# ZJU-FAST-Lab/Fast-Racing

Hardware: AMD Instinct MI355X
Metric: constraint-samples/s (higher is better)
Workload: dtype f64; 1 GPU; headline: 32 candidate trajs/GPU x 64 pieces x 16 quadrature intervals (34816 constraint samples/step/GPU), 16-gate Zhangjiajie-like corridor, K_i=8; state=iterate after 60 L-BFGS iterations from the reference initial guess, parallelism=candidates sharded 32/GPU, no data-path collective, front_end=one process, one device

## Files before the change

### fast-racing_amd/__init__.py

```python
from __future__ import annotations

import ctypes as C
import os

import numpy as np

from . import scenario

HERE = os.path.dirname(os.path.abspath(__file__))
LIB_PATH = os.path.join(HERE, "libfrx.so")

_dp = np.ctypeslib.ndpointer(dtype=np.float64, flags="C_CONTIGUOUS")
_ip = np.ctypeslib.ndpointer(dtype=np.int32, flags="C_CONTIGUOUS")


class FrxConfig(C.Structure):
    _fields_ = [
        ("rho", C.c_double), ("total_t", C.c_double), ("grid_res", C.c_double),
        ("qd_intervals", C.c_int), ("c2_diffeo", C.c_int),
        ("horiz_half_len", C.c_double), ("vert_half_len", C.c_double), ("safe_margin", C.c_double),
        ("vel_max", C.c_double), ("thr_acc_min", C.c_double), ("thr_acc_max", C.c_double),
        ("body_rate_max", C.c_double), ("grav_acc", C.c_double),
        ("penalty_pvtb", C.c_double * 4),
    ]

    @classmethod
    def from_params(cls, params: dict, **override):
        p = dict(params); p.update(override)
        c = cls()
        for name, _ in cls._fields_:
            if name == "penalty_pvtb":
                c.penalty_pvtb = (C.c_double * 4)(*p["penalty_pvtb"])
            else:
                setattr(c, name, p[name])
        return c


class LbfgsParams(C.Structure):
    _fields_ = [
        ("mem_size", C.c_int), ("g_epsilon", C.c_double), ("past", C.c_int), ("delta", C.c_double),
        ("max_iterations", C.c_int), ("max_linesearch", C.c_int), ("min_step", C.c_double), ("max_step", C.c_double),
        ("f_dec_coeff", C.c_double), ("s_curv_coeff", C.c_double), ("xtol", C.c_double),
    ]


BATCH_EVAL_FN = C.CFUNCTYPE(None, C.c_void_p, C.c_int, C.POINTER(C.c_int), C.POINTER(C.c_double), C.POINTER(C.c_double),
                            C.POINTER(C.c_double))

ABI_SYMBOLS = [
    "frx_version", "frx_last_error", "frx_device_count", "frx_lbfgs_default_params", "frx_lbfgs_gcopter_params",
    "frx_problem_create", "frx_problem_destroy", "frx_problem_set_solver", "frx_problem_set_lbfgs_mode", "frx_problem_totals", "frx_problem_layout", "frx_initial_guess",
    "frx_objective_eval", "frx_objective_eval_device", "frx_penalty_eval", "frx_penalty_eval_device", "frx_forward",
    "frx_optimize", "frx_optimize_stats", "frx_lbfgs_minimize_batch",
    "frx_problem_create_from_h", "frx_enumerate_vertices", "frx_traj_to_msg", "frx_msg_sample", "frx_line_segment_dilate", "frx_corridor_generate", "frx_traj_max_rates", "frx_objective_eval_async", "frx_wait",
    "frx_problem_set_resident", "frx_optimize_path", "frx_penalty_problem_create", "frx_eval_status",
    "frx_dilate_batch", "frx_multi_create", "frx_multi_destroy", "frx_multi_info", "frx_multi_layout", "frx_multi_initial_guess", "frx_multi_optimize", "frx_multi_last_exchange",
    "frx_map_mark_cloud", "frx_map_is_blocked", "frx_grid_search", "frx_jps_plan", "frx_route_plan",
    "frx_trajectory_check", "frx_trajectory_check_device", "frx_trajectory_sample", "frx_trajectory_sample_device",
    "frx_trajectory_extrema", "frx_trajectory_extrema_device",
    "frx_gate_from_corners", "frx_trajectory_gates", "frx_trajectory_gates_device", "frx_gate_flags",
    "frx_trajectory_clearance", "frx_trajectory_clearance_workspace", "frx_trajectory_clearance_device",
    "frx_corridor_generate_batch", "frx_corridor_generate_batch_device",
    "frx_enumerate_vertices_batch", "frx_enumerate_vertices_batch_device", "frx_corridor_slots_to_tasks_device",
]
DEBUG_SYMBOLS = [
    "frx_debug_trace", "frx_resident_profile", "frx_debug_direction_log", "frx_debug_direction_log_read", "frx_debug_set_resident_retry",
    "frx_debug_resident_counts", "frx_debug_resident_clusters", "frx_debug_resident_predictions", "frx_eval_stage_times", "frx_profile_phases", "frx_dv_selftest", "frx_jps_tables", "frx_debug_host_cpu_share", "frx_debug_taken_over", "frx_debug_compact_from_history",
    "frx_debug_set_eval_fused", "frx_debug_eval_fused", "frx_debug_eval_geometry", "frx_debug_set_eval_solo", "frx_debug_eval_solo", "frx_debug_penalty_kernel", "frx_debug_mailbox_numa", "frx_eval_launch_time", "frx_debug_profile_eval_cluster", "frx_debug_profile_eval_tail", "frx_debug_set_takeover_at", "frx_debug_shader_clock",
    "frx_debug_set_clear_chunk", "frx_debug_map_blocked_device", "frx_debug_dv_layout", "frx_debug_dv_round", "frx_debug_fold_rows",
]

CHECK_FIELDS = ("corridor", "speed", "thrust_min", "thrust_max", "body_rate", "acc", "worst_t", "worst_k")
CHECK_MAX_INTERVALS = 16384
CHECK_FLAG_CORRIDOR, CHECK_FLAG_SPEED, CHECK_FLAG_THRUST_MIN, CHECK_FLAG_THRUST_MAX, CHECK_FLAG_BODY_RATE, CHECK_FLAG_NONFINITE = 1, 2, 4, 8, 16, 32
EXTREMA_FIELDS = ("speed", "acc", "thrust_min", "thrust_max", "body_rate", "t_speed", "t_acc", "t_thrust_min", "t_thrust_max", "t_body_rate")
GATE_FIELDS = ("n_cross", "n_pass", "margin", "time", "piece", "u", "v", "reach_u", "reach_v", "normal_speed")
GATE_FLAG_MISSED, GATE_FLAG_REPEAT, GATE_FLAG_ORDER, GATE_FLAG_NONFINITE = 1, 2, 4, 8
CLEAR_FIELDS = ("ell", "dist", "worst_t", "worst_i")
CLEAR_MAX_POINTS = 1 << 24
CLEAR_FLAG_COLLISION, CLEAR_FLAG_NONFINITE = 1, 2
CLEAR_TILE, CLEAR_PASS = 64, 1024
SAMPLE_FIELDS = 20
SAMPLE_VIEWS = dict(pos=slice(0, 3), vel=slice(3, 6), acc=slice(6, 9), jerk=slice(9, 12), thrust=12, quat=slice(13, 17), omega=slice(17, 20))

_lib = None


def lib():
    global _lib
    if _lib is None:
        if not os.path.exists(LIB_PATH):
            raise RuntimeError(f"{LIB_PATH} is missing: build it first (python -c 'import __graft_entry__ as g; g.build()'). "
                               "There is no fallback implementation.")
        L = C.CDLL(LIB_PATH)
        L.frx_version.restype = C.c_int
        L.frx_last_error.restype = C.c_char_p
        L.frx_device_count.restype = C.c_int
        L.frx_lbfgs_default_params.argtypes = [C.POINTER(LbfgsParams)]
        L.frx_lbfgs_gcopter_params.argtypes = [C.POINTER(LbfgsParams), C.c_double]
        L.frx_problem_create.argtypes = [C.POINTER(FrxConfig), C.c_int, C.c_int, _ip, _dp, _dp, _ip, _dp, _ip, _dp, C.POINTER(C.c_void_p)]
        L.frx_problem_create_from_h.argtypes = [C.POINTER(FrxConfig), C.c_int, C.c_int, _ip, _dp, _dp, _ip, _dp, C.POINTER(C.c_void_p)]
        L.frx_enumerate_vertices.argtypes = [C.c_int, _dp, C.c_void_p, C.c_int, C.POINTER(C.c_int)]
        _up = np.ctypeslib.ndpointer(dtype=np.uint32, flags='C_CONTIGUOUS')
        L.frx_traj_to_msg.argtypes = [C.c_int, _dp, _dp, _dp, _dp, _dp, _dp, _up]
        L.frx_msg_sample.argtypes = [C.c_int, _dp, _dp, _dp, _dp, _up, C.c_double, _dp, _dp, _dp, _dp]
        L.frx_dv_selftest.argtypes = [C.c_int, C.c_int, C.c_int, C.c_int, C.c_int, C.c_void_p, C.c_uint, C.POINTER(C.c_double), C.POINTER(C.c_double)]
        L.frx_debug_dv_layout.argtypes = [C.c_int, C.c_void_p, C.c_int, C.c_void_p]
        L.frx_debug_dv_round.argtypes = [C.c_int, C.c_int, C.c_int, C.c_void_p, C.c_int] + [C.c_void_p] * 17
        L.frx_line_segment_dilate.argtypes = [_dp, _dp, _dp, C.c_int, C.c_void_p, C.c_double, C.c_int, C.POINTER(C.c_int), C.c_void_p, C.c_void_p, C.c_void_p]
        L.frx_corridor_generate.argtypes = [C.c_int, _dp, C.c_int, C.c_void_p, _dp, C.c_double, C.c_double, BLOCKED_FN, C.c_void_p, C.c_int, C.c_int,
                                            C.POINTER(C.c_int), _ip, _dp]
        L.frx_traj_max_rates.argtypes = [C.c_int, _dp, _dp, _dp, _dp]
        L.frx_objective_eval_async.argtypes = [C.c_void_p, _dp, _dp, _dp]
        L.frx_wait.argtypes = [C.c_void_p]
        L.frx_problem_set_resident.argtypes = [C.c_void_p, C.c_int]
        L.frx_optimize_path.argtypes = [C.c_void_p, C.POINTER(C.c_int), C.POINTER(C.c_uint)]
        L.frx_debug_trace.argtypes = [C.c_void_p, C.c_void_p, C.c_int]
        L.frx_resident_profile.argtypes = [C.c_void_p, C.c_void_p, C.c_int]
        L.frx_debug_direction_log.argtypes = [C.c_void_p, C.c_int, C.c_int]
        L.frx_debug_direction_log_read.argtypes = [C.c_void_p, C.c_int, C.c_void_p, C.c_int, C.POINTER(C.c_int), C.POINTER(C.c_int)]
        L.frx_debug_set_resident_retry.argtypes = [C.c_void_p, C.c_int]
        L.frx_debug_resident_counts.argtypes = [C.c_void_p, C.POINTER(C.c_int), C.POINTER(C.c_int)]
        L.frx_debug_resident_predictions.argtypes = [C.c_void_p, C.c_void_p]
        L.frx_debug_resident_clusters.argtypes = [C.c_void_p, C.POINTER(C.c_int)]
        L.frx_dilate_batch.argtypes = [C.c_int, C.c_int, _dp, _dp, _dp, C.c_int, C.c_void_p, C.c_double, C.c_int, _ip, _dp, _dp, _dp]
        L.frx_eval_stage_times.argtypes = [C.c_void_p, _dp, C.c_int, _dp]
        L.frx_eval_launch_time.argtypes = [C.c_void_p, _dp, C.c_int, _dp]
        L.frx_debug_set_eval_fused.argtypes = [C.c_void_p, C.c_int]
        L.frx_debug_eval_fused.argtypes = [C.c_void_p]
        L.frx_debug_eval_geometry.argtypes = [C.c_void_p]
        L.frx_debug_set_eval_solo.argtypes = [C.c_void_p, C.c_int]
        L.frx_debug_eval_solo.argtypes = [C.c_void_p]
        L.frx_debug_penalty_kernel.argtypes = [C.c_void_p]
        L.frx_debug_mailbox_numa.argtypes = [C.c_void_p, C.c_void_p]
        L.frx_debug_profile_eval_cluster.argtypes = [C.c_void_p, _dp, C.c_void_p]
        L.frx_debug_profile_eval_tail.argtypes = [C.c_void_p, _dp, C.c_void_p]
        L.frx_multi_create.argtypes = [C.POINTER(FrxConfig), C.c_int, C.c_void_p, C.c_int, _ip, _dp, _dp, _ip, _dp, _ip, _dp, C.POINTER(C.c_void_p)]
        L.frx_multi_destroy.argtypes = [C.c_void_p]
        L.frx_multi_info.argtypes = [C.c_void_p, C.POINTER(C.c_int), C.POINTER(C.c_int), C.c_void_p, C.c_void_p]
        L.frx_multi_layout.argtypes = [C.c_void_p, _ip, _ip]
        L.frx_multi_initial_guess.argtypes = [C.c_void_p, _dp]
        L.frx_multi_optimize.argtypes = [C.c_void_p, C.POINTER(LbfgsParams), _dp, _dp, _dp, _dp, _dp, _ip, _ip, _ip, C.POINTER(C.c_int), C.POINTER(C.c_double),
                                         _dp, _dp, C.POINTER(C.c_int)]
        L.frx_multi_last_exchange.argtypes = [C.c_void_p]
        L.frx_problem_destroy.argtypes = [C.c_void_p]
        L.frx_problem_set_solver.argtypes = [C.c_void_p, C.c_int]
        L.frx_problem_set_lbfgs_mode.argtypes = [C.c_void_p, C.c_int]
        L.frx_profile_phases.argtypes = [C.c_void_p, _dp, np.ctypeslib.ndpointer(dtype=np.int64, flags='C_CONTIGUOUS')]
        L.frx_problem_totals.argtypes = [C.c_void_p, _ip]
        L.frx_problem_layout.argtypes = [C.c_void_p, _ip, _ip, _ip, _ip]
        L.frx_initial_guess.argtypes = [C.c_void_p, _dp]
        L.frx_objective_eval.argtypes = [C.c_void_p, _dp, _dp, _dp]
        L.frx_objective_eval_device.argtypes = [C.c_void_p, C.c_void_p, C.c_void_p, C.c_void_p, C.c_void_p]
        L.frx_penalty_eval.argtypes = [C.c_void_p, _dp, _dp, _dp, _dp, _dp]
        L.frx_penalty_eval_device.argtypes = [C.c_void_p, C.c_void_p, C.c_void_p, C.c_void_p, C.c_void_p]
        L.frx_forward.argtypes = [C.c_void_p, _dp, _dp, _dp]
        L.frx_trajectory_check.argtypes = [C.c_void_p, C.c_void_p, C.c_void_p, C.c_int, C.c_void_p, C.c_void_p, C.c_void_p]
        L.frx_trajectory_check_device.argtypes = [C.c_void_p, C.c_void_p, C.c_void_p, C.c_int, C.c_void_p, C.c_void_p]
        L.frx_trajectory_extrema.argtypes = [C.c_void_p, C.c_void_p, C.c_void_p, C.c_void_p, C.c_void_p, C.c_void_p]
        L.frx_trajectory_extrema_device.argtypes = [C.c_void_p, C.c_void_p, C.c_void_p, C.c_void_p, C.c_void_p]
        L.frx_gate_from_corners.argtypes = [C.c_int, C.c_void_p, C.c_void_p, C.c_void_p]
        L.frx_trajectory_gates.argtypes = [C.c_void_p] * 7
        L.frx_trajectory_gates_device.argtypes = [C.c_void_p, C.c_void_p, C.c_void_p, C.c_int, C.c_void_p, C.c_void_p, C.c_void_p, C.c_void_p]
        L.frx_gate_flags.argtypes = [C.c_int, C.c_void_p, C.c_void_p, C.c_void_p]
        L.frx_trajectory_sample.argtypes = [C.c_void_p, C.c_void_p, C.c_void_p, C.c_int, C.c_double, C.c_double, C.c_void_p, C.c_void_p]
        L.frx_trajectory_sample_device.argtypes = [C.c_void_p, C.c_void_p, C.c_void_p, C.c_int, C.c_double, C.c_double, C.c_void_p, C.c_void_p, C.c_void_p]
        L.frx_trajectory_clearance.argtypes = [C.c_void_p, C.c_void_p, C.c_void_p, C.c_int, C.c_int, C.c_void_p, C.c_void_p, C.c_void_p, C.c_void_p]
        L.frx_trajectory_clearance_workspace.argtypes = [C.c_void_p, C.c_int, C.c_int, C.POINTER(C.c_size_t)]
        L.frx_trajectory_clearance_device.argtypes = [C.c_void_p, C.c_void_p, C.c_void_p, C.c_int, C.c_int, C.c_void_p, C.c_void_p, C.c_void_p, C.c_void_p]
        L.frx_debug_set_clear_chunk.argtypes = [C.c_void_p, C.c_int]
        L.frx_debug_fold_rows.argtypes = [C.c_int, C.c_int] + [C.c_void_p] * 6
        L.frx_corridor_generate_batch.argtypes = [C.c_int, C.c_int, C.c_void_p, C.c_void_p, C.c_int, C.c_void_p, C.c_void_p, C.c_double, C.c_double, C.c_void_p, C.c_int, C.c_int,
                                                  C.c_void_p, C.c_void_p, C.c_int, C.c_void_p, C.c_void_p, C.c_void_p]
        L.frx_corridor_generate_batch_device.argtypes = [C.c_int, C.c_void_p, C.c_void_p, C.c_int, C.c_void_p, C.c_void_p, C.c_double, C.c_double, C.c_void_p, C.c_int, C.c_int,
                                                         C.c_void_p, C.c_void_p, C.c_void_p, C.c_void_p, C.c_void_p]
        L.frx_enumerate_vertices_batch.argtypes = [C.c_int, C.c_int, C.c_void_p, C.c_void_p, C.c_void_p, C.c_int, C.c_void_p, C.c_void_p, C.c_int, C.c_void_p, C.c_void_p]
        L.frx_enumerate_vertices_batch_device.argtypes = [C.c_int, C.c_void_p, C.c_void_p, C.c_int, C.c_void_p, C.c_void_p, C.c_void_p, C.c_void_p]
        L.frx_corridor_slots_to_tasks_device.argtypes = [C.c_int, C.c_int, C.c_int, C.c_void_p, C.c_void_p, C.c_void_p, C.c_void_p]
        L.frx_debug_map_blocked_device.argtypes = [C.c_int, C.c_void_p, C.c_int, C.c_void_p, C.c_void_p, C.c_void_p]
        L.frx_optimize.argtypes = [C.c_void_p, C.POINTER(LbfgsParams), _dp, _dp, _dp, _dp, _dp, _ip, _ip, _ip]
        L.frx_optimize_stats.argtypes = [C.c_void_p, _dp]
        L.frx_lbfgs_minimize_batch.argtypes = [C.c_int, _ip, _dp, _dp, _ip, _ip, _ip, C.POINTER(LbfgsParams), BATCH_EVAL_FN,
                                               C.c_void_p, C.c_int]
        _vp = C.c_void_p
        L.frx_map_mark_cloud.argtypes = [C.c_double * 3, C.c_int * 3, C.c_double, C.c_int, _vp, _vp]
        L.frx_map_is_blocked.argtypes = [_vp, _vp, _vp]
        L.frx_grid_search.argtypes = [_vp, _vp, _vp, _vp, C.c_double, C.c_int, C.c_int, C.c_int, _vp, _vp, _vp, _vp]
        L.frx_jps_tables.argtypes = [_vp] * 6
        L.frx_jps_plan.argtypes = [_vp, _vp, _vp, C.c_double, C.c_int, C.c_int, _vp, _vp, _vp, _vp, _vp, _vp, _vp, _vp]
        L.frx_route_plan.argtypes = [_vp, _vp, _vp, C.c_int, _vp, C.c_double, C.c_int, C.c_int, C.c_int, _vp, _vp, _vp, _vp]
        for name in ABI_SYMBOLS + DEBUG_SYMBOLS:
            fn = getattr(L, name)
            if name not in ("frx_version", "frx_last_error", "frx_device_count", "frx_lbfgs_default_params",
                            "frx_lbfgs_gcopter_params", "frx_problem_destroy"):
                fn.restype = C.c_int
        _lib = L
    return _lib


class FrxError(RuntimeError):
    code = 0


def _check(rc: int):
    if rc != 0:
        e = FrxError(f"frx error {rc}: {lib().frx_last_error().decode()}")
        e.code = rc
        raise e


def shader_clock(device: int = 0, ms: float = 2.0):
    a, b, c = C.c_double(), C.c_double(), C.c_double()
    _check(lib().frx_debug_shader_clock(device, C.c_double(ms), C.byref(a), C.byref(b), C.byref(c)))
    return a.value, b.value, c.value


def gcopter_lbfgs_params(rel_cost_tol: float, max_iterations: int = 0) -> LbfgsParams:
    p = LbfgsParams()
    lib().frx_lbfgs_gcopter_params(C.byref(p), rel_cost_tol)
    p.max_iterations = max_iterations
    return p


def pack_batch(cands):
    coarse_n = np.array([c.coarse_n for c in cands], dtype=np.int32)
    ini = np.concatenate([c.ini_state.T.reshape(-1) for c in cands]).astype(np.float64)
    fin = np.concatenate([c.fin_state.T.reshape(-1) for c in cands]).astype(np.float64)
    h_off = [0]; v_off = [0]; h_rec = []; v_rec = []
    for c in cands:
        for h in c.h_polys:
            h_off.append(h_off[-1] + h.shape[1]); h_rec.append(h.T.reshape(-1))
        for v in c.v_polys:
            v_off.append(v_off[-1] + v.shape[1]); v_rec.append(v.T.reshape(-1))
    v_all = np.concatenate(v_rec).astype(np.float64) if v_rec else np.zeros(0)
    return (coarse_n, ini, fin, np.array(h_off, dtype=np.int32), np.concatenate(h_rec).astype(np.float64),
            np.array(v_off, dtype=np.int32), v_all)


def enumerate_vertices(hpoly: np.ndarray) -> np.ndarray:
    rec = np.ascontiguousarray(hpoly.T.reshape(-1), dtype=np.float64)
    nv = C.c_int()
    _check(lib().frx_enumerate_vertices(hpoly.shape[1], rec, None, 0, C.byref(nv)))
    out = np.zeros(3 * nv.value)
    _check(lib().frx_enumerate_vertices(hpoly.shape[1], rec, out.ctypes.data, nv.value, C.byref(nv)))
    return out.reshape(-1, 3).T.copy()


BLOCKED_FN = C.CFUNCTYPE(C.c_int, C.POINTER(C.c_double), C.POINTER(C.c_double), C.c_void_p)


def line_segment_dilate(p1, p2, bbox, obs, offset: float = 0.0):
    p1 = np.ascontiguousarray(p1, dtype=np.float64); p2 = np.ascontiguousarray(p2, dtype=np.float64); bbox = np.ascontiguousarray(bbox, dtype=np.float64)
    obs = np.ascontiguousarray(obs, dtype=np.float64).reshape(-1, 3)
    n = C.c_int()
    op = obs.ctypes.data if len(obs) else None
    _check(lib().frx_line_segment_dilate(p1, p2, bbox, len(obs), op, offset, 0, C.byref(n), None, None, None))
    rec = np.zeros(6 * n.value); Cm = np.zeros(9); d = np.zeros(3)
    _check(lib().frx_line_segment_dilate(p1, p2, bbox, len(obs), op, offset, n.value, C.byref(n), rec.ctypes.data, Cm.ctypes.data, d.ctypes.data))
    return rec.reshape(-1, 6).T.copy(), Cm.reshape(3, 3), d


def dilate_batch(p1, p2, bbox, obs, offset: float = 0.0, cap_planes: int = 96, device: int = 0):
    p1 = np.ascontiguousarray(p1, dtype=np.float64).reshape(-1, 3); p2 = np.ascontiguousarray(p2, dtype=np.float64).reshape(-1, 3)
    obs = np.ascontiguousarray(obs, dtype=np.float64).reshape(-1, 3)
    S = len(p1)
    npl = np.zeros(S, np.int32); rec = np.zeros(S * cap_planes * 6); Cm = np.zeros(S * 9); d = np.zeros(S * 3)
    _check(lib().frx_dilate_batch(device, S, p1.reshape(-1), p2.reshape(-1), np.ascontiguousarray(bbox, dtype=np.float64), len(obs),
                                  obs.ctypes.data if len(obs) else None, offset, cap_planes, npl, rec, Cm, d))
    rec = rec.reshape(S, cap_planes, 6)
    return [(rec[s, :npl[s]].T.copy(), Cm[9 * s:9 * s + 9].reshape(3, 3).copy(), d[3 * s:3 * s + 3].copy()) for s in range(S)]


def corridor_generate(path, obs, bbox, map_height: float, max_seg: float = 4.0, blocked=None, cap_polys: int = 4096, cap_planes: int = 1 << 18):
    path = np.ascontiguousarray(path, dtype=np.float64).reshape(-1, 3); obs = np.ascontiguousarray(obs, dtype=np.float64).reshape(-1, 3)
    user = None
    if isinstance(blocked, VoxelMap):
        cb = C.cast(lib().frx_map_is_blocked, BLOCKED_FN); user = C.cast(C.pointer(blocked._s), C.c_void_p)
    else:
        cb = BLOCKED_FN(lambda a, b, u: int(bool(blocked(np.array(a[:3]), np.array(b[:3]))))) if blocked else C.cast(None, BLOCKED_FN)
    n = C.c_int(); h_off = np.zeros(cap_polys + 1, dtype=np.int32); h_rec = np.zeros(6 * cap_planes)
    _check(lib().frx_corridor_generate(len(path), path.reshape(-1), len(obs), obs.ctypes.data if len(obs) else None, np.ascontiguousarray(bbox, dtype=np.float64),
                                       map_height, max_seg, cb, user, cap_polys, cap_planes, C.byref(n), h_off, h_rec))
    return [h_rec[6 * h_off[k]:6 * h_off[k + 1]].reshape(-1, 6).T.copy() for k in range(n.value)]
# ... 385 lines not shown

    def initial_guess(self):
        x = np.zeros(self.NX)
        _check(lib().frx_initial_guess(self.h, x))
        return x

    def objective(self, x):
        f = np.zeros(self.B); g = np.zeros(self.NX)
        _check(lib().frx_objective_eval(self.h, np.ascontiguousarray(x, dtype=np.float64), f, g))
        return f, g

    def objective_device(self, x_ptr: int, f_ptr: int, g_ptr: int, stream: int = 0):
        _check(lib().frx_objective_eval_device(self.h, x_ptr, f_ptr, g_ptr, stream))

    def penalty(self, T, Cf):
        cost = np.zeros(self.B); gdT = np.zeros(self.P); gdC = np.zeros(self.P * 18)
        _check(lib().frx_penalty_eval(self.h, np.ascontiguousarray(T, dtype=np.float64),
                                      np.ascontiguousarray(Cf, dtype=np.float64).reshape(-1), cost, gdT, gdC))
        return cost, gdT, gdC.reshape(-1, 3)

    def penalty_device(self, T_ptr: int, C_ptr: int, out_ptr: int, stream: int = 0):
        _check(lib().frx_penalty_eval_device(self.h, T_ptr, C_ptr, out_ptr, stream))

    def _traj_TC(self, who, T, Cf):
        T = np.ascontiguousarray(T, dtype=np.float64).reshape(-1); Cf = np.ascontiguousarray(Cf, dtype=np.float64).reshape(-1)
        if T.size != self.P or Cf.size != 18 * self.P:
            raise ValueError(f"{who}: expected {self.P} durations and {18 * self.P} coefficients, got {T.size} and {Cf.size}")
        return T, Cf

    def _traj_folded(self, fields, cand_key, entry, *args):
        piece = np.zeros((self.P, len(fields))); cand = np.zeros((self.B, len(fields))); flags = np.zeros(self.B, np.uint32)
        _check(entry(self.h, *args, piece.ctypes.data, cand.ctypes.data, flags.ctypes.data))
        out = {"piece": piece, cand_key: cand, "flags": flags}
        out.update({name: cand[:, i] for i, name in enumerate(fields)})
        return out

    def trajectory_check(self, T, Cf, intervals: int = 256):
        T, Cf = self._traj_TC("trajectory_check", T, Cf)
        return self._traj_folded(CHECK_FIELDS, "candidate", lib().frx_trajectory_check, T.ctypes.data, Cf.ctypes.data, int(intervals))

    def trajectory_check_device(self, T_ptr: int, C_ptr: int, out_ptr: int, intervals: int = 256, stream: int = 0):
        _check(lib().frx_trajectory_check_device(self.h, T_ptr, C_ptr, int(intervals), out_ptr, stream))

    def trajectory_extrema(self, T, Cf):
        T, Cf = self._traj_TC("trajectory_extrema", T, Cf)
        return self._traj_folded(EXTREMA_FIELDS, "cand", lib().frx_trajectory_extrema, T.ctypes.data, Cf.ctypes.data)

    def trajectory_extrema_device(self, T_ptr: int, C_ptr: int, out_ptr: int, stream: int = 0):
        _check(lib().frx_trajectory_extrema_device(self.h, T_ptr, C_ptr, out_ptr, stream))

    def trajectory_gates(self, T, Cf, gates, gate_off):
        T, Cf = self._traj_TC("trajectory_gates", T, Cf)
        gate_off = np.ascontiguousarray(gate_off, dtype=np.int32).reshape(-1)
        gates = np.ascontiguousarray(gates, dtype=np.float64)
        if gate_off.size != self.B + 1:
            raise ValueError(f"trajectory_gates: gate_off must hold {self.B + 1} offsets, got {gate_off.size}")
        if gates.ndim != 2 or gates.shape[1] != 9 or gates.shape[0] != int(gate_off[-1]):
            raise ValueError(f"trajectory_gates: gates must have shape ({int(gate_off[-1])}, 9), got {gates.shape}")
        rows = np.zeros((gates.shape[0], len(GATE_FIELDS))); flags = np.zeros(self.B, np.uint32)
        _check(lib().frx_trajectory_gates(self.h, T.ctypes.data, Cf.ctypes.data, gate_off.ctypes.data, gates.ctypes.data, rows.ctypes.data, flags.ctypes.data))
        out = {"gate": rows, "flags": flags}
        out.update({name: rows[:, i] for i, name in enumerate(GATE_FIELDS)})
        return out

    def trajectory_gates_device(self, T_ptr: int, C_ptr: int, n_gates: int, gate_off_ptr: int, gates_ptr: int, out_ptr: int, stream: int = 0):
        _check(lib().frx_trajectory_gates_device(self.h, T_ptr, C_ptr, int(n_gates), gate_off_ptr, gates_ptr, out_ptr, stream))

    def trajectory_sample(self, T, Cf, n_samples: int, dt: float = 0.0, t0: float = 0.0, times=None):
        T, Cf = self._traj_TC("trajectory_sample", T, Cf)
        S = int(n_samples)
        tp = None
        if times is not None:
            times = np.ascontiguousarray(times, dtype=np.float64)
            if times.shape != (self.B, S):
                raise ValueError(f"trajectory_sample: times must have shape ({self.B}, {S}), got {times.shape}")
            tp = times.ctypes.data
        rows = np.empty((self.B, max(S, 0), SAMPLE_FIELDS))
        _check(lib().frx_trajectory_sample(self.h, T.ctypes.data, Cf.ctypes.data, S, float(t0), float(dt), tp, rows.ctypes.data))
        out = dict(rows=rows)
        out.update({name: rows[..., sl] for name, sl in SAMPLE_VIEWS.items()})
        return out

    def trajectory_sample_device(self, T_ptr: int, C_ptr: int, out_ptr: int, n_samples: int, dt: float = 0.0, t0: float = 0.0, times_ptr: int = 0,
                                 stream: int = 0):
        _check(lib().frx_trajectory_sample_device(self.h, T_ptr, C_ptr, int(n_samples), float(t0), float(dt), times_ptr or None, out_ptr, stream))

    def trajectory_clearance(self, T, Cf, obs, intervals: int = 256):
        T, Cf = self._traj_TC("trajectory_clearance", T, Cf)
        obs = np.ascontiguousarray(obs, dtype=np.float64)
        if obs.ndim != 2 or obs.shape[1] != 3:
            raise ValueError(f"trajectory_clearance: obs must have shape (n_obs, 3), got {obs.shape}")
        return self._traj_folded(CLEAR_FIELDS, "cand", lib().frx_trajectory_clearance, T.ctypes.data, Cf.ctypes.data, int(intervals), obs.shape[0], obs.ctypes.data)

    def trajectory_clearance_workspace(self, n_obs: int, intervals: int = 256) -> int:
        n = C.c_size_t(0)
        _check(lib().frx_trajectory_clearance_workspace(self.h, int(intervals), int(n_obs), C.byref(n)))
        return int(n.value)

    def trajectory_clearance_device(self, T_ptr: int, C_ptr: int, obs_ptr: int, n_obs: int, work_ptr: int, out_ptr: int, intervals: int = 256, stream: int = 0):
        _check(lib().frx_trajectory_clearance_device(self.h, T_ptr, C_ptr, int(intervals), int(n_obs), obs_ptr, work_ptr or None, out_ptr, stream))

    def set_clear_chunk(self, points: int):
        _check(lib().frx_debug_set_clear_chunk(self.h, int(points)))

    def forward(self, x):
        T = np.zeros(self.P); Cf = np.zeros(self.P * 18)
        _check(lib().frx_forward(self.h, np.ascontiguousarray(x, dtype=np.float64), T, Cf))
        return T, Cf.reshape(-1, 3)

    def optimize(self, rel_cost_tol: float, x0=None, max_iterations: int = 0):
        x = self.initial_guess() if x0 is None else np.ascontiguousarray(x0, dtype=np.float64).copy()
        pm = gcopter_lbfgs_params(rel_cost_tol, max_iterations)
        Cf = np.zeros(self.P * 18); T = np.zeros(self.P)
        jc = np.zeros(self.B); obj = np.zeros(self.B)
        st = np.zeros(self.B, np.int32); it = np.zeros(self.B, np.int32); ev = np.zeros(self.B, np.int32)
        _check(lib().frx_optimize(self.h, C.byref(pm), x, Cf, T, jc, obj, st, it, ev))
        stats = np.zeros(4)
        _check(lib().frx_optimize_stats(self.h, stats))
        resident, dev_status = self.optimize_path()
        return dict(x=x, C=Cf.reshape(-1, 3), T=T, jerk_cost=jc, objective=obj, status=st, iters=it, evals=ev,
                    ms_total=stats[0], ms_device=stats[1], ms_host=stats[2], rounds=int(stats[3]), resident=resident, device_status=dev_status,
                    resident_failed=self.resident_counts()[0], resident_retried=self.resident_counts()[1], predictions=self.resident_predictions(),
                    clusters=self.resident_clusters() if resident else 0, taken_over=self.taken_over())

    def stage_times(self, x, reps: int = 100):
        out = np.zeros(3)
        _check(lib().frx_eval_stage_times(self.h, np.ascontiguousarray(x, dtype=np.float64), reps, out))
        return {"forward": float(out[0]), "penalty": float(out[1]), "adjoint": float(out[2])}

    def eval_launch_time(self, x, reps: int = 100) -> float:
        out = np.zeros(1)
        _check(lib().frx_eval_launch_time(self.h, np.ascontiguousarray(x, dtype=np.float64), reps, out))
        return float(out[0])

    def profile_eval_cluster(self, x):
        out = np.zeros(64, np.int64)
        _check(lib().frx_debug_profile_eval_cluster(self.h, np.ascontiguousarray(x, dtype=np.float64), out.ctypes.data))
        return out

    def profile_eval_tail(self, x):
        out = np.zeros(80, np.int64)
        _check(lib().frx_debug_profile_eval_tail(self.h, np.ascontiguousarray(x, dtype=np.float64), out.ctypes.data))
        return out

    def set_eval_fused(self, on: bool):
        _check(lib().frx_debug_set_eval_fused(self.h, int(on)))

    def eval_fused(self) -> int:
        return int(lib().frx_debug_eval_fused(self.h))

    def eval_geometry(self) -> int:
        return int(lib().frx_debug_eval_geometry(self.h))

    def set_eval_solo(self, mode: int):
        _check(lib().frx_debug_set_eval_solo(self.h, int(mode)))

    def solo_applies(self) -> bool:
        was = int(lib().frx_debug_set_eval_solo(self.h, 2))
        if was != 0: return False
        ok = self.eval_solo() >= 1
        _check(lib().frx_debug_set_eval_solo(self.h, 1))
        return ok

    def eval_solo(self) -> int:
        return int(lib().frx_debug_eval_solo(self.h))

    def mailbox_numa(self):
        out = np.zeros(4, np.int32)
        _check(lib().frx_debug_mailbox_numa(self.h, out.ctypes.data))
        return {"cmd_node": int(out[0]), "res_node": int(out[1]), "device_node": int(out[2]), "caller_cpu": int(out[3])}

    def penalty_kernel(self) -> str:
        return {0: "frx::k_penalty", 1: "frx::k_penalty_lat", 2: "frx::k_penalty_lat2"}.get(int(lib().frx_debug_penalty_kernel(self.h)), "?")

    def algorithmic_bytes(self) -> int:
        return 312 * self.P + 48 * self.sum_K

    def samples(self) -> int:
        return self.P * (self.kappa + 1)


class PenaltyProblem(Problem):

    def __init__(self, params: dict, piece_n, piece_poly, h_polys, device: int = 0, **override):
        self.cfg = FrxConfig.from_params(params, **override)
        self.kappa = int(self.cfg.qd_intervals)
        piece_n = np.ascontiguousarray(piece_n, dtype=np.int32); piece_poly = np.ascontiguousarray(piece_poly, dtype=np.int32)
        h_off = np.zeros(len(h_polys) + 1, dtype=np.int32)
        for i, hp in enumerate(h_polys):
            h_off[i + 1] = h_off[i] + hp.shape[1]
        h_rec = np.ascontiguousarray(np.concatenate([hp.T.reshape(-1) for hp in h_polys]), dtype=np.float64)
        h = C.c_void_p()
        _check(lib().frx_penalty_problem_create(C.byref(self.cfg), device, len(piece_n), C.c_void_p(piece_n.ctypes.data), C.c_void_p(piece_poly.ctypes.data),
                                                C.c_void_p(h_off.ctypes.data), C.c_void_p(h_rec.ctypes.data), C.byref(h)))
        self.h = h
        t = np.zeros(6, dtype=np.int32)
        _check(lib().frx_problem_totals(self.h, t))
        self.B, self.P, self.Pc, self.NX, self.Kmax, self.sum_K = (int(v) for v in t)
        self.piece_off = np.zeros(self.B + 1, np.int32); self.coarse_off = np.zeros(self.B + 1, np.int32)
        self.x_off = np.zeros(self.B + 1, np.int32); self.dim_t = np.zeros(self.B, np.int32)
        _check(lib().frx_problem_layout(self.h, self.piece_off, self.coarse_off, self.x_off, self.dim_t))
```

### fast-racing_amd/csrc/frx_api.cpp

```cpp
#include <hip/hip_runtime_api.h>

#include <algorithm>
#include <atomic>
#include <cctype>
#include <cfloat>
#include <chrono>
#include <cmath>
#include <cstdint>
#include <cstdio>
#include <cstdlib>
#include <cstring>
#include <functional>
#include <map>
#include <memory>
#include <mutex>
#include <string>
#include <thread>

#include <pthread.h>
#include <sched.h>
#include <unistd.h>
#include <sys/syscall.h>
#include <vector>

#include "../../include/frx.h"
#include "../../include/frx_debug.h"
#include "frx_device.hpp"
#include "frx_launch_forms.hpp"
#include "frx_internal.hpp"
#include "frx_lbfgs.hpp"
#include "frx_host_pool.hpp"
#include "frx_host_setup.hpp"
#include "frx_compact.hpp"
#include "frx_traj_fold.hpp"
#include "frx_gate_host.hpp"

namespace {

thread_local std::string g_err = "";
int fail(int code, const std::string &msg) { g_err = msg; return code; }

#define HIP_TRY(expr)                                                                                   \
    do {                                                                                                \
        hipError_t e_ = (expr);                                                                         \
        if (e_ != hipSuccess)                                                                           \
            return fail(FRX_ERR_HIP, std::string(#expr) + ": " + hipGetErrorString(e_));                \
    } while (0)

struct HipEventPair {
    hipEvent_t e0 = nullptr, e1 = nullptr;
    hipError_t create() { hipError_t e = hipEventCreate(&e0); return e != hipSuccess ? e : hipEventCreate(&e1); }
    ~HipEventPair() { if (e0) (void)hipEventDestroy(e0); if (e1) (void)hipEventDestroy(e1); }
};

using clk = std::chrono::steady_clock;
inline double ms_since(clk::time_point t0) { return std::chrono::duration<double, std::milli>(clk::now() - t0).count(); }

template <class T> struct DevBuf {
    T *p = nullptr;
    size_t n = 0;
    ~DevBuf() { if (p) (void)hipFree(p); }
    void release() { if (p) (void)hipFree(p); p = nullptr; n = 0; }
    hipError_t alloc(size_t count) {
        release();
        const hipError_t e = hipMalloc((void **)&p, std::max<size_t>(count, 1) * sizeof(T));
        if (e == hipSuccess) n = count; else p = nullptr;
        return e;
    }
    hipError_t upload(const std::vector<T> &h) {
        hipError_t e = alloc(h.size());
        if (e != hipSuccess || h.empty()) return e;
        return hipMemcpy(p, h.data(), h.size() * sizeof(T), hipMemcpyHostToDevice);
    }
};
template <class T> struct PinBuf {
    T *p = nullptr;
    size_t n = 0;
    ~PinBuf() { if (p) (void)hipHostFree(p); }
    void release() { if (p) (void)hipHostFree(p); p = nullptr; n = 0; }
    hipError_t alloc(size_t count) {
        release();
        hipError_t e = hipHostMalloc((void **)&p, std::max<size_t>(count, 1) * sizeof(T), hipHostMallocMapped | hipHostMallocCoherent);
        if (e == hipSuccess) { n = count; std::memset(p, 0, std::max<size_t>(count, 1) * sizeof(T)); } else p = nullptr;
        return e;
    }
};

}

namespace frx {
int set_error(int code, const std::string &msg) { return fail(code, msg); }

static std::atomic<int> g_extra_plans{0};
void concurrent_plans_hint(int delta) { g_extra_plans.fetch_add(delta, std::memory_order_relaxed); }
double host_cpu_budget() {
    double cpus = (double)std::max(1u, std::thread::hardware_concurrency());
    cpu_set_t allowed;
    CPU_ZERO(&allowed);
    if (sched_getaffinity(0, sizeof(allowed), &allowed) == 0 && CPU_COUNT(&allowed) > 0) cpus = std::min(cpus, (double)CPU_COUNT(&allowed));
    auto read2 = [](const char *path, double &a, double &b) -> int {
        FILE *f = std::fopen(path, "r");
        if (!f) return 0;
        char t0[64] = {0}, t1[64] = {0};
        const int n = std::fscanf(f, "%63s %63s", t0, t1);
        std::fclose(f);
        if (n >= 1 && std::strcmp(t0, "max") == 0) return -1;
        if (n >= 1) a = std::atof(t0);
        if (n >= 2) b = std::atof(t1);
        return n;
    };
    double q = 0.0, per = 0.0;
    const int n2 = read2("/sys/fs/cgroup/cpu.max", q, per);
    if (n2 == 2 && q > 0.0 && per > 0.0) cpus = std::min(cpus, q / per);
    else if (n2 == 0) {
        double q1 = 0.0, p1 = 0.0, dummy = 0.0;
        if (read2("/sys/fs/cgroup/cpu/cpu.cfs_quota_us", q1, dummy) >= 1 && read2("/sys/fs/cgroup/cpu/cpu.cfs_period_us", p1, dummy) >= 1 && q1 > 0.0 && p1 > 0.0)
            cpus = std::min(cpus, q1 / p1);
    }
    if (const char *e = std::getenv("FRX_HOST_CPUS")) { const double v = std::atof(e); if (v > 0.0) cpus = v; }
    return std::max(1.0, cpus);
}
int host_cpu_share();
int mailbox_threads(int S) { return std::max(1, std::min(std::max(1, std::min(4, S / 16)), host_cpu_share() - 1)); }
static int share_of(int extra_plans) {
    int ranks = 1;
    if (const char *e = std::getenv("FRX_LOCAL_RANKS")) ranks = std::max(1, std::atoi(e));
    else if (const char *e2 = std::getenv("LOCAL_WORLD_SIZE")) {
        ranks = std::max(1, std::atoi(e2));
        cpu_set_t allowed;
        CPU_ZERO(&allowed);
        const long online = sysconf(_SC_NPROCESSORS_ONLN);
        if (ranks > 1 && sched_getaffinity(0, sizeof(allowed), &allowed) == 0 && online > 0 && (long)CPU_COUNT(&allowed) * ranks <= online) ranks = 1;
    }
    const int plans = ranks * (1 + std::max(0, extra_plans));
    return std::max(1, (int)(host_cpu_budget() / plans));
}
int host_cpu_share() { return share_of(g_extra_plans.load(std::memory_order_relaxed)); }
int mailbox_threads_for(int S, int extra_plans) { return std::max(1, std::min(std::max(1, std::min(4, S / 16)), share_of(extra_plans) - 1)); }
int host_cpu_share_for(int extra_plans) { return share_of(extra_plans); }
}

static bool device_numa_cpus(int device, cpu_set_t *out);
static bool device_numa_cpus_uncached(int device, cpu_set_t *out);
static bool device_numa_cpus(int device, cpu_set_t *out) {
    struct Entry { bool ok; cpu_set_t set; };
    static std::mutex lock;
    static std::map<int, Entry> cache;
    std::lock_guard<std::mutex> g(lock);
    auto it = cache.find(device);
    if (it == cache.end()) { Entry e; e.ok = device_numa_cpus_uncached(device, &e.set); it = cache.emplace(device, e).first; }
    if (it->second.ok) *out = it->second.set;
    return it->second.ok;
}
static bool device_numa_cpus_uncached(int device, cpu_set_t *out) {
    char bdf[64] = {0};
    if (hipDeviceGetPCIBusId(bdf, sizeof(bdf), device) != hipSuccess) return false;
    for (char *c = bdf; *c; c++) *c = (char)std::tolower(*c);
    int node = -1;
    { const std::string p = std::string("/sys/bus/pci/devices/") + bdf + "/numa_node"; if (FILE *f = std::fopen(p.c_str(), "r")) { if (std::fscanf(f, "%d", &node) != 1) node = -1; std::fclose(f); } }
    if (node < 0) return false;
    std::string list;
    { const std::string p = "/sys/devices/system/node/node" + std::to_string(node) + "/cpulist"; if (FILE *f = std::fopen(p.c_str(), "r")) { char buf[4096] = {0}; if (std::fgets(buf, sizeof(buf), f)) list = buf; std::fclose(f); } }
    if (list.empty()) return false;
    cpu_set_t allowed, want;
    CPU_ZERO(&allowed); CPU_ZERO(&want);
    if (sched_getaffinity(0, sizeof(allowed), &allowed) != 0) return false;
    for (size_t i = 0; i < list.size();) {
        if (!std::isdigit((unsigned char)list[i])) { i++; continue; }
        size_t j = i; int a = 0; while (j < list.size() && std::isdigit((unsigned char)list[j])) a = 10 * a + (list[j++] - '0');
        int b = a;
        if (j < list.size() && list[j] == '-') { j++; b = 0; while (j < list.size() && std::isdigit((unsigned char)list[j])) b = 10 * b + (list[j++] - '0'); }
        for (int c = a; c <= b && c < CPU_SETSIZE; c++) if (CPU_ISSET(c, &allowed)) CPU_SET(c, &want);
        i = j;
    }
    if (CPU_COUNT(&want) < 2) return false;
    *out = want;
    return true;
}

struct NumaScope {
    cpu_set_t saved; bool active = false;
    explicit NumaScope(int device) {
        const char *e = std::getenv("FRX_NUMA"), *ea = std::getenv("FRX_NUMA_ALLOC");
        cpu_set_t want;
        if ((e && e[0] == '0') || (ea && ea[0] == '0') || !device_numa_cpus(device, &want)) return;
        if (pthread_getaffinity_np(pthread_self(), sizeof(saved), &saved) != 0) return;
        active = pthread_setaffinity_np(pthread_self(), sizeof(want), &want) == 0;
    }
    ~NumaScope() { if (active) (void)pthread_setaffinity_np(pthread_self(), sizeof(saved), &saved); }
};

constexpr int FRX_STAMP_SLOTS = 80;

struct frx_problem {
    frx_config cfg;
    int device = 0, B = 0, P = 0, Pc = 0, NX = 0, Kmax = 0, maxN = 0, maxCN = 0, sumKfine = 0;
    bool softT = true;
    std::vector<frx::HostCand> cand;
    std::vector<int> poff, coff, xoff, boff, dimT;
    frx::DevProblem dp;
    hipStream_t stream = nullptr;
    DevBuf<int> d_cvoff, d_poff, d_coff, d_xoff, d_boff, d_piece_hbeg, d_piece_K, d_piece_coarse, d_piece_iv, d_coarse_iv, d_coarse_fbeg, d_wp_vbeg,
        d_wp_nv, d_wp_xbeg;
    DevBuf<double> d_head, d_tail, d_hblk, d_vrec;
    DevBuf<double> d_x, d_f, d_g, d_T, d_C, d_band, d_out20;
    DevBuf<long long> d_stamps;
    DevBuf<double> d_pcrw;
    DevBuf<double> d_wq;
    PinBuf<double> h_x, h_f, h_g, h_T, h_C, h_out20;
    DevBuf<double> d_check;
    DevBuf<double> d_extrema;
    DevBuf<double> d_sample;
    DevBuf<double> d_gates;
    DevBuf<double> d_clear;
    int clear_chunk = 0;
    DevBuf<double> d_xp, d_gp, d_dir, d_S, d_Y, d_ys, d_gt;
    PinBuf<frx::DvCommand> h_cmd;
    PinBuf<frx::DvResult> h_res;
    int dv_mem = 0; size_t dv_hs = 0;
    double *pending_f = nullptr, *pending_g = nullptr;
    frx::TapLaunch tap;
    DevBuf<unsigned> d_arrive; PinBuf<unsigned> h_flag; DevBuf<int> d_flags, d_pflags;
    DevBuf<double> d_pubsyg, d_part, d_upub, d_dpub, d_rdbg, d_out20ll;
    int dirlog_cap = 0, dirlog_cands = 0, dirlog_nxp = 0;
    std::vector<double> dirlog;
    DevBuf<unsigned long long> d_rprof;
    std::vector<unsigned long long> rprof;
    DevBuf<unsigned> d_rwords;
    DevBuf<unsigned char> d_rargs;
    PinBuf<unsigned long long> h_rcmd, h_rres;
    int rk_B = 0, rk_S = 0, rk_G = 0, rk_NXP = 0;
    DevBuf<int> d_rs_int; DevBuf<double> d_rs_f, d_rs_rinv, d_rs_yy, d_rs_vd;
    int taken_over = 0;
    long takeover_at = 0;
    int resident_clusters = 0;
    int resident_mode = 1;
    int resident_retry = 0;
    int resident_retried = 0;
    unsigned long long spec_counts[4] = {0, 0, 0, 0};
    int resident_failed = 0;
    int resident_used = 0;
    unsigned resident_status = 0;
    std::vector<double> trace;
    DevBuf<unsigned long long> d_ev_ll; unsigned *d_ev_words = nullptr;
    int eval_fused = 0, eval_fused_G = 0, eval_fused_stamps = 0;
    unsigned long long eval_fused_ticks = 25000000ull;
    std::vector<unsigned char> ev_args, ev_args_st;
    DevBuf<unsigned char> d_ev_args, d_ev_args_st;
    PinBuf<unsigned> h_ev_status;
    unsigned eval_fused_code = 0;
    int eval_solo = 0, eval_solo_min_B = 0, eval_solo_max_B = 0;
    frx::LaunchGeom geo;
    bool banded_ok = true;
    bool penalty_only = false;
    int lbfgs_mode = 0;
    double stats[4] = {0, 0, 0, 0};
};

namespace {

int launch_eval(frx_problem *p, const double *x_dev, double *f_dev, double *g_dev, void *st, bool backward) {
    if (p->eval_fused && p->h_ev_status.p && *(volatile unsigned *)p->h_ev_status.p != 0u) { p->eval_fused_code = *(volatile unsigned *)p->h_ev_status.p; p->eval_fused = 0; }
    switch (frx::eval_route(backward, p->tap.d != nullptr, p->dp.cand_active != nullptr, p->dp.stamps != nullptr, p->eval_fused != 0, p->eval_fused_stamps != 0, p->eval_solo, p->B,
                            p->eval_solo_min_B, p->eval_solo_max_B, p->geo.lds_solo != 0, p->geo.solver == frx::SOLVER_KNOT_PCR)) {
    case frx::EVAL_CLUSTER: {
        const bool stamped = p->dp.stamps != nullptr;
        if (stamped && !p->d_ev_args_st.p) return (int)hipErrorInvalidValue;
        return frx::launch_eval_cluster(p->geo, p->B, stamped ? p->ev_args_st.data() : p->ev_args.data(), stamped ? p->d_ev_args_st.p : p->d_ev_args.p, x_dev, f_dev, g_dev, p->eval_fused_ticks, st, p->h_ev_status.p);
    }
    case frx::EVAL_SOLO: return frx::launch_eval_solo(p->dp, p->geo, x_dev, p->d_T.p, p->d_C.p, p->d_out20.p, f_dev, g_dev, st, p->tap);
    case frx::EVAL_STAGES: break;
    }
    int e = frx::launch_forward(p->dp, p->geo, x_dev, p->d_T.p, p->d_C.p, backward ? p->d_band.p : (double *)nullptr, st);
    if (e || !backward) return e;
    if ((e = frx::launch_penalty(p->dp, p->geo, p->d_T.p, p->d_C.p, p->d_out20.p, st))) return e;
    return frx::launch_backward(p->dp, p->geo, x_dev, p->d_T.p, p->d_C.p, p->d_band.p, p->d_out20.p, f_dev, g_dev, st, p->tap);
}

int eval_cluster_status(frx_problem *p, const double *f) {
    if (!p->eval_fused_G || !p->d_ev_words) return FRX_OK;
    const unsigned seen = p->h_ev_status.p ? *(volatile unsigned *)p->h_ev_status.p : 0u;
    if (!p->eval_fused && !p->eval_fused_code && !seen) return FRX_OK;
    bool any_nan = f == nullptr || seen != 0u || p->eval_fused_code != 0u;
    for (int b = 0; f && b < p->B; b++) any_nan = any_nan || f[b] != f[b];
    if (!any_nan) return FRX_OK;
    unsigned st = 0;
    unsigned *w = p->d_ev_words + (size_t)64 * p->B;
    HIP_TRY(hipMemcpy(&st, w, sizeof(unsigned), hipMemcpyDeviceToHost));
    if (st == 0 && seen == 0u && p->eval_fused_code == 0u) return FRX_OK;
    if (st == 0) st = seen ? seen : p->eval_fused_code;
    HIP_TRY(hipMemset(w, 0, sizeof(unsigned)));
    if (p->h_ev_status.p) *(volatile unsigned *)p->h_ev_status.p = 0u;
    p->eval_fused = 0; p->eval_fused_code = 0;
    return fail(FRX_ERR_TIMEOUT, "one-launch evaluation: a wait between the workgroups of a cluster expired (code " + std::to_string(st) + "); this handle continues with one launch per stage");
}

}

extern "C" {

int frx_version(void) { return FRX_VERSION; }
const char *frx_last_error(void) { return g_err.c_str(); }
int frx_device_count(void) {
    int n = 0;
    if (hipGetDeviceCount(&n) != hipSuccess) return 0;
    return n;
}
void frx_lbfgs_default_params(frx_lbfgs_params *p) { if (p) frx::lbfgs_defaults(*p); }
void frx_lbfgs_gcopter_params(frx_lbfgs_params *p, double rel_cost_tol) {
    if (!p) return;
    frx::lbfgs_defaults(*p);
    p->mem_size = 128; p->past = 3; p->g_epsilon = 1.0e-16; p->min_step = 1.0e-32; p->delta = rel_cost_tol;
}

int frx_problem_create(const frx_config *cfg, int device, int B, const int *coarse_n, const double *ini_state,
                       const double *fin_state, const int *h_off, const double *h_rec, const int *v_off, const double *v_rec,
                       frx_problem **out) {
    if (!cfg || !coarse_n || !ini_state || !fin_state || !h_off || !h_rec || !v_off || !v_rec || !out || B <= 0)
        return fail(FRX_ERR_INVALID_ARG, "frx_problem_create: null argument or B <= 0");
    if (cfg->qd_intervals < 1) return fail(FRX_ERR_INVALID_ARG, "qd_intervals must be >= 1");
    *out = nullptr;
    int ndev = 0;
    if (hipGetDeviceCount(&ndev) != hipSuccess || ndev <= 0)
        return fail(FRX_ERR_NO_DEVICE, "no HIP device available (this library has no CPU fallback)");
    if (device < 0 || device >= ndev) return fail(FRX_ERR_INVALID_ARG, "device ordinal out of range");
    if (hipSetDevice(device) != hipSuccess) return fail(FRX_ERR_NO_DEVICE, "hipSetDevice failed");

    const auto t_create0 = clk::now();
    frx_problem *p = new (std::nothrow) frx_problem();
    if (!p) return fail(FRX_ERR_ALLOC, "out of host memory");
    p->cfg = *cfg;
    p->device = device;
    p->B = B;
    p->softT = cfg->rho > 0;
    p->cand.resize(B);
    p->poff.assign(B + 1, 0); p->coff.assign(B + 1, 0); p->xoff.assign(B + 1, 0); p->boff.assign(B + 1, 0);
    p->dimT.assign(B, 0);

    std::vector<int> piece_hbeg, piece_K, piece_coarse, piece_iv, coarse_iv, coarse_fbeg, wp_vbeg, wp_nv, wp_xbeg, cvoff(B + 1, 0);
    std::vector<double> hrec, horg, vrec, head(ini_state, ini_state + 9 * (size_t)B), tail(fin_state, fin_state + 9 * (size_t)B);
    int hpoly = 0, vpoly = 0;
    for (int b = 0; b < B; b++) {
        frx::HostCand &hc = p->cand[b];
        const int cN = coarse_n[b];
        if (cN < 1) { delete p; return fail(FRX_ERR_INVALID_ARG, "coarse_n[b] < 1"); }
        if (frx::host_cand_init(hc, *cfg, p->softT, cN, ini_state + 9 * (size_t)b, fin_state + 9 * (size_t)b, v_off + vpoly, v_rec) != FRX_OK) {
            delete p; return fail(FRX_ERR_EMPTY_POLYTOPE, "a corridor polytope has no vertices");
        }
        cvoff[b] = (int)(vrec.size() / 3);
        const int gp0 = p->poff[b], gc0 = p->coff[b];
        int offset = 0;
        int xcur = p->xoff[b] + hc.dimT;
        for (int i = 0; i < cN; i++) {
            const int hb = h_off[hpoly + i], K = h_off[hpoly + i + 1] - hb;
            if (K < 1) { delete p; return fail(FRX_ERR_INVALID_ARG, "an H-polytope has no half-spaces"); }
            const int hbeg_dev = (int)(hrec.size() / 4);
            const double *org = h_rec + 6 * (size_t)hb + 3;
            horg.push_back(org[0]); horg.push_back(org[1]); horg.push_back(org[2]);
            for (int k = 0; k < K; k++) {
                const double *rec = h_rec + 6 * (size_t)(hb + k);
                const double nn = std::sqrt(rec[0] * rec[0] + rec[1] * rec[1] + rec[2] * rec[2]);
                const double n0 = rec[0] / nn, n1 = rec[1] / nn, n2 = rec[2] / nn;
                hrec.push_back(n0); hrec.push_back(n1); hrec.push_back(n2);
                hrec.push_back(n0 * (rec[3] - org[0]) + n1 * (rec[4] - org[1]) + n2 * (rec[5] - org[2]) - cfg->safe_margin);
            }
            p->Kmax = std::max(p->Kmax, K);
            coarse_iv.push_back(hc.intervals[i]);
            coarse_fbeg.push_back(gp0 + offset);
            for (int j = 0; j < hc.intervals[i]; j++) {
                int vm = -1;
                if (j < hc.intervals[i] - 1) vm = 2 * i;
                else if (i < cN - 1) vm = 2 * i + 1;
                if (vm >= 0) {
                    const int nv = (int)(hc.cfgVs[vm].size() / 3);
                    wp_vbeg.push_back((int)(vrec.size() / 3)); wp_nv.push_back(nv); wp_xbeg.push_back(xcur);
                    vrec.insert(vrec.end(), hc.cfgVs[vm].begin(), hc.cfgVs[vm].end());
                    xcur += nv - 1;
                }
                piece_hbeg.push_back(hbeg_dev); piece_K.push_back(K); piece_coarse.push_back(gc0 + i); piece_iv.push_back(hc.intervals[i]);
                p->sumKfine += K;
                offset++;
            }
        }
        hpoly += cN;
        vpoly += 2 * cN - 1;
        p->dimT[b] = hc.dimT;
        p->poff[b + 1] = gp0 + hc.fineN;
        p->coff[b + 1] = gc0 + cN;
        p->xoff[b + 1] = p->xoff[b] + hc.dimT + hc.dimP;
        p->boff[b + 1] = p->boff[b] + 6 * hc.fineN * FRX_BAND_W;
        p->maxN = std::max(p->maxN, hc.fineN);
        p->maxCN = std::max(p->maxCN, cN);
    }
    cvoff[B] = (int)(vrec.size() / 3);
    p->P = p->poff[B]; p->Pc = p->coff[B]; p->NX = p->xoff[B];
    int maxXb = 1, maxVb = 3;
    for (int b = 0; b < B; b++) {
        maxXb = std::max(maxXb, p->xoff[b + 1] - p->xoff[b]);
        maxVb = std::max(maxVb, 3 * (cvoff[b + 1] - cvoff[b]));
    }

    const int spp = cfg->qd_intervals + 1;
    frx::LaunchGeom &ge = p->geo;
    ge.maxN = p->maxN; ge.maxCN = p->maxCN; ge.Kmax = p->Kmax;
    ge.lpp = std::min(spp, 64);
    ge.ppw = 64 / ge.lpp;
    {
        int best_w = 1; double best_u = 0.0;
        for (int w = 1; w <= 4; w++) {
            const double u = (double)((64 * w) / ge.lpp * ge.lpp) / (64.0 * w);
            if (u > best_u + 1e-9) { best_u = u; best_w = w; }
        }
        int simds = 1024;
        { hipDeviceProp_t prop; if (hipGetDeviceProperties(&prop, device) == hipSuccess) simds = 4 * prop.multiProcessorCount; }
        if ((p->P + ge.ppw - 1) / ge.ppw <= simds) best_w = 1;
        if (const char *pw = std::getenv("FRX_PENALTY_WAVES")) { const int w = std::atoi(pw); if (w >= 1 && w <= 4) best_w = w; }
        while (best_w > 1 && frx::pen_wg_bytes((64 * best_w) / ge.lpp, p->Kmax, best_w, 21) > (size_t)160 * 1024) best_w--;
        ge.pen_w = best_w; ge.ppg = (64 * best_w) / ge.lpp;
    }
    ge.lds_fwd = sizeof(double) * ((size_t)6 * p->maxN * (FRX_BAND_W + 3) + p->maxN + p->maxCN);
    ge.lds_bwd = sizeof(double) * ((size_t)6 * p->maxN * (FRX_BAND_W + 6) + 2 * (size_t)p->maxN + p->maxCN);
    ge.lds_pen = frx::pen_wg_bytes(ge.ppg, p->Kmax, ge.pen_w, 21);
    ge.lds_pen2 = (ge.pen_w == 4 && spp <= 64) ? frx::pen_wg_bytes(ge.ppg, p->Kmax, ge.pen_w, 11) : 0;
    ge.solver = frx::SOLVER_KNOT_PCR;
    ge.knot_threads = 64 * ((p->maxN + 63) / 64);
    {
        const size_t nt = ge.knot_threads;
        ge.maxXb = maxXb; ge.maxVb = maxVb;
        ge.pcr_steps = 0;
        for (int s = 1; s < p->maxN - 1; s <<= 1) ge.pcr_steps++;
        ge.lds_kfwd = sizeof(double) * (36 * nt + 9 * (nt + 1) + nt + p->maxCN + maxXb + maxVb + (size_t)(ge.pcr_steps * 8 + 5) * nt);
        ge.pcr_steps = 0;
        for (int s = 1; s < p->maxN - 1; s <<= 1) ge.pcr_steps++;
        ge.lds_kbwd = sizeof(double) * (36 * nt + 9 * (nt + 1) + 2 * nt + p->maxCN + 2 * 4 + 2 + 2 * maxXb + maxVb + (size_t)(ge.pcr_steps * 8 + 5) * nt);
    }
    {
        int cus = 256;
        { hipDeviceProp_t prop; if (hipGetDeviceProperties(&prop, device) == hipSuccess) cus = prop.multiProcessorCount; }
        const char *ef = std::getenv("FRX_EVAL_FUSED");
        const int G = frx::eval_cluster_geometry(ge);
        int ranks = 1;
        if (const char *e = std::getenv("FRX_LOCAL_RANKS")) ranks = std::max(1, std::atoi(e));
        else if (const char *e2 = std::getenv("LOCAL_WORLD_SIZE")) ranks = std::max(1, std::atoi(e2));
        const bool shared_device = ranks > ndev && !(ef && ef[0] == '1');
        if (!G || (long long)B * G > cus || (ef && ef[0] == '0') || shared_device) { ge.ev_G = 0; ge.lds_ev = 0; }
        p->eval_fused_G = ge.ev_G; p->eval_fused = ge.ev_G ? 1 : 0;
        frx::eval_solo_geometry(ge, spp);
        p->eval_solo = ge.lds_solo ? 1 : 0; p->eval_solo_min_B = 384; p->eval_solo_max_B = 512;
        if (const char *es = std::getenv("FRX_EVAL_SOLO")) { if (es[0] == '0') p->eval_solo = 0; else if (es[0] == '1' && ge.lds_solo) p->eval_solo = 2; }
        if (const char *mb = std::getenv("FRX_EVAL_SOLO_MIN_B")) { const int v = std::atoi(mb); if (v > 0) p->eval_solo_min_B = v; }
        if (const char *mb = std::getenv("FRX_EVAL_SOLO_MAX_B")) { const int v = std::atoi(mb); if (v > 0) p->eval_solo_max_B = v; }
        if (const char *tm = std::getenv("FRX_EVAL_TIMEOUT_MS")) { const double v = std::atof(tm); if (v > 0.0) p->eval_fused_ticks = (unsigned long long)(v * 1e5); }
    }
    const size_t lds_cap = 160 * 1024;
    if (ge.knot_threads > 256 || ge.lds_kbwd > lds_cap) {
        delete p;
        return fail(FRX_ERR_CAPACITY, "a candidate's knot system does not fit one workgroup: " + std::to_string(ge.lds_kbwd / 1024) + " KB of LDS needed, 160 KB available (" +
                                          std::to_string(ge.knot_threads) + " knot threads, limit 256; about 128 pieces per candidate fit; the reference caps at 100, cuda_computer.cuh:24)");
    }
    p->banded_ok = !(ge.lds_bwd > lds_cap || ge.lds_fwd > lds_cap);
    if (!p->banded_ok) { ge.lds_fwd = ge.lds_bwd = 1024; }
    if (ge.lds_pen > lds_cap) {
        delete p;
        return fail(FRX_ERR_CAPACITY, "piece count / half-space count too large for the LDS-resident kernels (160 KiB per CU)");
    }

#define CR(expr)                                                                                        \
    do {                                                                                                \
        hipError_t e_ = (expr);                                                                         \
        if (e_ != hipSuccess) {                                                                         \
            std::string m_ = std::string(#expr) + ": " + hipGetErrorString(e_);                        \
            if (p->stream) (void)hipStreamDestroy(p->stream);                                           \
            delete p;                                                                                   \
            return fail(e_ == hipErrorOutOfMemory ? FRX_ERR_ALLOC : FRX_ERR_HIP, m_);                   \
        }                                                                                               \
    } while (0)
    const double ms_host_build = ms_since(t_create0);
    CR(hipStreamCreateWithFlags(&p->stream, hipStreamNonBlocking));
    CR((hipError_t)frx::launch_set_limits(p->geo));
    CR((hipError_t)frx::eval_solo_raise_limit(p->geo));
    if (p->geo.lds_solo && frx::eval_solo_blocks_per_cu(p->geo) < 1) { p->geo.lds_solo = 0; p->eval_solo = 0; }
    if (p->geo.ev_G && frx::eval_cluster_blocks_per_cu(p->geo.lds_ev) < 1) { p->geo.ev_G = 0; p->geo.lds_ev = 0; p->eval_fused_G = 0; p->eval_fused = 0; }
    CR(p->d_cvoff.upload(cvoff)); CR(p->d_poff.upload(p->poff)); CR(p->d_coff.upload(p->coff)); CR(p->d_xoff.upload(p->xoff)); CR(p->d_boff.upload(p->boff));
    CR(p->d_piece_hbeg.upload(piece_hbeg)); CR(p->d_piece_K.upload(piece_K)); CR(p->d_piece_coarse.upload(piece_coarse)); CR(p->d_piece_iv.upload(piece_iv));
    CR(p->d_coarse_iv.upload(coarse_iv)); CR(p->d_coarse_fbeg.upload(coarse_fbeg));
    CR(p->d_wp_vbeg.upload(wp_vbeg)); CR(p->d_wp_nv.upload(wp_nv)); CR(p->d_wp_xbeg.upload(wp_xbeg));
    CR(p->d_head.upload(head)); CR(p->d_tail.upload(tail)); {
        const int hs = (p->Kmax + 1) * 4;
        std::vector<double> hblk((size_t)p->P * hs, 0.0);
        for (int gp = 0; gp < p->P; gp++) {
            double *blk = &hblk[(size_t)gp * hs];
            const int gc = piece_coarse[gp], K = piece_K[gp];
            blk[0] = horg[3 * (size_t)gc]; blk[1] = horg[3 * (size_t)gc + 1]; blk[2] = horg[3 * (size_t)gc + 2]; blk[3] = (double)K;
            std::memcpy(blk + 4, &hrec[4 * (size_t)piece_hbeg[gp]], sizeof(double) * 4 * K);
        }
        CR(p->d_hblk.upload(hblk));
    } CR(p->d_vrec.upload(vrec));
    CR(p->d_x.alloc(p->NX)); CR(p->d_f.alloc(B)); CR(p->d_g.alloc(p->NX));
    CR(p->d_T.alloc(p->P)); CR(p->d_C.alloc((size_t)p->P * 18)); CR(p->d_band.alloc(p->boff[B])); CR(p->d_out20.alloc((size_t)p->P * 20));
    CR(p->d_pcrw.alloc((size_t)(p->geo.pcr_steps * 8 + 4) * p->P)); p->geo.pcrw = p->d_pcrw.p;
    CR(p->d_wq.alloc((size_t)4 * p->P)); CR(hipMemset(p->d_wq.p, 0, sizeof(double) * 4 * p->P));
    if (p->eval_fused_G) {
        const size_t n_ll = (size_t)40 * p->P, n_w64 = ((size_t)64 * B + 2) / 2;
        CR(p->d_ev_ll.alloc(n_ll + n_w64)); CR(hipMemset(p->d_ev_ll.p, 0, sizeof(unsigned long long) * (n_ll + n_w64)));
        p->d_ev_words = (unsigned *)(p->d_ev_ll.p + n_ll);
        { NumaScope numa_alloc(device); CR(p->h_ev_status.alloc(16)); }
        p->ev_args.assign(frx::eval_cluster_args_bytes(), 0); CR(p->d_ev_args.alloc(p->ev_args.size()));
    }
    {
        NumaScope numa_alloc(device);
        CR(p->h_x.alloc(p->NX)); CR(p->h_f.alloc(B)); CR(p->h_g.alloc(p->NX));
        CR(p->h_T.alloc(p->P)); CR(p->h_C.alloc((size_t)p->P * 18)); CR(p->h_out20.alloc((size_t)p->P * 20));
    }
#undef CR

    frx::DevProblem &d = p->dp;
    d.B = B; d.P = p->P; d.kappa = cfg->qd_intervals; d.inv_kappa = 1.0 / cfg->qd_intervals; d.soft = p->softT ? 1 : 0; d.c2 = cfg->c2_diffeo ? 1 : 0;
    d.rho = p->softT ? cfg->rho : 0.0;
    d.sumT = p->softT ? 1.0 : cfg->total_t;
    d.pc.ell[0] = cfg->horiz_half_len; d.pc.ell[1] = cfg->horiz_half_len; d.pc.ell[2] = cfg->vert_half_len;
    d.pc.safeMargin = cfg->safe_margin;
    d.pc.vMaxSqr = cfg->vel_max * cfg->vel_max;
    d.pc.thrMinSqr = cfg->thr_acc_min * cfg->thr_acc_min;
    d.pc.thrMaxSqr = cfg->thr_acc_max * cfg->thr_acc_max;
    d.pc.bdrMaxSqr = cfg->body_rate_max * cfg->body_rate_max;
    d.pc.gAcc = cfg->grav_acc;
    for (int q = 0; q < 4; q++) d.pc.chi[q] = cfg->penalty_pvtb[q];
    d.cvoff = p->d_cvoff.p; d.poff = p->d_poff.p; d.coff = p->d_coff.p; d.xoff = p->d_xoff.p; d.boff = p->d_boff.p;
    d.headPVA = p->d_head.p; d.tailPVA = p->d_tail.p;
    d.piece_hbeg = p->d_piece_hbeg.p; d.piece_K = p->d_piece_K.p; d.piece_coarse = p->d_piece_coarse.p; d.piece_iv = p->d_piece_iv.p;
    d.coarse_iv = p->d_coarse_iv.p; d.coarse_fbeg = p->d_coarse_fbeg.p;
    d.wp_vbeg = p->d_wp_vbeg.p; d.wp_nv = p->d_wp_nv.p; d.wp_xbeg = p->d_wp_xbeg.p;
    d.hblk = p->d_hblk.p; d.vrec = p->d_vrec.p; d.wq_glob = p->d_wq.p; d.stamps = nullptr; d.cand_active = nullptr; d.piece_active = nullptr;
    if (p->eval_fused_G) {
        frx::eval_cluster_args(p->dp, p->geo, p->d_T.p, p->d_C.p, p->d_ev_ll.p, p->d_ev_words, p->ev_args.data());
        const hipError_t e_ = hipMemcpy(p->d_ev_args.p, p->ev_args.data(), p->ev_args.size(), hipMemcpyHostToDevice);
        if (e_ != hipSuccess) { const std::string m_ = std::string("upload of the evaluation arguments: ") + hipGetErrorString(e_); (void)hipStreamDestroy(p->stream); delete p; return fail(FRX_ERR_HIP, m_); }
    }
    if (std::getenv("FRX_SETUP_TIMING")) fprintf(stderr, "[frx setup] frx_problem_create: B = %d, host descriptors %.3f ms, device allocations + uploads %.3f ms\n", B, ms_host_build, ms_since(t_create0) - ms_host_build);
    *out = p;
    return FRX_OK;
}

void frx_problem_destroy(frx_problem *p) {
    if (!p) return;
    (void)hipSetDevice(p->device);
    if (p->stream) { (void)hipStreamSynchronize(p->stream); (void)hipStreamDestroy(p->stream); }
    delete p;
}

int frx_penalty_problem_create(const frx_config *cfg, int device, int B, const int *piece_n, const int *piece_poly, const int *h_off, const double *h_rec,
                               frx_problem **out) {
    if (!cfg || !piece_n || !piece_poly || !h_off || !h_rec || !out || B <= 0) return fail(FRX_ERR_INVALID_ARG, "frx_penalty_problem_create: null argument or B <= 0");
    *out = nullptr;
    size_t P = 0;
    for (int b = 0; b < B; b++) { if (piece_n[b] < 1) return fail(FRX_ERR_INVALID_ARG, "piece_n[b] < 1"); P += (size_t)piece_n[b]; }
    std::vector<int> hoff2(P + 1, 0), voff(1, 0);
    std::vector<double> hrec2, vrec, states((size_t)9 * B, 0.0);
    for (size_t gp = 0; gp < P; gp++) {
        const int m = piece_poly[gp];
        if (m < 0) return fail(FRX_ERR_INVALID_ARG, "piece_poly: negative polytope index");
        const int hb = h_off[m], K = h_off[m + 1] - hb;
        if (K < 1) return fail(FRX_ERR_INVALID_ARG, "an H-polytope has no half-spaces");
        hrec2.insert(hrec2.end(), h_rec + 6 * (size_t)hb, h_rec + 6 * (size_t)(hb + K));
        hoff2[gp + 1] = hoff2[gp] + K;
    }
    for (int b = 0; b < B; b++)
        for (int q = 0; q < 2 * piece_n[b] - 1; q++) {
            const double v2[6] = {0.0, 0.0, 0.0, 1.0, 0.0, 0.0};
            vrec.insert(vrec.end(), v2, v2 + 6);
            voff.push_back(voff.back() + 2);
        }
    frx_config c2 = *cfg;
    c2.grid_res = INFINITY;
    if (!(c2.rho > 0.0)) { c2.rho = 1.0; }
    frx_problem *p = nullptr;
    const int rc = frx_problem_create(&c2, device, B, piece_n, states.data(), states.data(), hoff2.data(), hrec2.data(), voff.data(), vrec.data(), &p);
    if (rc != FRX_OK) return rc;
    p->penalty_only = true;
    *out = p;
    return FRX_OK;
}

int frx_problem_set_lbfgs_mode(frx_problem *p, int mode) {
    if (!p) return fail(FRX_ERR_INVALID_ARG, "null argument");
    if (mode != FRX_LBFGS_DEVICE_VECTORS && mode != FRX_LBFGS_HOST_VECTORS) return fail(FRX_ERR_INVALID_ARG, "unknown L-BFGS mode");
    p->lbfgs_mode = mode;
    return FRX_OK;
}

int frx_problem_set_solver(frx_problem *p, int solver) {
    if (!p) return fail(FRX_ERR_INVALID_ARG, "null argument");
    if (solver != FRX_SOLVER_KNOT_PCR && solver != FRX_SOLVER_BANDED_LU) return fail(FRX_ERR_INVALID_ARG, "unknown solver id");
    if (solver == FRX_SOLVER_BANDED_LU && !p->banded_ok)
        return fail(FRX_ERR_CAPACITY, "banded-LU kernels need the 6N x 13 band in LDS: too many pieces");
    p->geo.solver = solver;
    return FRX_OK;
}

int frx_profile_phases(frx_problem *p, const double *x, long long *out32) {
    if (!p || !x || !out32) return fail(FRX_ERR_INVALID_ARG, "null argument");
    HIP_TRY(hipSetDevice(p->device));
    if (!p->d_stamps.p) HIP_TRY(p->d_stamps.alloc(FRX_STAMP_SLOTS));
    HIP_TRY(hipMemset(p->d_stamps.p, 0, 64 * sizeof(long long)));
    std::vector<double> f(p->B), g(p->NX);
    int rc = frx_objective_eval(p, x, f.data(), g.data());
    if (rc != FRX_OK) return rc;
    p->dp.stamps = p->d_stamps.p;
    rc = frx_objective_eval(p, x, f.data(), g.data());
    p->dp.stamps = nullptr;
    if (rc != FRX_OK) return rc;
    HIP_TRY(hipMemcpy(out32, p->d_stamps.p, 32 * sizeof(long long), hipMemcpyDeviceToHost));
    return FRX_OK;
}

static int profile_eval_cluster(frx_problem *p, const double *x, long long *out, int first, int n) {
    if (!p || !x || !out) return fail(FRX_ERR_INVALID_ARG, "null argument");
    if (!p->eval_fused) return fail(FRX_ERR_INVALID_ARG, "the one-launch evaluation does not apply to this handle");
    HIP_TRY(hipSetDevice(p->device));
    if (!p->d_stamps.p) HIP_TRY(p->d_stamps.alloc(FRX_STAMP_SLOTS));
    HIP_TRY(hipMemset(p->d_stamps.p, 0, FRX_STAMP_SLOTS * sizeof(long long)));
    std::vector<double> f(p->B), g(p->NX);
    int rc = frx_objective_eval(p, x, f.data(), g.data());
    if (rc != FRX_OK) return rc;
    p->dp.stamps = p->d_stamps.p; p->eval_fused_stamps = 1;
    {
        p->ev_args_st.assign(frx::eval_cluster_args_bytes(), 0);
        frx::eval_cluster_args(p->dp, p->geo, p->d_T.p, p->d_C.p, p->d_ev_ll.p, p->d_ev_words, p->ev_args_st.data());
        hipError_t e_ = p->d_ev_args_st.p ? hipSuccess : p->d_ev_args_st.alloc(p->ev_args_st.size());
        if (e_ == hipSuccess) e_ = hipMemcpy(p->d_ev_args_st.p, p->ev_args_st.data(), p->ev_args_st.size(), hipMemcpyHostToDevice);
        if (e_ != hipSuccess) { p->dp.stamps = nullptr; p->eval_fused_stamps = 0; return fail(FRX_ERR_HIP, hipGetErrorString(e_)); }
    }
    rc = frx_objective_eval(p, x, f.data(), g.data());
    p->dp.stamps = nullptr; p->eval_fused_stamps = 0;
    if (rc != FRX_OK) return rc;
    HIP_TRY(hipMemcpy(out, p->d_stamps.p + first, n * sizeof(long long), hipMemcpyDeviceToHost));
    return FRX_OK;
}
int frx_debug_profile_eval_cluster(frx_problem *p, const double *x, long long *out64) { return profile_eval_cluster(p, x, out64, 0, 64); }
int frx_debug_profile_eval_tail(frx_problem *p, const double *x, long long *out80) { return profile_eval_cluster(p, x, out80, 0, FRX_STAMP_SLOTS); }

int frx_dv_selftest(int device, int n, int B, int m, int iters, const int *geom4, unsigned seed, double *max_rel_err, double *avg_us) {
    if (n < 1 || B < 1 || m < 1 || m > 512 || iters < 1 || !max_rel_err || !avg_us) return fail(FRX_ERR_INVALID_ARG, "bad selftest argument");
    HIP_TRY(hipSetDevice(device));
    int E = 0, W = 0, PF = 0, BLK = 4;
    frx::dv_geometry(n, &E, &W, &PF);
    if (geom4) { E = geom4[0]; W = geom4[1]; PF = geom4[2]; BLK = geom4[3]; }
    if (E == 0 || n > 64 * W * E) return fail(FRX_ERR_CAPACITY, "vector too long for k_lbfgs_pre");
    const char *tight_env = std::getenv("FRX_DV_TIGHT");
    const size_t HS = frx::dv_row_stride(n, E, W, !(tight_env && tight_env[0] == '0')), NX = (size_t)n * B;
    DevBuf<double> dx, dg, dxp, dgp, dd, dS, dY, dys, dgt; DevBuf<int> dxoff;
    PinBuf<frx::DvCommand> cmd; PinBuf<frx::DvResult> res;
    hipError_t e;
    if ((e = dx.alloc(NX)) || (e = dg.alloc(NX)) || (e = dxp.alloc(NX)) || (e = dgp.alloc(NX)) || (e = dd.alloc(NX)) || (e = dS.alloc(m * B * HS)) ||
        (e = dY.alloc(m * B * HS)) || (e = dys.alloc((size_t)B * m)) || (e = dgt.alloc((size_t)B * m * 4)) || (e = dxoff.alloc(B + 1)) || (e = cmd.alloc(B)) || (e = res.alloc(B)))
        return fail(FRX_ERR_ALLOC, hipGetErrorString(e));
    HIP_TRY(hipMemset(dS.p, 0, sizeof(double) * m * B * HS)); HIP_TRY(hipMemset(dY.p, 0, sizeof(double) * m * B * HS));
    HIP_TRY(hipMemset(dys.p, 0, sizeof(double) * B * m)); HIP_TRY(hipMemset(dgt.p, 0, sizeof(double) * B * m * 4));
    std::vector<int> xoff(B + 1);
    for (int b = 0; b <= B; b++) xoff[b] = b * n;
    HIP_TRY(hipMemcpy(dxoff.p, xoff.data(), sizeof(int) * (B + 1), hipMemcpyHostToDevice));
    frx::DvLaunch dv;
    dv.xoff = dxoff.p; dv.x = dx.p; dv.g = dg.p; dv.xp = dxp.p; dv.gp = dgp.p; dv.d = dd.p; dv.S = dS.p; dv.Y = dY.p; dv.ys = dys.p; dv.gt = dgt.p;
    dv.ld = NX; dv.hs = HS; dv.m = m; dv.B = B; dv.E = E; dv.W = W; dv.PF = PF; dv.BLK = BLK;
    unsigned long long st = 0x9E3779B97F4A7C15ull * (seed + 1);
    auto rnd = [&]() { st += 0x9E3779B97F4A7C15ull; unsigned long long z = st; z = (z ^ (z >> 30)) * 0xBF58476D1CE4E5B9ull; z = (z ^ (z >> 27)) * 0x94D049BB133111EBull; z ^= z >> 31; return (double)(z >> 11) * (1.0 / 9007199254740992.0) - 0.5; };
    std::vector<double> x(NX), g(NX), xp(NX), gp(NX), dref(n), ddev(NX);
    std::vector<std::vector<double>> S(B * (size_t)m, std::vector<double>(n)), Y(B * (size_t)m, std::vector<double>(n));
    std::vector<double> ysv((size_t)B * m), alpha(m);
    for (size_t i = 0; i < NX; i++) { x[i] = rnd(); g[i] = rnd(); }
    HIP_TRY(hipMemcpy(dx.p, x.data(), sizeof(double) * NX, hipMemcpyHostToDevice)); HIP_TRY(hipMemcpy(dg.p, g.data(), sizeof(double) * NX, hipMemcpyHostToDevice));
    for (int b = 0; b < B; b++) { cmd.p[b].flags = frx::DV_INIT; cmd.p[b].slot = cmd.p[b].bound = cmd.p[b].newest = 0; cmd.p[b].step = 0.0; }
    if (frx::launch_lbfgs_pre(dv, cmd.p, res.p, nullptr)) return fail(FRX_ERR_HIP, "k_lbfgs_pre launch (geometry not instantiated?)");
    HIP_TRY(hipDeviceSynchronize());
    xp = x; gp = g;
    HipEventPair evp; HIP_TRY(evp.create());
    const hipEvent_t e0 = evp.e0, e1 = evp.e1;
    double worst = 0.0, us_sum = 0.0; int us_n = 0, end = 0;
    for (int k = 1; k <= iters; k++) {
        for (size_t i = 0; i < NX; i++) { const double sx = 0.1 * rnd(); x[i] = xp[i] + sx; g[i] = gp[i] + 3.0 * sx + 0.05 * rnd(); }
        HIP_TRY(hipMemcpy(dx.p, x.data(), sizeof(double) * NX, hipMemcpyHostToDevice)); HIP_TRY(hipMemcpy(dg.p, g.data(), sizeof(double) * NX, hipMemcpyHostToDevice));
        const int bound = m <= k ? m : k;
        for (int b = 0; b < B; b++) { cmd.p[b].flags = frx::DV_ADVANCE; cmd.p[b].slot = end; cmd.p[b].bound = bound; cmd.p[b].newest = end; cmd.p[b].step = 0.0; }
        HIP_TRY(hipEventRecord(e0, nullptr));
        if (frx::launch_lbfgs_pre(dv, cmd.p, res.p, nullptr)) return fail(FRX_ERR_HIP, "k_lbfgs_pre launch");
        HIP_TRY(hipEventRecord(e1, nullptr));
        HIP_TRY(hipDeviceSynchronize());
        float ms = 0.f; HIP_TRY(hipEventElapsedTime(&ms, e0, e1));
        if (k > iters - 32) { us_sum += 1e3 * ms; us_n++; }
        HIP_TRY(hipMemcpy(ddev.data(), dd.p, sizeof(double) * NX, hipMemcpyDeviceToHost));
        for (int b = 0; b < B; b++) {
            double *sx = S[(size_t)b * m + end].data(), *yx = Y[(size_t)b * m + end].data();
            double ys = 0.0, yy = 0.0;
            for (int i = 0; i < n; i++) { sx[i] = x[b * (size_t)n + i] - xp[b * (size_t)n + i]; yx[i] = g[b * (size_t)n + i] - gp[b * (size_t)n + i]; ys += yx[i] * sx[i]; yy += yx[i] * yx[i]; }
            ysv[(size_t)b * m + end] = ys;
            for (int i = 0; i < n; i++) dref[i] = -g[b * (size_t)n + i];
            int j = (end + 1) % m;
            for (int i = 0; i < bound; i++) {
                j = (j + m - 1) % m;
                const double *sj = S[(size_t)b * m + j].data(), *yj = Y[(size_t)b * m + j].data();
                double a = 0.0; for (int q = 0; q < n; q++) a += sj[q] * dref[q];
                a /= ysv[(size_t)b * m + j]; alpha[j] = a;
                for (int q = 0; q < n; q++) dref[q] -= a * yj[q];
            }
            for (int q = 0; q < n; q++) dref[q] *= ys / yy;
            for (int i = 0; i < bound; i++) {
                const double *sj = S[(size_t)b * m + j].data(), *yj = Y[(size_t)b * m + j].data();
                double be = 0.0; for (int q = 0; q < n; q++) be += yj[q] * dref[q];
                be /= ysv[(size_t)b * m + j];
                for (int q = 0; q < n; q++) dref[q] += (alpha[j] - be) * sj[q];
                j = (j + 1) % m;
            }
            double num = 0.0, den = 0.0, dgr = 0.0;
            for (int q = 0; q < n; q++) { num = std::max(num, std::fabs(dref[q] - ddev[b * (size_t)n + q])); den = std::max(den, std::fabs(dref[q])); dgr += dref[q] * g[b * (size_t)n + q]; }
            worst = std::max(worst, num / den);
            worst = std::max(worst, std::fabs(res.p[b].dginit - dgr) / std::max(std::fabs(dgr), 1e-300));
        }
        xp = x; gp = g; end = (end + 1) % m;
    }
    *max_rel_err = worst; *avg_us = us_n ? us_sum / us_n : 0.0;
    return FRX_OK;
}

int frx_debug_dv_layout(int n_max, const int *geom4, int tight, int *out5) {
    if (n_max < 1 || !out5) return fail(FRX_ERR_INVALID_ARG, "bad layout argument");
    int E = 0, W = 0, PF = 0, BLK = 4;
    frx::dv_geometry(n_max, &E, &W, &PF);
    if (geom4) { E = geom4[0]; W = geom4[1]; PF = geom4[2]; BLK = geom4[3]; }
    if (E < 2 || E > 8 || (E & 1) || W < 1 || W > 8 || PF < 1 || PF > 16 || BLK < 1 || BLK > 4 || n_max > 64 * W * E)
        return fail(FRX_ERR_CAPACITY, "vector too long for k_lbfgs_pre (or no such geometry)");
    out5[0] = E; out5[1] = W; out5[2] = PF; out5[3] = BLK; out5[4] = (int)frx::dv_row_stride(n_max, E, W, tight != 0);
    return FRX_OK;
}

int frx_debug_dv_round(int device, int B, int m, const int *geom4, int hs, const long long *lens7, const int *xoff, double *x, double *g, double *xp, double *gp,
                       double *d, double *S, double *Y, double *ys, double *gt, const void *cmd, void *res, const int *poff, int *dflags, int *pflags,
                       const double *f) {
    if (B < 1 || m < 1 || m > 512 || !geom4 || !lens7 || !xoff || !x || !g || !xp || !gp || !d || !S || !Y || !ys || !gt || !cmd || !res)
        return fail(FRX_ERR_INVALID_ARG, "bad dv round argument");
    const int E = geom4[0], W = geom4[1], PF = geom4[2], BLK = geom4[3];
    if (E < 2 || E > 8 || (E & 1) || W < 1 || W > 8 || PF < 1 || PF > 16 || BLK < 1 || BLK > 4) return fail(FRX_ERR_INVALID_ARG, "no such k_lbfgs_pre geometry");
    const long long n_vec = lens7[0], n_hist = lens7[1], n_ys = lens7[2], n_gt = lens7[3], n_df = lens7[4], n_pf = lens7[5], n_res = lens7[6];
    int n_max = 0;
    if (xoff[0] < 0) return fail(FRX_ERR_INVALID_ARG, "xoff[0] < 0");
    for (int b = 0; b < B; b++) {
        if (xoff[b + 1] <= xoff[b]) return fail(FRX_ERR_INVALID_ARG, "every candidate needs at least one variable");
        n_max = std::max(n_max, xoff[b + 1] - xoff[b]);
    }
    if (n_max > 64 * W * E) return fail(FRX_ERR_CAPACITY, "vector too long for the geometry");
    if ((size_t)hs != frx::dv_row_stride(n_max, E, W, true) && hs != 64 * W * E) return fail(FRX_ERR_INVALID_ARG, "hs is neither the tight nor the full row of this batch");
    if (xoff[B] > n_vec || (long long)B * m * hs > n_hist || (long long)B * m > n_ys || (long long)B * m * 4 > n_gt || n_res < B)
        return fail(FRX_ERR_INVALID_ARG, "an array is shorter than the batch needs");
    const frx::DvCommand *hc = (const frx::DvCommand *)cmd;
    for (int b = 0; b < B; b++)
        if ((hc[b].flags & frx::DV_ADVANCE) && (hc[b].slot < 0 || hc[b].slot >= m || hc[b].bound < 1 || hc[b].bound > m))
            return fail(FRX_ERR_INVALID_ARG, "ADVANCE command with slot or bound outside the history");
    if (dflags && n_df < B) return fail(FRX_ERR_INVALID_ARG, "dflags shorter than the batch");
    if ((pflags != nullptr) != (poff != nullptr)) return fail(FRX_ERR_INVALID_ARG, "pflags and poff come together");
    if (pflags) {
        if (poff[0] < 0 || poff[B] > n_pf) return fail(FRX_ERR_INVALID_ARG, "pflags shorter than poff asks for");
        for (int b = 0; b < B; b++) if (poff[b + 1] < poff[b]) return fail(FRX_ERR_INVALID_ARG, "poff not ascending");
    }
    HIP_TRY(hipSetDevice(device));
    DevBuf<double> dx, dg, dxp, dgp, dd, dS, dY, dys, dgt, df; DevBuf<int> dxoff, dpoff, ddf, dpf;
    PinBuf<frx::DvCommand> pc; PinBuf<frx::DvResult> pr;
    hipError_t e;
    if ((e = dx.alloc(n_vec)) || (e = dg.alloc(n_vec)) || (e = dxp.alloc(n_vec)) || (e = dgp.alloc(n_vec)) || (e = dd.alloc(n_vec)) || (e = dS.alloc(n_hist)) ||
        (e = dY.alloc(n_hist)) || (e = dys.alloc(n_ys)) || (e = dgt.alloc(n_gt)) || (e = dxoff.alloc(B + 1)) || (e = pc.alloc(B)) || (e = pr.alloc(n_res)) ||
        (dflags && (e = ddf.alloc(n_df))) || (pflags && ((e = dpf.alloc(n_pf)) || (e = dpoff.alloc(B + 1)))) || (f && (e = df.alloc(B))))
        return fail(FRX_ERR_ALLOC, hipGetErrorString(e));
    auto up = [](auto &buf, const void *h, long long count) { return count > 0 ? hipMemcpy(buf.p, h, sizeof(*buf.p) * count, hipMemcpyHostToDevice) : hipSuccess; };
    auto down = [](void *h, auto &buf, long long count) { return count > 0 ? hipMemcpy(h, buf.p, sizeof(*buf.p) * count, hipMemcpyDeviceToHost) : hipSuccess; };
    HIP_TRY(up(dx, x, n_vec)); HIP_TRY(up(dg, g, n_vec)); HIP_TRY(up(dxp, xp, n_vec)); HIP_TRY(up(dgp, gp, n_vec)); HIP_TRY(up(dd, d, n_vec));
    HIP_TRY(up(dS, S, n_hist)); HIP_TRY(up(dY, Y, n_hist)); HIP_TRY(up(dys, ys, n_ys)); HIP_TRY(up(dgt, gt, n_gt)); HIP_TRY(up(dxoff, xoff, B + 1));
    if (dflags) HIP_TRY(up(ddf, dflags, n_df));
    if (pflags) { HIP_TRY(up(dpf, pflags, n_pf)); HIP_TRY(up(dpoff, poff, B + 1)); }
    if (f) HIP_TRY(up(df, f, B));
    std::memcpy(pc.p, cmd, sizeof(frx::DvCommand) * B); std::memcpy(pr.p, res, sizeof(frx::DvResult) * n_res);
    frx::DvLaunch dv;
    dv.xoff = dxoff.p; dv.x = dx.p; dv.g = dg.p; dv.xp = dxp.p; dv.gp = dgp.p; dv.d = dd.p; dv.S = dS.p; dv.Y = dY.p; dv.ys = dys.p; dv.gt = dgt.p;
    dv.dflags = dflags ? ddf.p : nullptr; dv.pflags = pflags ? dpf.p : nullptr; dv.poff = pflags ? dpoff.p : nullptr;
    dv.ld = (size_t)n_vec; dv.hs = (size_t)hs; dv.m = m; dv.B = B; dv.E = E; dv.W = W; dv.PF = PF; dv.BLK = BLK;
    if (frx::launch_lbfgs_pre(dv, pc.p, pr.p, nullptr)) return fail(FRX_ERR_HIP, "k_lbfgs_pre launch (geometry not instantiated?)");
    if (f && frx::launch_lbfgs_post(dv, df.p, pc.p, pr.p, nullptr)) return fail(FRX_ERR_HIP, "k_lbfgs_post launch");
    HIP_TRY(hipDeviceSynchronize());
    HIP_TRY(down(x, dx, n_vec)); HIP_TRY(down(g, dg, n_vec)); HIP_TRY(down(xp, dxp, n_vec)); HIP_TRY(down(gp, dgp, n_vec)); HIP_TRY(down(d, dd, n_vec));
    HIP_TRY(down(S, dS, n_hist)); HIP_TRY(down(Y, dY, n_hist)); HIP_TRY(down(ys, dys, n_ys)); HIP_TRY(down(gt, dgt, n_gt));
    if (dflags) HIP_TRY(down(dflags, ddf, n_df));
    if (pflags) HIP_TRY(down(pflags, dpf, n_pf));
    std::memcpy(res, pr.p, sizeof(frx::DvResult) * n_res);
    return FRX_OK;
}

int frx_eval_stage_times(frx_problem *p, const double *x, int reps, double *out3_us) {
    if (!p || !x || !out3_us || reps < 1) return fail(FRX_ERR_INVALID_ARG, "null argument or reps < 1");
    HIP_TRY(hipSetDevice(p->device));
    std::vector<double> f(p->B), g(p->NX);
    int rc;
    {
        struct Stage { frx_problem *q; int was, was_solo; ~Stage() { q->eval_fused = was; q->eval_solo = was_solo; } } stage{p, p->eval_fused, p->eval_solo};
        p->eval_fused = 0; p->eval_solo = 0;
        rc = frx_objective_eval(p, x, f.data(), g.data());
    }
    if (rc != FRX_OK) return rc;
    HipEventPair evp; HIP_TRY(evp.create());
    const hipEvent_t e0 = evp.e0, e1 = evp.e1;
    auto time_it = [&](int which, double &us) -> int {
        for (int w = 0; w < 3; w++) {
            hipError_t e = hipSuccess;
            if (which == 0) e = (hipError_t)frx::launch_forward(p->dp, p->geo, p->d_x.p, p->d_T.p, p->d_C.p, p->d_band.p, p->stream);
            if (which == 1) e = (hipError_t)frx::launch_penalty(p->dp, p->geo, p->d_T.p, p->d_C.p, p->d_out20.p, p->stream);
            if (which == 2) e = (hipError_t)frx::launch_backward(p->dp, p->geo, p->d_x.p, p->d_T.p, p->d_C.p, p->d_band.p, p->d_out20.p, p->d_f.p, p->d_g.p, p->stream);
            if (e != hipSuccess) return fail(FRX_ERR_HIP, hipGetErrorString(e));
        }
        if (hipEventRecord(e0, p->stream) != hipSuccess) return fail(FRX_ERR_HIP, "hipEventRecord");
        for (int r = 0; r < reps; r++) {
            if (which == 0) (void)frx::launch_forward(p->dp, p->geo, p->d_x.p, p->d_T.p, p->d_C.p, p->d_band.p, p->stream);
            if (which == 1) (void)frx::launch_penalty(p->dp, p->geo, p->d_T.p, p->d_C.p, p->d_out20.p, p->stream);
            if (which == 2) (void)frx::launch_backward(p->dp, p->geo, p->d_x.p, p->d_T.p, p->d_C.p, p->d_band.p, p->d_out20.p, p->d_f.p, p->d_g.p, p->stream);
        }
        if (hipEventRecord(e1, p->stream) != hipSuccess || hipEventSynchronize(e1) != hipSuccess) return fail(FRX_ERR_HIP, "hipEventSynchronize");
        float ms = 0.f;
        if (hipEventElapsedTime(&ms, e0, e1) != hipSuccess) return fail(FRX_ERR_HIP, "hipEventElapsedTime");
        us = 1e3 * ms / reps;
        return FRX_OK;
    };
    for (int k = 0; k < 3; k++) if ((rc = time_it(k, out3_us[k])) != FRX_OK) break;
    return rc;
}

int frx_debug_set_eval_fused(frx_problem *p, int enable) {
    if (!p) return fail(FRX_ERR_INVALID_ARG, "null argument");
    if (enable && p->eval_fused_G && (p->eval_fused_code || (p->h_ev_status.p && *(volatile unsigned *)p->h_ev_status.p))) (void)eval_cluster_status(p, nullptr);
    p->eval_fused = (enable && p->eval_fused_G) ? 1 : 0;
    p->eval_fused_ticks = enable == 2 ? 1ull : 25000000ull;
    return FRX_OK;
}
int frx_debug_eval_fused(const frx_problem *p) { return (p && p->eval_fused) ? p->eval_fused_G : 0; }
int frx_debug_eval_geometry(const frx_problem *p) { return (p && p->eval_fused) ? frx::eval_cluster_class(p->geo) : 0; }
int frx_debug_set_eval_solo(frx_problem *p, int mode) {
    if (!p || mode < 0 || mode > 2) return fail(FRX_ERR_INVALID_ARG, "null argument or unknown mode");
    if (mode == 2 && !p->geo.lds_solo) return fail(FRX_ERR_INVALID_ARG, "the solo form does not apply to this handle (more than 64 pieces or samples per piece, or the banded solver)");
    p->eval_solo = mode;
    return FRX_OK;
}
int frx_debug_penalty_kernel(const frx_problem *p) {
    if (!p) return -1;
    const char *f = std::getenv("FRX_PENALTY_FORM"), *tp = std::getenv("FRX_PENALTY_TWOPHASE");
    return frx::penalty_form_code(frx::penalty_form(p->geo.lds_pen2 != 0, p->geo.lpp, !f ? 0 : f[0] == 'l' ? 1 : 2, tp ? tp[0] : 0));
}
int frx_debug_eval_solo(const frx_problem *p) {
    if (!p) return 0;
    const frx::EvalRoute plain = frx::eval_route(true, false, false, false, p->eval_fused != 0, p->eval_fused_stamps != 0, p->eval_solo, p->B, p->eval_solo_min_B,
                                                 p->eval_solo_max_B, p->geo.lds_solo != 0, p->geo.solver == frx::SOLVER_KNOT_PCR);
    return plain == frx::EVAL_SOLO ? frx::eval_solo_blocks_per_cu(p->geo) : 0;
}
int frx_eval_launch_time(frx_problem *p, const double *x, int reps, double *out_us) {
    if (!p || !x || !out_us || reps < 1) return fail(FRX_ERR_INVALID_ARG, "null argument or reps < 1");
    HIP_TRY(hipSetDevice(p->device));
    std::vector<double> f(p->B), g(p->NX);
    int rc = frx_objective_eval(p, x, f.data(), g.data());
    if (rc != FRX_OK) return rc;
    HipEventPair evp; HIP_TRY(evp.create());
    for (int w = 0; w < 3; w++) HIP_TRY((hipError_t)launch_eval(p, p->d_x.p, p->d_f.p, p->d_g.p, p->stream, true));
    HIP_TRY(hipEventRecord(evp.e0, p->stream));
    for (int r = 0; r < reps; r++) (void)launch_eval(p, p->d_x.p, p->d_f.p, p->d_g.p, p->stream, true);
    HIP_TRY(hipEventRecord(evp.e1, p->stream));
    HIP_TRY(hipEventSynchronize(evp.e1));
    float ms = 0.f;
    HIP_TRY(hipEventElapsedTime(&ms, evp.e0, evp.e1));
    *out_us = 1e3 * ms / reps;
    HIP_TRY(hipMemcpy(f.data(), p->d_f.p, sizeof(double) * p->B, hipMemcpyDeviceToHost));
    return eval_cluster_status(p, f.data());
}

int frx_problem_totals(const frx_problem *p, int *out6) {
    if (!p || !out6) return fail(FRX_ERR_INVALID_ARG, "null argument");
    out6[0] = p->B; out6[1] = p->P; out6[2] = p->Pc; out6[3] = p->NX; out6[4] = p->Kmax; out6[5] = p->sumKfine;
    return FRX_OK;
}
int frx_problem_layout(const frx_problem *p, int *piece_off, int *coarse_off, int *x_off, int *dim_t) {
    if (!p) return fail(FRX_ERR_INVALID_ARG, "null argument");
    if (piece_off) std::copy(p->poff.begin(), p->poff.end(), piece_off);
    if (coarse_off) std::copy(p->coff.begin(), p->coff.end(), coarse_off);
    if (x_off) std::copy(p->xoff.begin(), p->xoff.end(), x_off);
    if (dim_t) std::copy(p->dimT.begin(), p->dimT.end(), dim_t);
    return FRX_OK;
}

int frx_initial_guess(frx_problem *p, double *x0) {
    if (!p || !x0) return fail(FRX_ERR_INVALID_ARG, "null argument");
    if (p->penalty_only) return fail(FRX_ERR_INVALID_ARG, "this handle serves frx_penalty_eval[_device] only (frx_penalty_problem_create)");
    frx::initial_guess_batch(p->cfg, p->softT, p->cand, p->xoff.data(), x0);
    return FRX_OK;
}

int frx_objective_eval_device(frx_problem *p, const double *x_dev, double *f_dev, double *g_dev, void *hip_stream) {
    if (!p || !x_dev || !f_dev || !g_dev) return fail(FRX_ERR_INVALID_ARG, "null argument");
    if (p->penalty_only) return fail(FRX_ERR_INVALID_ARG, "this handle serves frx_penalty_eval[_device] only (frx_penalty_problem_create)");
    HIP_TRY((hipError_t)launch_eval(p, x_dev, f_dev, g_dev, hip_stream, true));
    return FRX_OK;
}

int frx_eval_status(frx_problem *p) {
    if (!p) return fail(FRX_ERR_INVALID_ARG, "null argument");
    HIP_TRY(hipSetDevice(p->device));
    return eval_cluster_status(p, nullptr);
}

int frx_objective_eval(frx_problem *p, const double *x, double *f, double *g) {
    if (!p || !x || !f || !g) return fail(FRX_ERR_INVALID_ARG, "null argument");
    if (p->penalty_only) return fail(FRX_ERR_INVALID_ARG, "this handle serves frx_penalty_eval[_device] only (frx_penalty_problem_create)");
    HIP_TRY(hipSetDevice(p->device));
    std::memcpy(p->h_x.p, x, sizeof(double) * p->NX);
    HIP_TRY(hipMemcpyAsync(p->d_x.p, p->h_x.p, sizeof(double) * p->NX, hipMemcpyHostToDevice, p->stream));
    HIP_TRY((hipError_t)launch_eval(p, p->d_x.p, p->d_f.p, p->d_g.p, p->stream, true));
    HIP_TRY(hipMemcpyAsync(p->h_f.p, p->d_f.p, sizeof(double) * p->B, hipMemcpyDeviceToHost, p->stream));
    HIP_TRY(hipMemcpyAsync(p->h_g.p, p->d_g.p, sizeof(double) * p->NX, hipMemcpyDeviceToHost, p->stream));
    HIP_TRY(hipStreamSynchronize(p->stream));
    std::memcpy(f, p->h_f.p, sizeof(double) * p->B);
    std::memcpy(g, p->h_g.p, sizeof(double) * p->NX);
    return eval_cluster_status(p, f);
}

int frx_objective_eval_async(frx_problem *p, const double *x, double *f, double *g) {
    if (!p || !x || !f || !g) return fail(FRX_ERR_INVALID_ARG, "null argument");
    if (p->penalty_only) return fail(FRX_ERR_INVALID_ARG, "this handle serves frx_penalty_eval[_device] only (frx_penalty_problem_create)");
    if (p->pending_f) return fail(FRX_ERR_INVALID_ARG, "an asynchronous evaluation is already in flight on this handle (call frx_wait)");
    HIP_TRY(hipSetDevice(p->device));
    std::memcpy(p->h_x.p, x, sizeof(double) * p->NX);
    HIP_TRY(hipMemcpyAsync(p->d_x.p, p->h_x.p, sizeof(double) * p->NX, hipMemcpyHostToDevice, p->stream));
    HIP_TRY((hipError_t)launch_eval(p, p->d_x.p, p->d_f.p, p->d_g.p, p->stream, true));
    HIP_TRY(hipMemcpyAsync(p->h_f.p, p->d_f.p, sizeof(double) * p->B, hipMemcpyDeviceToHost, p->stream));
    HIP_TRY(hipMemcpyAsync(p->h_g.p, p->d_g.p, sizeof(double) * p->NX, hipMemcpyDeviceToHost, p->stream));
    p->pending_f = f; p->pending_g = g;
    return FRX_OK;
}
int frx_wait(frx_problem *p) {
    if (!p) return fail(FRX_ERR_INVALID_ARG, "null argument");
    HIP_TRY(hipSetDevice(p->device));
    HIP_TRY(hipStreamSynchronize(p->stream));
    if (p->pending_f) {
        std::memcpy(p->pending_f, p->h_f.p, sizeof(double) * p->B);
        std::memcpy(p->pending_g, p->h_g.p, sizeof(double) * p->NX);
        const double *fdone = p->pending_f;
        p->pending_f = nullptr; p->pending_g = nullptr;
        return eval_cluster_status(p, fdone);
    }
    return FRX_OK;
}

int frx_penalty_eval_device(frx_problem *p, const double *T_dev, const double *C_dev, double *out_dev, void *hip_stream) {
    if (!p || !T_dev || !C_dev || !out_dev) return fail(FRX_ERR_INVALID_ARG, "null argument");
    HIP_TRY((hipError_t)frx::launch_penalty(p->dp, p->geo, T_dev, C_dev, out_dev, hip_stream));
    return FRX_OK;
}

static int stage_TC(frx_problem *p, const double *T, const double *C) {
    std::memcpy(p->h_T.p, T, sizeof(double) * p->P);
    std::memcpy(p->h_C.p, C, sizeof(double) * 18 * (size_t)p->P);
    HIP_TRY(hipMemcpyAsync(p->d_T.p, p->h_T.p, sizeof(double) * p->P, hipMemcpyHostToDevice, p->stream));
    HIP_TRY(hipMemcpyAsync(p->d_C.p, p->h_C.p, sizeof(double) * 18 * (size_t)p->P, hipMemcpyHostToDevice, p->stream));
    return FRX_OK;
}
static int fetch_rows(frx_problem *p, const double *d_rows, size_t n, double *piece_out) {
    HIP_TRY(hipMemcpyAsync(p->h_out20.p, d_rows, sizeof(double) * n, hipMemcpyDeviceToHost, p->stream));
    HIP_TRY(hipStreamSynchronize(p->stream));
    if (piece_out) std::memcpy(piece_out, p->h_out20.p, sizeof(double) * n);
    return FRX_OK;
}
static int grow(DevBuf<double> &buf, size_t need, const char *entry) {
    if (buf.n < need && buf.alloc(need) != hipSuccess) {
        (void)hipGetLastError();
        return fail(FRX_ERR_ALLOC, std::string(entry) + ": cannot allocate " + std::to_string(need * sizeof(double)) + " bytes on the device");
    }
    return FRX_OK;
}
#define FRX_TRY(expr) do { const int rc_ = (expr); if (rc_ != FRX_OK) return rc_; } while (0)

int frx_penalty_eval(frx_problem *p, const double *T, const double *C, double *cost, double *gdT, double *gdC) {
    if (!p || !T || !C || !cost || !gdT || !gdC) return fail(FRX_ERR_INVALID_ARG, "null argument");
    HIP_TRY(hipSetDevice(p->device));
    FRX_TRY(stage_TC(p, T, C));
    FRX_TRY(frx_penalty_eval_device(p, p->d_T.p, p->d_C.p, p->d_out20.p, p->stream));
    FRX_TRY(fetch_rows(p, p->d_out20.p, 20 * (size_t)p->P, nullptr));
    for (int b = 0; b < p->B; b++) {
        double s = 0.0;
        for (int gp = p->poff[b]; gp < p->poff[b + 1]; gp++) {
            const double *o = p->h_out20.p + 20 * (size_t)gp;
            s += o[0];
            gdT[gp] += o[1];
            for (int v = 0; v < 18; v++) gdC[18 * (size_t)gp + v] += o[2 + v];
// ... 1082 lines not shown
```

### fast-racing_amd/csrc/frx_device.hpp

```cpp
#pragma once
#include <cstddef>
#include <cstdlib>

#include "frx_math.hpp"

#define FRX_BAND_W 13

namespace frx {

struct DevProblem {
    int B, P, kappa, soft, c2;
    double rho, sumT;
    double inv_kappa;
    PenaltyConst pc;
    const int *poff, *coff, *xoff, *boff;
    const int *cvoff;
    const double *headPVA, *tailPVA;
    const int *piece_hbeg, *piece_K;
    const int *piece_coarse, *piece_iv;
    const int *coarse_iv, *coarse_fbeg;
    const int *wp_vbeg, *wp_nv, *wp_xbeg;
    const double *hblk;
    const double *vrec;
    const int *cand_active, *piece_active;
    double *wq_glob;
    long long *stamps;
};

enum { SOLVER_KNOT_PCR = 0, SOLVER_BANDED_LU = 1 };

struct LaunchGeom {
    int maxN, maxCN, Kmax, lpp, ppw;
    int pen_w, ppg;
    size_t lds_fwd, lds_bwd, lds_pen;
    size_t lds_pen2;
    int solver;
    int knot_threads;
    size_t lds_kfwd, lds_kbwd;
    int maxXb, maxVb;
    int pcr_steps;
    double *pcrw;
    int ev_G = 0;
    size_t lds_ev = 0;
    size_t lds_solo = 0;
};

inline bool env_is(const char *name, char ch) { const char *e = std::getenv(name); return e && e[0] == ch; }
inline bool env_off(const char *name) { return env_is(name, '0'); }

struct TapLaunch {
    const double *d = nullptr; const int *flags = nullptr; void *res = nullptr;
    unsigned *arrive = nullptr; volatile unsigned *flag = nullptr; unsigned round = 0;
};

int raise_lds_limit(const void *fn, size_t bytes);
int launch_set_limits(const LaunchGeom &g);
int launch_forward(const DevProblem &dp, const LaunchGeom &g, const double *x, double *T, double *C, double *band, void *stream);
int launch_penalty(const DevProblem &dp, const LaunchGeom &g, const double *T, const double *C, double *out20, void *stream);
int launch_backward(const DevProblem &dp, const LaunchGeom &g, const double *x, const double *T, const double *C,
                    const double *band, const double *out20, double *f, double *grad, void *stream, const TapLaunch &tap = TapLaunch());


int eval_cluster_class(const LaunchGeom &g);
int eval_cluster_geometry(LaunchGeom &g);
size_t eval_cluster_args_bytes();
void eval_cluster_args(const DevProblem &dp, const LaunchGeom &g, double *T, double *C, unsigned long long *ll, unsigned *words, void *out);
int launch_eval_cluster(const LaunchGeom &g, int B, const void *args_host, const void *args_dev, const double *x, double *f, double *grad,
                        unsigned long long timeout_ticks, void *stream, unsigned *status_host = nullptr);
int eval_cluster_blocks_per_cu(size_t lds_bytes);
int eval_cluster_raise_limit(size_t lds_bytes);

int eval_solo_geometry(LaunchGeom &g, int samples_per_piece);
int eval_solo_raise_limit(const LaunchGeom &g);
int eval_solo_blocks_per_cu(const LaunchGeom &g);
int launch_eval_solo(const DevProblem &dp, const LaunchGeom &g, const double *x, double *T, double *C, double *out20, double *f, double *grad, void *stream,
                     const TapLaunch &tap = TapLaunch());

int check_geometry(int intervals, int Kmax, int *lpp, int *ppw);
int launch_check(const DevProblem &dp, int Kmax, const double *T, const double *C, int intervals, double *out, void *stream);

enum { EXTREMA_FIELDS = 10 };
int launch_extrema(int P, double g_acc, const double *T, const double *C, double *out, void *stream);

enum { GATE_FIELDS = 10 };
int launch_gates(int B, const int *poff, double g_acc, const double *ell, const double *T, const double *C, int n_gates, const int *gate_off,
                 const double *gates, double *out, void *stream);

int sample_fits(int maxN);
int launch_sample(const DevProblem &dp, int maxN, const double *T, const double *C, int S, double t0, double dt, const double *times, double *out,
                  void *stream);

enum { CLEAR_TILE = 64,
       CLEAR_PASS = 1024,
       CLEAR_TARGET_WGS = 2048 };
inline int clear_geometry(int P, int n_obs, int force, int *chunk, int *nchunks) {
    long long c = force;
    if (force <= 0) {
        const long long want = P < CLEAR_TARGET_WGS ? CLEAR_TARGET_WGS / P : 1;
        c = ((long long)n_obs + want - 1) / want;
        c = (c + CLEAR_PASS - 1) / CLEAR_PASS * CLEAR_PASS;
    }
    const long long nc = ((long long)n_obs + c - 1) / c;
    if ((long long)P * nc > 0x7fffffffLL) return 0;
    *chunk = (int)(c < n_obs ? c : n_obs); *nchunks = (int)nc;
    return 1;
}
int launch_clear(const DevProblem &dp, const double *T, const double *C, int intervals, int n_obs, const double *obs, int chunk, int nchunks,
                 double *work, double *rows, void *stream);

struct DvBuffers;
struct DvLaunch {
    const int *xoff; double *x, *g, *xp, *gp, *d, *S, *Y, *ys, *gt; int *dflags = nullptr, *pflags = nullptr; const int *poff = nullptr; size_t ld; size_t hs = 0; int m, B, E, W, PF, BLK;
};
inline void dv_geometry(int n, int *E, int *W, int *PF) {
    size_t best = ~(size_t)0;
    *E = *W = *PF = 0;
    for (int e : {8, 6, 4, 2})
        for (int w = 1; w <= 8; w++) {
            const size_t hs = (size_t)64 * w * e;
            if ((size_t)n <= hs && hs < best) { best = hs; *E = e; *W = w; *PF = e == 2 ? 16 : e == 8 ? 4 : 8; }
        }
}
inline size_t dv_row_stride(int n, int E, int W, bool tight = true) {
    const size_t HS = (size_t)64 * W * E, hs = ((size_t)n + 2 + 15) & ~(size_t)15;
    if (!tight || hs >= HS) return HS;
    if (HS < 512) return HS;
    if (hs / 2 <= (size_t)64 * W * (E / 2 - 1)) return HS;
    return hs;
}
int launch_lbfgs_pre(const DvLaunch &dv, const void *cmd, void *res, void *stream);

struct RoundLaunch {
    double *x, *g, *xp, *gp, *d, *f, *T, *C, *out20;
    unsigned long long *out20ll = nullptr;
    double *pubsyg, *part, *upub, *dpub, *dbg;
    unsigned *words;
    void *h_cmd, *h_res;
    unsigned long long timeout_ticks;
    unsigned long long *prof = nullptr;
    unsigned long long *trace = nullptr; int trace_cap = 0; unsigned trace_lo = 0, trace_hi = 0;
    int B, S, G, m, E, NXP;
    int dbg_cap = 0, dbg_cands = 0;
    double ls_ftol = 1e-4, ls_gtol = 0.9, ls_min_step = 1e-20, ls_max_step = 1e20, ls_xtol = 1e-16;
    int ls_max_linesearch = 40, speculate = 1;
    int cmd_stride = 4;
    int fast_control = 1;
    int stamp_round = 0;
    const int *rs_cand = nullptr, *rs_newest = nullptr, *rs_bound = nullptr;
    const double *rs_f = nullptr, *rs_S = nullptr, *rs_Y = nullptr, *rs_rinv = nullptr, *rs_yy = nullptr, *rs_vd = nullptr;
    size_t rs_hs = 0;
    void *args_dev = nullptr;
};
enum { ROUND_E = 56, ROUND_E_SMALL = 28, ROUND_WORDS_PER_CAND = 128 };
size_t round_lds_bytes(const LaunchGeom &g, int m, int E);
size_t round_args_bytes();
int launch_round(const DevProblem &dp, const LaunchGeom &g, const RoundLaunch &r, void *stream);
int launch_lbfgs_post(const DvLaunch &dv, const double *f, const void *cmd, void *res, void *stream);

struct DilateLaunch {
    const double *p1, *p2, *obs;
    double bbox[3], offset;
    int S, n_obs, cap_planes, pcap;
    int *n_planes; double *h_rec, *ell_C, *ell_d;
};
size_t dilate_lds_bytes(int pcap);
int launch_clock_probe(double *out, unsigned long long *stamps, int blocks, unsigned long long ticks, void *stream);
int launch_dilate(const DilateLaunch &d, void *stream);

struct ChainLaunch {
    const int *path_off; const double *path, *obs;
    double map_origin[3], map_res; int map_dim[3]; const signed char *map_cells;
    double bbox[3], map_height, max_seg;
    int n_paths, n_obs, cap_polys, cap_planes, pcap;
    double *h_slot; int *cell_planes, *n_polys, *status;
};
enum { CHAIN_PCAP = 4096, CHAIN_MAX_PLANES = 512 };
size_t chain_lds_bytes(int pcap, int cap_planes);
int launch_chain(const ChainLaunch &c, void *stream);
int launch_map_blocked_pairs(const ChainLaunch &map_of, int n, const double *a, const double *b, int *out, void *stream);

struct EnumLaunch {
    const int *tasks; const double *h_rec;
    int n_tasks, cap_v;
    double *v_slot; int *nv, *status;
};
enum { ENUM_MAX_PLANES = 256, ENUM_MIN_CAP_V = 4, ENUM_MAX_CAP_V = 512 };
size_t enumerate_lds_bytes(int cap_v);
int launch_enumerate(const EnumLaunch &e, void *stream);
int launch_slots_to_tasks(int n_paths, int cap_polys, int cap_planes, const int *cell_planes, const int *n_polys, int *tasks, void *stream);

}
```

### fast-racing_amd/csrc/frx_device_eval.hip

```cpp
#include <hip/hip_runtime.h>

#include <algorithm>
#include <cassert>
#include <cstdint>
#include <cstdlib>
#include <cstring>
#include <type_traits>

#define FRX_KERNEL_LINKAGE static
#include "frx_eval_kernel.hpp"
#include "frx_launch_forms.hpp"

namespace frx {

static const EvalSwitches &eval_switches() {
    static const EvalSwitches s{!env_off("FRX_EVAL_ARGPTR"), !env_off("FRX_EVAL_EARLY_T"), !env_off("FRX_EVAL_TAIL"), !env_off("FRX_EVAL_HANDOFF"), !env_off("FRX_EVAL_CHAIN"), !env_off("FRX_EVAL_GEOM")};
    return s;
}
typedef eval_geom<EvalGeomK16> GeomK16;
static_assert(GeomK16::pen_lds == pen_wave_doubles(GeomK16::ppw, GeomK16::kmax), "the class's per-wave LDS is pen_wave_doubles of its integers");
static bool eval_geom_class(const LaunchGeom &g) { return g.ev_G && g.lpp == GeomK16::lpp && g.ppw == GeomK16::ppw && g.Kmax == GeomK16::kmax && g.pcr_steps == GeomK16::nsteps; }
int eval_cluster_class(const LaunchGeom &g) { return (eval_switches().geom_on() && eval_geom_class(g)) ? 1 : 0; }

template <bool ARGP, bool ET, bool TAIL = true, bool HO = false, bool CH = false, class GEO = void> struct eval_inst {
    static constexpr EvalClusterForm form() { return {ARGP, ET, TAIL, HO, CH, !std::is_void<GEO>::value}; }
};
template <class F> static int with_eval_kernel(const EvalClusterForm &m, F &&f) {
#define FRX_EVAL_FORM(...) if (m == eval_inst<__VA_ARGS__>::form()) return f(k_eval_cluster<__VA_ARGS__>);
    FRX_EVAL_FORM(true, true, true, true)
    FRX_EVAL_FORM(true, false, true, true)
    FRX_EVAL_FORM(true, true, true, true, true)
    FRX_EVAL_FORM(true, false, true, true, true)
    FRX_EVAL_FORM(true, true, false)
    FRX_EVAL_FORM(true, true)
    FRX_EVAL_FORM(true, false)
    FRX_EVAL_FORM(false, true)
    FRX_EVAL_FORM(false, false)
    FRX_EVAL_FORM(true, true, true, true, true, EvalGeomK16)
    FRX_EVAL_FORM(true, true, true, true, false, EvalGeomK16)
#undef FRX_EVAL_FORM
    return (int)hipErrorInvalidValue;
}
static EvalClusterForm eval_plain_form() { EvalClusterForm m; (void)eval_cluster_form(eval_switches(), false, false, true, m); return m; }

int eval_cluster_raise_limit(size_t bytes) {
    EvalClusterForm forms[4];
    const int n = eval_cluster_raised_forms(eval_switches(), forms);
    for (int i = 0; i < n; i++)
        if (const int e = with_eval_kernel(forms[i], [&](auto kernel) { return raise_lds_limit((const void *)kernel, bytes); })) return e;
    return 0;
}
int eval_cluster_geometry(LaunchGeom &g) {
    g.ev_G = 0; g.lds_ev = 0;
    (void)eval_switches();
    if (g.solver != SOLVER_KNOT_PCR || g.knot_threads != 64 || g.ppw < 1) return 0;
    const int ntasks = (g.maxN + g.ppw - 1) / g.ppw;
    const size_t lds = sizeof(double) * (size_t)eval_cluster_lds(g.maxN * 19, g.maxXb, g.maxVb, g.maxCN, g.pcr_steps, pen_wave_doubles(g.ppw, g.Kmax)).total;
    if (lds > (size_t)160 * 1024) return 0;
    g.ev_G = 1 + (ntasks + 3) / 4;
    g.lds_ev = lds;
    return g.ev_G;
}
int eval_cluster_blocks_per_cu(size_t lds_bytes) {
    int n = 0;
    (void)with_eval_kernel(eval_plain_form(), [&](auto kernel) {
        if (hipOccupancyMaxActiveBlocksPerMultiprocessor(&n, (const void *)kernel, 256, lds_bytes) != hipSuccess) { (void)hipGetLastError(); n = 0; }
        return 0;
    });
    return n;
}
size_t eval_cluster_args_bytes() { return sizeof(EvalClusterArgs); }
void eval_cluster_args(const DevProblem &dp, const LaunchGeom &g, double *T, double *C, unsigned long long *ll, unsigned *words, void *out) {
    EvalClusterArgs a;
    std::memset(&a, 0, sizeof(a));
    assert(!eval_switches().handoff_on() || (reinterpret_cast<uintptr_t>(ll) & 15u) == 0);
    a.dp = dp; a.T = T; a.C = C; a.out20ll = ll; a.words = words; a.status = words + (size_t)64 * dp.B;
    a.G = g.ev_G; a.maxCN = g.maxCN; a.maxXb = g.maxXb; a.maxVb = g.maxVb; a.nsteps = g.pcr_steps; a.lpp = g.lpp; a.ppw = g.ppw; a.Kmax = g.Kmax; a.pen_lds = pen_wave_doubles(g.ppw, g.Kmax); a.maxN19 = g.maxN * 19;
    std::memcpy(out, &a, sizeof(a));
}
int launch_eval_cluster(const LaunchGeom &g, int B, const void *args_host, const void *args_dev, const double *x, double *f, double *grad,
                        unsigned long long timeout_ticks, void *stream, unsigned *status_host) {
    if (!g.ev_G) return (int)hipErrorInvalidValue;
    EvalCallArgs c;
    c.x = x; c.f = f; c.g = grad; c.status_host = status_host; c.timeout_ticks = timeout_ticks;
    c.force_wt = env_is("FRX_EVAL_FUSED_WT", '1') ? 1 : 0;
    c.test_drop_members = timeout_ticks == 1ull ? 1 : 0;
    if (c.test_drop_members) c.timeout_ticks = 5000ull;
    const dim3 grid(8 * g.ev_G * ((B + 7) / 8));
    const EvalClusterArgs *host = (const EvalClusterArgs *)args_host;
    EvalClusterForm m;
    if (!eval_cluster_form(eval_switches(), eval_geom_class(g), host->dp.stamps != nullptr, args_dev != nullptr, m)) return (int)hipErrorInvalidValue;
    assert(!m.geo || (host->pen_lds == GeomK16::pen_lds && host->nsteps == GeomK16::nsteps));
    return with_eval_kernel(m, [&](auto kernel) {
        if constexpr (std::is_same<decltype(kernel), void (*)(EvalClusterArgs, EvalCallArgs)>::value) hipLaunchKernelGGL(kernel, grid, dim3(256), g.lds_ev, (hipStream_t)stream, *host, c);
        else hipLaunchKernelGGL(kernel, grid, dim3(256), g.lds_ev, (hipStream_t)stream, (const EvalClusterArgs *)args_dev, c);
        return (int)hipGetLastError();
    });
}
}
```

### fast-racing_amd/csrc/frx_eval_kernel.hpp

```cpp
#pragma once
#include <type_traits>

#include "frx_round_kernel.hpp"

namespace frx {

struct EvalClusterArgs {
    DevProblem dp;
    double *T, *C;
    ll_u64 *out20ll;
    unsigned *words;
    unsigned *status;
    int G, maxCN, maxXb, maxVb, nsteps, lpp, ppw, Kmax, pen_lds, maxN19;
};

struct EvalClusterLds { int ctl, xs, vs, pw, wq, ev, mem, total; };
__host__ __device__ inline EvalClusterLds eval_cluster_lds(int maxN19, int maxXb, int maxVb, int maxCN, int nsteps, int pen_lds) {
    EvalClusterLds L;
    int o = 2;
    L.ctl = o; o += (maxN19 + 1) & ~1;
    L.xs = o; o += (maxXb + 1) & ~1;
    L.vs = o; o += (maxVb + 1) & ~1;
    L.pw = o; o += ((nsteps * 8 + 5) * 64 + 1) & ~1;
    L.wq = o; o += 4 * 64;
    L.ev = o;
    const int e = 36 * 64 + 9 * 65 + 2 * 64 + maxCN + 16;
    o += (e + 1) & ~1;
    L.mem = o;
    L.total = o + 4 * pen_lds + 8;
    return L;
}

struct EvalCallArgs {
    const double *x; double *f, *g;
    unsigned *status_host;
    rk_u64 timeout_ticks;
    int test_drop_members;
    int force_wt;
};
template <class F, bool NS = false> struct EvalEarlySync {
    static constexpr bool nostamps = NS;
    const F &f; long long *st; bool steps;
    __device__ __forceinline__ bool sync() const { return f(); }
};
struct EvalGeomK16 { static constexpr int LPP = 17, PPW = 3, KMAX = 8, NSTEPS = 6; };
template <class GEO> struct eval_geom {
    static constexpr bool fixed = true;
    static constexpr int lpp = GEO::LPP, ppw = GEO::PPW, kmax = GEO::KMAX, nsteps = GEO::NSTEPS;
    static constexpr int hstride = (kmax + 1) * 4, pen_lds = ppw * 19 + ppw * hstride + 64 * 21;
    static_assert(ppw * lpp <= 64 && ppw * hstride <= 2 * 64, "a wave-task: one lane per sample, one double2 of its corridor blocks per lane");
};
template <> struct eval_geom<void> { static constexpr bool fixed = false; static constexpr int lpp = 0, ppw = 0, kmax = 0, nsteps = 0, hstride = 0, pen_lds = 0; };
template <bool ARGP, bool ET, bool TAIL = true, bool HO = false, bool CH = false, class GEO = void>
__global__ __launch_bounds__(256, 1) void k_eval_cluster(typename std::conditional<ARGP, const EvalClusterArgs *__restrict__, EvalClusterArgs>::type arg, EvalCallArgs call) {
    static_assert(!CH || (ARGP && TAIL && HO), "the production form: argument pointer, inline tail, value-major hand-off");
    typedef eval_geom<GEO> GC;
    constexpr bool GF = GC::fixed;
    static_assert(!GF || (ARGP && ET && TAIL && HO), "the geometry class: the default form of every other switch");
    const EvalClusterArgs &a = [&]() -> const EvalClusterArgs & { if constexpr (ARGP) return *arg; else return arg; }();
    const auto stp = [&]() -> long long * { if constexpr (CH) return nullptr; else return a.dp.stamps; };
    extern __shared__ __attribute__((aligned(16))) double sm[];
    const int lane8 = blockIdx.x & 7, rest = blockIdx.x >> 3;
    const int wg = rest % a.G, k = lane8 + 8 * (rest / a.G);
    if (k >= a.dp.B) return;
    const int t = threadIdx.x, lane = t & 63, wave = __builtin_amdgcn_readfirstlane(t >> 6);
    const int c = k;
    if (stp() && k == 0 && wg == 0 && t == 0) { stp()[40] = (long long)wall_clock64(); stp()[49] = (long long)__builtin_readcyclecounter(); }
    unsigned *flag = a.words + (size_t)k * 64, *done = flag + 32;
    const int p0 = a.dp.poff[c], N = a.dp.poff[c + 1] - p0;
    const auto g_ppw = [&]() -> int { if constexpr (GF) return GC::ppw; else return a.ppw; };
    const auto g_pen_lds = [&]() -> int { if constexpr (GF) return GC::pen_lds; else return a.pen_lds; };
    const auto g_kmax = [&]() -> int { if constexpr (GF) return GC::kmax; else return a.Kmax; };
    const int ntasks = (N + g_ppw() - 1) / g_ppw();
    if (wg != 0 && ((wg - 1) * 4 >= ntasks || call.test_drop_members)) return;
    unsigned st0 = 0u;
    if constexpr (ET) { if (t == 0) st0 = __hip_atomic_load(a.status, FRX_RLX_AGENT); }
    else {
    if (__builtin_expect(__hip_atomic_load(a.status, FRX_RLX_AGENT) != 0u, 0)) {
        if (wg == 0 && threadIdx.x == 0) call.f[k] = __builtin_nan("");
        return;
    }
    }
    unsigned tag = __hip_atomic_load(done, FRX_RLX_AGENT) + 1u;
    if (tag >= (1u << 28)) tag = 1u;
    unsigned my_xcc = 0;
    asm volatile("s_getreg_b32 %0, hwreg(HW_REG_XCC_ID)" : "=s"(my_xcc));
    my_xcc = call.force_wt ? 0u : (my_xcc & 7u) + 1u;
    int nsteps = GC::nsteps;
    if constexpr (!GF) nsteps = a.nsteps;
    if constexpr (CH || GF) asm volatile("" : "+s"(nsteps));
    const EvalClusterLds L = eval_cluster_lds(a.maxN19, a.maxXb, a.maxVb, a.maxCN, nsteps, g_pen_lds());
    double *ctl = sm + L.ctl, *ev = sm + L.ev;
    const lds_vuptr verdict = (lds_vuptr)(unsigned *)sm;
    ResidentOps ro;
    ro.xs = sm + L.xs; ro.vs = sm + L.vs; ro.dsv = sm + L.xs; ro.pw = sm + L.pw; ro.gs = nullptr; ro.vskew = 0; ro.wq = sm + L.wq; ro.gpub = nullptr; ro.gwt = true;
    ro.quiet = wg != 0;
    const int task = (wg - 1) * 4 + wave;
    const bool has_task = wg != 0 && task < ntasks;
    const int gp0 = p0 + task * g_ppw(), npieces = has_task ? min(g_ppw(), N - task * g_ppw()) : 0;
    const int hstride = (g_kmax() + 1) * 4;
    double *wsm = sm + L.mem + (size_t)wave * g_pen_lds(), *hS = wsm, *red = wsm + (size_t)g_ppw() * hstride;
    double2 hv[4];
    const double2 *h2 = (const double2 *)(a.dp.hblk + (size_t)gp0 * hstride);
    const int nh2 = (npieces * hstride) >> 1;
    bool bad = false;
    double m_chi[4] = {0.0, 0.0, 0.0, 0.0}, m_invk = 0.0; int m_kappa = 0;
    gptr<ll_u64> m_llv = nullptr;
    if constexpr (GF) {
#pragma unroll
        for (int i = 0; i < 4; i++) m_chi[i] = a.dp.pc.chi[i];
        m_invk = a.dp.inv_kappa; m_kappa = a.dp.kappa;
        m_llv = (gptr<ll_u64>)(a.out20ll + (size_t)p0 * 40);
        asm volatile("" : "+v"(m_chi[0]), "+v"(m_chi[1]), "+v"(m_chi[2]), "+v"(m_chi[3]), "+v"(m_invk), "+v"(m_kappa), "+v"(m_llv));
    }
    if constexpr (ET) {
        if (k == 0 && wg == 1 && wave == 0 && lane == 0 && stp()) stp()[44] = (long long)wall_clock64();
        const auto early = [&]() -> bool {
            if (has_task) {
                if constexpr (GF) hv[0] = h2[lane < nh2 ? lane : nh2 - 1];
                else {
#pragma unroll
                for (int u = 0; u < 4; u++) { const int i = lane + 64 * u; hv[u] = h2[i < nh2 ? i : nh2 - 1]; }
                }
            }
            unsigned *w = (unsigned *)(ev + 24 * 64);
            if (t == 0) { w[0] = 0u; w[2] = 0u; w[3] = 0u; w[4] = 0u; w[5] = st0; *verdict = 0u; }
            asm volatile("s_waitcnt lgkmcnt(0)\n\ts_barrier" ::: "memory");
            bad = *(volatile unsigned *)(w + 5) != 0u;
            if (!bad && wg == 0 && t == 0) __hip_atomic_store(flag, (tag << 4) | (my_xcc ? my_xcc : 15u), FRX_RLX_AGENT);
            return bad;
        };
        const int wg_last = min(a.G - 1, (ntasks - 1) / 4 + 1);
        long long *est = nullptr;
        if (stp() && k == 0 && (wg == 0 || wg == wg_last)) est = stp() + (wg == 0 ? 50 : 60);
        const EvalEarlySync<decltype(early), CH> es{early, est, wg == 0};
        forward_knot_body<false, 64, 5, 0, true>(a.dp, call.x, a.T, a.C, a.maxCN, a.maxXb, a.maxVb, 64, nullptr, nsteps, c, ev, ctl, true, &ro, nullptr, nullptr, &es);
        if (bad) {
            if (wg == 0 && t == 0) call.f[k] = __builtin_nan("");
            return;
        }
        if constexpr (GF) {
            if (has_task && lane < nh2) { hS[2 * lane] = hv[0].x; hS[2 * lane + 1] = hv[0].y; }
        } else
        if (has_task) {
#pragma unroll
            for (int u = 0; u < 4; u++) { const int i = lane + 64 * u; if (i < nh2) { hS[2 * i] = hv[u].x; hS[2 * i + 1] = hv[u].y; } }
            for (int i0 = lane + 4 * 64; i0 < nh2; i0 += 4 * 64) {
                double2 v[4];
#pragma unroll
                for (int u = 0; u < 4; u++) { const int i = i0 + 64 * u; v[u] = h2[i < nh2 ? i : nh2 - 1]; }
#pragma unroll
                for (int u = 0; u < 4; u++) { const int i = i0 + 64 * u; if (i < nh2) { hS[2 * i] = v[u].x; hS[2 * i + 1] = v[u].y; } }
            }
        }
    } else {
    if (wg == 0) { if (t == 0) { *verdict = 0u; __hip_atomic_store(flag, (tag << 4) | (my_xcc ? my_xcc : 15u), FRX_RLX_AGENT); } }
    else if (has_task) {
        if (k == 0 && wg == 1 && wave == 0 && lane == 0 && stp()) stp()[44] = (long long)wall_clock64();
        for (int i0 = lane; i0 < nh2; i0 += 4 * 64) {
            double2 v[4];
#pragma unroll
            for (int u = 0; u < 4; u++) { const int i = i0 + 64 * u; v[u] = h2[i < nh2 ? i : nh2 - 1]; }
#pragma unroll
            for (int u = 0; u < 4; u++) { const int i = i0 + 64 * u; if (i < nh2) { hS[2 * i] = v[u].x; hS[2 * i + 1] = v[u].y; } }
        }
    }
    forward_knot_body<false, 64, 5>(a.dp, call.x, a.T, a.C, a.maxCN, a.maxXb, a.maxVb, 64, nullptr, nsteps, c, ev, ctl, true, &ro);
    }
    if (wg != 0) {
        if (!has_task) return;
        long long *const mst = (k == 0 && wg == 1 && wave == 0 && lane == 0) ? stp() : nullptr;
        if (mst) mst[46] = (long long)wall_clock64();
        int m_lpp = GC::lpp;
        if constexpr (!GF) m_lpp = a.lpp;
        int m_t0 = task * g_ppw(), m_N = N;
        ll_u64 *m_ll = nullptr;
        if constexpr (!GF) m_ll = a.out20ll + (size_t)p0 * 40;
        if constexpr (GF) {
            m_N = as_uniform(m_N);
            gptr<ll_u64> q_ll = as_uniform(m_llv);
            asm volatile("" : "+s"(m_N), "+s"(q_ll));
            m_ll = (ll_u64 *)q_ll;
        } else
        if constexpr (CH) {
            m_N = as_uniform(m_N);
            gptr<ll_u64> q_ll = (gptr<ll_u64>)as_uniform(m_ll);
            asm volatile("" : "+s"(m_lpp), "+s"(m_t0), "+s"(m_N), "+s"(q_ll));
            m_ll = (ll_u64 *)q_ll;
        }
        const int pl = lane / m_lpp, jl = lane - pl * m_lpp;
        if constexpr (GF) {
            DevProblem mdp = a.dp;
#pragma unroll
            for (int i = 0; i < 4; i++) mdp.pc.chi[i] = m_chi[i];
            mdp.inv_kappa = m_invk; mdp.kappa = m_kappa;
            if (pl < npieces) penalty_lane_samples<true>(mdp, ctl + (size_t)(m_t0 + pl) * 19, hS + (size_t)pl * hstride, ctl[(m_t0 + pl) * 19 + 18], jl, m_lpp, GC::kmax, red + lane * 21);
        } else
        if constexpr (CH) {
            DevProblem mdp = a.dp;
            asm volatile("" : "+s"(mdp.pc.chi[0]), "+s"(mdp.pc.chi[1]), "+s"(mdp.pc.chi[2]), "+s"(mdp.pc.chi[3]));
            if (pl < npieces) penalty_lane_samples<true>(mdp, ctl + (size_t)(m_t0 + pl) * 19, hS + (size_t)pl * hstride, ctl[(m_t0 + pl) * 19 + 18], jl, m_lpp, a.Kmax, red + lane * 21);
        } else
        if (pl < npieces) penalty_lane_samples<true>(a.dp, ctl + (size_t)(m_t0 + pl) * 19, hS + (size_t)pl * hstride, ctl[(m_t0 + pl) * 19 + 18], jl, m_lpp, a.Kmax, red + lane * 21);
        asm volatile("s_waitcnt lgkmcnt(0)" ::: "memory");
        if (mst) mst[47] = (long long)wall_clock64();
        const unsigned gv = __hip_atomic_load(flag, FRX_RLX_AGENT);
        if (mst) { asm volatile("" :: "v"(gv)); mst[69] = (long long)wall_clock64(); }
        const bool wt = my_xcc == 0u || (gv >> 4) != tag || (gv & 15u) != my_xcc;
        if constexpr (HO) penalty_reduce<true, true>(red, npieces, m_lpp, nullptr, lane, 64, wt, m_ll, tag, m_N, m_t0);
        else penalty_reduce<true>(red, npieces, m_lpp, nullptr, lane, 64, wt, a.out20ll + (size_t)gp0 * 40, tag);
        if (mst) mst[48] = (long long)wall_clock64();
        return;
    }
    if (stp() && k == 0 && t == 0) stp()[41] = (long long)wall_clock64();
    ro.o20ll = a.out20ll; ro.o20tag = tag; ro.status = a.status; ro.spin_ticks = call.timeout_ticks;
    const LineSearchTap tap{nullptr, nullptr, nullptr, nullptr, nullptr, 0u, nullptr, nullptr};
    EvalChain ch{0.0, 0.0, 0, 0, nullptr};
    double *t_f = call.f; unsigned *t_done = done, *t_sh = call.status_host;
    if constexpr (CH) {
        ch = EvalChain{a.dp.rho, a.dp.sumT, a.dp.soft, a.dp.c2, nullptr};
        gptr<double> q_g = (gptr<double>)call.g, q_f = (gptr<double>)t_f;
        gptr<unsigned> q_done = (gptr<unsigned>)t_done, q_sh = (gptr<unsigned>)t_sh;
        asm volatile("" : "+s"(ch.rho), "+s"(ch.sumT), "+s"(ch.soft), "+s"(ch.c2), "+s"(q_g), "+s"(q_f), "+s"(q_done), "+s"(q_sh));
        ch.g = (double *)q_g; t_f = (double *)q_f; t_done = (unsigned *)q_done; t_sh = (unsigned *)q_sh;
    }
    const EvalTail tl{verdict, t_f, t_done, tag, t_sh, k == 0 ? stp() : nullptr, TAIL};
    const EvalHandoff<HO, CH> ho{k == 0 ? stp() : nullptr, ch};
    backward_knot_body<true, 64, 0, EvalTail, EvalHandoff<HO, CH>>(a.dp, call.x, a.T, a.C, nullptr, call.f, call.g, a.maxCN, a.maxXb, a.maxVb, 64, nullptr, nsteps, tap, c, ev, ctl, &ro, &tl, &ho);
    if (stp() && k == 0 && t == 0) stp()[42] = (long long)wall_clock64();
    if constexpr (TAIL) {
        if (stp() && k == 0 && t == 0) stp()[43] = (long long)wall_clock64();
    } else {
    __syncthreads();
    if (t == 0) {
        const double fv = ev[36 * 64 + 9 * 65 + 2 * 64 + a.maxCN];
        const unsigned code = __hip_atomic_load(a.status, FRX_RLX_AGENT);
        const bool bad = code != 0u;
        if (tl.st) { asm volatile("" :: "v"(code)); tl.st[67] = (long long)wall_clock64(); }
        call.f[c] = bad ? __builtin_nan("") : fv;
        if (bad && call.status_host) __hip_atomic_store(call.status_host, code, FRX_RLX_SYS);
        __hip_atomic_store(done, tag, FRX_RLX_AGENT);
        if (tl.st) { const long long e = (long long)wall_clock64(); tl.st[68] = e; tl.st[43] = e; }
    }
    }
}

}
```

### fast-racing_amd/csrc/frx_kernels.hpp

```cpp
#pragma once
#include <hip/hip_runtime.h>
#include <type_traits>

#include "frx_device.hpp"
#include "frx_minco.hpp"
#include "frx_lbfgs.hpp"
#include "frx_wave.hpp"

#ifndef FRX_KERNEL_LINKAGE
#define FRX_KERNEL_LINKAGE
#endif

namespace frx {

struct LineSearchTap { const double *d; const int *flags; DvResult *res; unsigned *arrive; volatile unsigned *flag; unsigned round; double *lds_out = nullptr; const unsigned long long *early_cmd = nullptr; };



template <bool SH> __device__ __forceinline__ double ldg(const double *p) {
    if (SH) return __longlong_as_double((long long)__hip_atomic_load((const unsigned long long *)p, __ATOMIC_RELAXED, __HIP_MEMORY_SCOPE_AGENT));
    return *p;
}
template <bool SH> __device__ __forceinline__ void stg(double *p, double v, bool wt = true) {
    if (SH && wt) __hip_atomic_store((unsigned long long *)p, (unsigned long long)__double_as_longlong(v), __ATOMIC_RELAXED, __HIP_MEMORY_SCOPE_AGENT);
    else *p = v;
}

typedef unsigned long long ll_u64;
__device__ __forceinline__ void rk_ll_put(ll_u64 *slot, double v, unsigned tag, bool wt) {
    const ll_u64 b = (ll_u64)__double_as_longlong(v), tg = (ll_u64)tag << 32;
    const ll_u64 w0 = (b & 0xFFFFFFFFull) | tg, w1 = (b >> 32) | tg;
    if (wt) { __hip_atomic_store(slot, w0, __ATOMIC_RELAXED, __HIP_MEMORY_SCOPE_AGENT); __hip_atomic_store(slot + 1, w1, __ATOMIC_RELAXED, __HIP_MEMORY_SCOPE_AGENT); }
    else { slot[0] = w0; slot[1] = w1; }
}
__device__ __forceinline__ bool rk_ll_ok(ll_u64 w0, ll_u64 w1, unsigned tag) { return (unsigned)(w0 >> 32) == tag && (unsigned)(w1 >> 32) == tag; }
__device__ __forceinline__ double rk_ll_value(ll_u64 w0, ll_u64 w1) { return __longlong_as_double((long long)((w0 & 0xFFFFFFFFull) | (w1 << 32))); }

struct ResidentOps { double *xs, *vs, *dsv, *pw, *gs = nullptr; int vskew = 0; double *wq = nullptr; double *gpub = nullptr; bool gwt = true;
                     const ll_u64 *o20ll = nullptr; unsigned o20tag = 0; unsigned *status = nullptr; ll_u64 spin_ticks = 0;
                     bool quiet = false; };

struct KnotPre { int p0, N, c0, cN, x0, cv0, pc, piv, wnv, wvb, wxb; double bs[6]; };
struct GranuleOut { ll_u64 *ll; unsigned tag; unsigned *gate; unsigned gate_val; const unsigned *mxw; int nmx; };
struct EvalTail { volatile __attribute__((address_space(3))) unsigned *verdict; double *f; unsigned *done; unsigned tag; unsigned *status_host; long long *st; bool inl; };
struct EvalChain { double rho, sumT; int soft, c2; double *g; };
template <bool TR, bool CH = false> struct EvalHandoff { static constexpr bool tr = TR, chain = CH; long long *st; EvalChain ch; };
template <class HO> struct ho_transposed { static constexpr bool value = HO::tr; };
template <> struct ho_transposed<void> { static constexpr bool value = false; };
template <class HO> struct ho_chain { static constexpr bool value = HO::chain; };
template <> struct ho_chain<void> { static constexpr bool value = false; };
template <class ES> struct es_nostamps { static constexpr bool value = ES::nostamps; };
template <> struct es_nostamps<void> { static constexpr bool value = false; };
template <class T> using gptr = __attribute__((address_space(1))) T *;
template <class V> __device__ __forceinline__ V as_uniform(V v) {
    static_assert(sizeof(V) == 4 || sizeof(V) == 8, "a 4- or 8-byte value");
    int w[sizeof(V) / 4]; __builtin_memcpy(w, &v, sizeof(V));
    for (unsigned i = 0; i < sizeof(V) / 4; i++) w[i] = __builtin_amdgcn_readfirstlane(w[i]);
    __builtin_memcpy(&v, w, sizeof(V));
    return v;
}

template <int U> __device__ __forceinline__ void stage_to_lds(double *dst, const double *__restrict__ src, int n, int k, int nthr) {
    for (int i0 = k; i0 < n; i0 += U * nthr) {
        double tmp[U];
#pragma unroll
        for (int u = 0; u < U; u++) { const int i = i0 + u * nthr; tmp[u] = src[i < n ? i : n - 1]; }
#pragma unroll
        for (int u = 0; u < U; u++) { const int i = i0 + u * nthr; if (i < n) dst[i] = tmp[u]; }
    }
}

__device__ __forceinline__ double wave_sum(double v) {
#pragma unroll
    for (int o = 32; o > 0; o >>= 1) v += __shfl_xor(v, o, 64);
    return v;
}

#define BAND(i, j) band[(i) * FRX_BAND_W + ((j) - (i) + 6)]

FRX_KERNEL_LINKAGE __global__ __launch_bounds__(64) void k_forward(DevProblem dp, const double *__restrict__ x, double *__restrict__ Tout,
                                                double *__restrict__ Cout, double *__restrict__ bandOut, int maxN, int maxCN) {
    extern __shared__ double sm[];
    const int b = blockIdx.x, lane = threadIdx.x;
    const int p0 = dp.poff[b], N = dp.poff[b + 1] - p0, n6 = 6 * N;
    const int c0 = dp.coff[b], cN = dp.coff[b + 1] - c0;
    const int x0 = dp.xoff[b];
    double *band = sm;
    double *rhs = band + (size_t)6 * maxN * FRX_BAND_W;
    double *Tf = rhs + (size_t)6 * maxN * 3;
    double *Tc = Tf + maxN;

    if (dp.soft) {
        for (int i = lane; i < cN; i += 64) Tc[i] = tau_to_T(x[x0 + i], dp.c2 != 0);
    } else {
        if (lane == 0) {
            const int Ms1 = cN - 1;
            double sum = 0.0;
            for (int i = 0; i < Ms1; i++) { Tc[i] = tau_to_T(x[x0 + i], dp.c2 != 0); }
            Tc[Ms1] = 0.0;
            for (int i = 0; i <= Ms1; i++) sum += Tc[i];
            const double den = 1.0 + sum;
            for (int i = 0; i <= Ms1; i++) Tc[i] /= den;
            sum = 0.0;
            for (int i = 0; i <= Ms1; i++) sum += Tc[i];
            Tc[Ms1] = 1.0 - sum;
            for (int i = 0; i <= Ms1; i++) Tc[i] *= dp.sumT;
        }
    }
    for (int i = lane; i < n6 * FRX_BAND_W; i += 64) band[i] = 0.0;
    for (int i = lane; i < n6 * 3; i += 64) rhs[i] = 0.0;
    __syncthreads();
    for (int i = lane; i < N; i += 64) {
        const int gc = dp.piece_coarse[p0 + i];
        const double t = Tc[gc - c0] / dp.coarse_iv[gc];
        Tf[i] = t;
        Tout[p0 + i] = t;
    }
    __syncthreads();

    const int w0 = p0 - b;
    for (int i = lane; i < N - 1; i += 64) {
        const int gw = w0 + i;
        const int k = dp.wp_nv[gw] - 1;
        const double *V = dp.vrec + 3 * (size_t)dp.wp_vbeg[gw];
        const double *xi = x + dp.wp_xbeg[gw];
        double nrm = 0.0;
        for (int a = 0; a < k; a++) nrm += xi[a] * xi[a];
        const double sc = 2.0 / (1.0 + nrm);
        double q0 = 0.0, q1 = 0.0, q2 = 0.0;
        for (int a = 0; a < k; a++) {
            const double r = sc * xi[a], rr = r * r;
            q0 += V[3 * (a + 1)] * rr;
            q1 += V[3 * (a + 1) + 1] * rr;
            q2 += V[3 * (a + 1) + 2] * rr;
        }
        rhs[(6 * i + 5) * 3 + 0] = q0 + V[0];
        rhs[(6 * i + 5) * 3 + 1] = q1 + V[1];
        rhs[(6 * i + 5) * 3 + 2] = q2 + V[2];

        const double t1 = Tf[i], t2 = t1 * t1, t3 = t2 * t1, t4 = t2 * t2, t5 = t4 * t1;
        const int r = 6 * i;
        BAND(r + 3, r + 3) = 6.0;  BAND(r + 3, r + 4) = 24.0 * t1; BAND(r + 3, r + 5) = 60.0 * t2; BAND(r + 3, r + 9) = -6.0;
        BAND(r + 4, r + 4) = 24.0; BAND(r + 4, r + 5) = 120.0 * t1; BAND(r + 4, r + 10) = -24.0;
        BAND(r + 5, r) = 1.0; BAND(r + 5, r + 1) = t1; BAND(r + 5, r + 2) = t2; BAND(r + 5, r + 3) = t3; BAND(r + 5, r + 4) = t4; BAND(r + 5, r + 5) = t5;
        BAND(r + 6, r) = 1.0; BAND(r + 6, r + 1) = t1; BAND(r + 6, r + 2) = t2; BAND(r + 6, r + 3) = t3; BAND(r + 6, r + 4) = t4; BAND(r + 6, r + 5) = t5;
        BAND(r + 6, r + 6) = -1.0;
        BAND(r + 7, r + 1) = 1.0; BAND(r + 7, r + 2) = 2 * t1; BAND(r + 7, r + 3) = 3 * t2; BAND(r + 7, r + 4) = 4 * t3; BAND(r + 7, r + 5) = 5 * t4;
        BAND(r + 7, r + 7) = -1.0;
        BAND(r + 8, r + 2) = 2.0; BAND(r + 8, r + 3) = 6 * t1; BAND(r + 8, r + 4) = 12 * t2; BAND(r + 8, r + 5) = 20 * t3;
        BAND(r + 8, r + 8) = -2.0;
    }
    if (lane == 0) {
        BAND(0, 0) = 1.0; BAND(1, 1) = 1.0; BAND(2, 2) = 2.0;
        const double t1 = Tf[N - 1], t2 = t1 * t1, t3 = t2 * t1, t4 = t2 * t2, t5 = t4 * t1;
        BAND(n6 - 3, n6 - 6) = 1.0; BAND(n6 - 3, n6 - 5) = t1; BAND(n6 - 3, n6 - 4) = t2; BAND(n6 - 3, n6 - 3) = t3; BAND(n6 - 3, n6 - 2) = t4; BAND(n6 - 3, n6 - 1) = t5;
        BAND(n6 - 2, n6 - 5) = 1.0; BAND(n6 - 2, n6 - 4) = 2 * t1; BAND(n6 - 2, n6 - 3) = 3 * t2; BAND(n6 - 2, n6 - 2) = 4 * t3; BAND(n6 - 2, n6 - 1) = 5 * t4;
        BAND(n6 - 1, n6 - 4) = 2; BAND(n6 - 1, n6 - 3) = 6 * t1; BAND(n6 - 1, n6 - 2) = 12 * t2; BAND(n6 - 1, n6 - 1) = 20 * t3;
    }
    if (lane < 9) {
        rhs[lane] = dp.headPVA[b * 9 + lane];
        rhs[(n6 - 3) * 3 + lane] = dp.tailPVA[b * 9 + lane];
    }
    __syncthreads();

    {
        const int a = lane / 6, bb = lane % 6;
        for (int k = 0; k <= n6 - 2; k++) {
            const int i = k + 1 + a, j = k + 1 + bb;
            const bool act = lane < 36 && i < n6 && j < n6;
            double l = 0.0, u = 0.0, v = 0.0;
            if (act) {
                l = BAND(i, k);
                u = BAND(k, j);
                v = BAND(i, j);
                if (l != 0.0) l /= BAND(k, k);
            }
            __syncthreads();
            if (act) {
                if (bb == 0) BAND(i, k) = l;
                if (u != 0.0 && l != 0.0) BAND(i, j) = v - l * u;
            }
            __syncthreads();
        }
    }
    {
        const int a = lane / 3, c = lane % 3;
        for (int j = 0; j <= n6 - 1; j++) {
            const int i = j + 1 + a;
            if (lane < 18 && i < n6) {
                const double l = BAND(i, j);
                if (l != 0.0) rhs[i * 3 + c] -= l * rhs[j * 3 + c];
            }
            __syncthreads();
        }
        for (int j = n6 - 1; j >= 0; j--) {
            double xj = 0.0;
            if (lane < 18) xj = rhs[j * 3 + c] / BAND(j, j);
            __syncthreads();
            if (lane < 18) {
                if (a == 0) rhs[j * 3 + c] = xj;
                const int i = j - 1 - a;
                if (i >= 0) {
                    const double u = BAND(i, j);
                    if (u != 0.0) rhs[i * 3 + c] -= u * xj;
                }
// ... 773 lines not shown
            const int st = it - lag;
            if (st >= 0 && st < nst) {
#pragma unroll
                for (int h = 0; h < 2; h++) pcr_axis_step(rsb, nrow, lane + 64 * h, ax, N, 1 << st, st, pw, pws, r0[h], r1[h]);
            }
        }
        asm volatile("s_waitcnt lgkmcnt(0)\n\ts_barrier" ::: "memory");
    }
    if (wave >= 1) {
#pragma unroll
        for (int h = 0; h < 2; h++) {
            const int kk = lane + 64 * h;
            if (act[h]) {
                const double *Di = pw + kk * pws + nsteps * 8;
                KV[ax * (nrow + 1) + kk] = Di[0] * r0[h] + Di[1] * r1[h];
                KA[ax * (nrow + 1) + kk] = Di[2] * r0[h] + Di[3] * r1[h];
            }
        }
    }
}

typedef volatile __attribute__((address_space(3))) unsigned *lds_vuptr;
__device__ __forceinline__ void lds_wait_ge(lds_vuptr w, unsigned want) {
    for (unsigned spins = 0; *w < want && spins < (1u << 24); spins++) __builtin_amdgcn_s_sleep(1);
    asm volatile("" ::: "memory");
}
template <bool NOBAR = false>
__device__ __forceinline__ void pcr_matrix_wave64(double *rowbuf, int kk, int N, double hL, double hR, double *pw, int pws, double *save, size_t sstride,
                                                  size_t gk0, int nsteps, lds_vuptr progress, long long *est = nullptr) {
    const int nrow = 64;
    const bool act = kk >= 1 && kk <= N - 1;
    int nst = 0;
    for (int s = 1; s < N - 1; s <<= 1) nst++;
    double D[4], L[4], I[4];
    {
        KnotRow me;
        knot_row_matrix(hL, hR, me);
#pragma unroll
        for (int i = 0; i < 4; i++) { D[i] = me.D[i]; L[i] = kk == 1 ? 0.0 : me.L[i]; }
    }
    m2_inv_fast(D, I);
    if (kk == 0) {
#pragma unroll
        for (int buf = 0; buf < 2; buf++) {
            MR2(buf, 0, 0) = make_double2(1.0, 0.0); MR2(buf, 1, 0) = make_double2(0.0, 1.0);
            MR2(buf, 2, 0) = make_double2(0.0, 0.0); MR2(buf, 3, 0) = make_double2(0.0, 0.0);
        }
    } else if (act) {
        MR2(0, 0, kk) = make_double2(I[0], I[1]); MR2(0, 1, kk) = make_double2(I[2], I[3]);
        MR2(0, 2, kk) = make_double2(L[0], L[1]); MR2(0, 3, kk) = make_double2(L[2], L[3]);
    }
    double2 *sp = save ? (double2 *)(save + (gk0 + kk) * sstride) : nullptr;
    for (int it = 0; it < nst; it++) {
        const int s = 1 << it, buf = it & 1;
        const bool inlo = act && kk - s >= 1, inhi = act && kk + s <= N - 1;
        const int klo = inlo ? kk - s : 0, khi = inhi ? kk + s : 0;
        const double2 a0 = MR2(buf, 0, klo), a1 = MR2(buf, 1, klo), a2 = MR2(buf, 2, klo), a3 = MR2(buf, 3, klo);
        const double2 b0 = MR2(buf, 0, khi), b1 = MR2(buf, 1, khi), b2 = MR2(buf, 2, khi), b3 = MR2(buf, 3, khi);
        const double iLo[4] = {a0.x, a0.y, a1.x, a1.y}, lL[4] = {a2.x, a2.y, a3.x, a3.y};
        const double iHi[4] = {b0.x, b0.y, b1.x, b1.y}, hL[4] = {b2.x, b2.y, b3.x, b3.y};
        const double U[4] = {hL[0], hL[2], hL[1], hL[3]};
        const double Lt[4] = {L[0], L[2], L[1], L[3]};
        double al[4], be[4], tt[4];
        m2_mul(L, iLo, al);
        m2_mul(U, iHi, be);
        m2_mul(al, Lt, tt);
#pragma unroll
        for (int i = 0; i < 4; i++) D[i] = D[i] - tt[i];
        m2_mul(be, hL, tt);
#pragma unroll
        for (int i = 0; i < 4; i++) D[i] -= tt[i];
        m2_mul(al, lL, tt);
#pragma unroll
        for (int i = 0; i < 4; i++) L[i] = -tt[i];
        m2_inv_fast(D, I);
        if (act) {
            MR2(buf ^ 1, 0, kk) = make_double2(I[0], I[1]); MR2(buf ^ 1, 1, kk) = make_double2(I[2], I[3]);
            MR2(buf ^ 1, 2, kk) = make_double2(L[0], L[1]); MR2(buf ^ 1, 3, kk) = make_double2(L[2], L[3]);
#pragma unroll
            for (int i = 0; i < 4; i++) { pw[kk * pws + it * 8 + i] = al[i]; pw[kk * pws + it * 8 + 4 + i] = be[i]; }
            if (sp) {
                sp[it * 4 + 0] = make_double2(al[0], al[1]); sp[it * 4 + 1] = make_double2(al[2], al[3]);
                sp[it * 4 + 2] = make_double2(be[0], be[1]); sp[it * 4 + 3] = make_double2(be[2], be[3]);
            }
        }
        asm volatile("s_waitcnt lgkmcnt(0)" ::: "memory");
        if (kk == 0) *progress = (unsigned)(it + 1);
        if constexpr (NOBAR) { if (est && kk == 0) est[it] = (long long)wall_clock64(); }
        else if (it == (nst > 1 ? 1 : 0)) asm volatile("s_waitcnt lgkmcnt(0)\n\ts_barrier" ::: "memory");
    }
    if (act) {
#pragma unroll
        for (int i = 0; i < 4; i++) pw[kk * pws + nsteps * 8 + i] = I[i];
        if (sp) { sp[nsteps * 4] = make_double2(I[0], I[1]); sp[nsteps * 4 + 1] = make_double2(I[2], I[3]); }
    }
    asm volatile("s_waitcnt lgkmcnt(0)" ::: "memory");
    if (kk == 0) *progress = (unsigned)(nst + 1);
    if constexpr (NOBAR) { if (est && kk == 0) est[6] = (long long)wall_clock64(); }
    else if (nst == 0) asm volatile("s_waitcnt lgkmcnt(0)\n\ts_barrier" ::: "memory");
}
#undef MR2
#undef RS

template <bool SH, int NR = 0, int MODE = 0, int RB = 0, bool ET = false, class ES = void>
__device__ __forceinline__ void forward_knot_body(const DevProblem &dp, const double *__restrict__ x, double *__restrict__ Tout, double *__restrict__ Cout,
                               int maxCN, int maxXb, int maxVb, int nrow_rt, double *__restrict__ pcrw, int nsteps, int b, double *sm, double *ct_lds = nullptr, bool wt = true, const ResidentOps *ro = nullptr,
                               const KnotPre *pre = nullptr, const GranuleOut *go = nullptr, const ES *es = nullptr) {
    const int nrow = NR > 0 ? NR : nrow_rt;
    const int k = threadIdx.x, nthr = NR > 0 ? 256 : (int)blockDim.x;
    const int p0 = pre ? pre->p0 : dp.poff[b], N = pre ? pre->N : dp.poff[b + 1] - p0;
    const int c0 = pre ? pre->c0 : dp.coff[b], cN = pre ? pre->cN : dp.coff[b + 1] - c0;
    const int x0 = pre ? pre->x0 : dp.xoff[b];
    double *rowbuf = sm;
    static_assert(RB == 0 || (NR == 64 && RB >= 24 * 64 + 2), "a short row buffer: the <= 64-piece path only, progress words included");
    double *KP = rowbuf + (RB > 0 ? (size_t)RB : (size_t)36 * nrow);
    double *KV = KP + 3 * (nrow + 1);
    double *KA = KV + 3 * (nrow + 1);
    double *Tf = KA + 3 * (nrow + 1);
    double *Tc = Tf + nrow;
    double *xs = Tc + maxCN;
    double *vs = xs + maxXb;
    double *pwf = vs + maxVb;
    if (ro) { xs = ro->xs; vs = ro->vs; if (nrow == 64 && nthr == 256) pwf = ro->pw; }
#define KN(arr, axis, idx) arr[(axis) * (nrow + 1) + (idx)]
#define FWD_STAMP(slot) do { if constexpr (!es_nostamps<ES>::value) { if (!(ro && ro->quiet)) FRX_STAMP(slot); } } while (0)
#define FWD_STAMP_AX(slot) do { if constexpr (!es_nostamps<ES>::value) { if (!(ro && ro->quiet)) FRX_STAMP_AX(slot); } } while (0)
    FWD_STAMP(0);
    int r_pc = 0, r_piv = 1, r_wnv = 1, r_wvb = 0, r_wxb = 0;
    const int cv0 = pre ? pre->cv0 : __builtin_amdgcn_readfirstlane(dp.cvoff[b]);
    double r_bs[6] = {0, 0, 0, 0, 0, 0};
    if (pre) { r_pc = pre->pc; r_piv = pre->piv; }
    else if (k < N) { r_pc = dp.piece_coarse[p0 + k]; r_piv = dp.piece_iv[p0 + k]; }
    const bool wsp64 = nrow == 64 && nthr == 256;
    const int t2 = k - 64;
    const int wq = wsp64 ? (t2 >= 0 ? (t2 >> 1) : N) : (k >> 2);
    if (pre) { r_wnv = pre->wnv; r_wvb = pre->wvb; r_wxb = pre->wxb; }
    else if (wq < N - 1) { const int gw = p0 - b + wq; r_wnv = dp.wp_nv[gw]; r_wvb = dp.wp_vbeg[gw]; r_wxb = dp.wp_xbeg[gw]; }
    const int kbs = wsp64 ? t2 : k;
    if (pre) { r_bs[0] = pre->bs[0]; r_bs[1] = pre->bs[1]; r_bs[2] = pre->bs[2]; r_bs[3] = pre->bs[3]; r_bs[4] = pre->bs[4]; r_bs[5] = pre->bs[5]; }
    else if (kbs >= 0 && kbs < 3) {
#pragma unroll
        for (int q = 0; q < 3; q++) { r_bs[q] = dp.headPVA[b * 9 + 3 * q + kbs]; r_bs[3 + q] = dp.tailPVA[b * 9 + 3 * q + kbs]; }
    }
    lds_vuptr progress = (lds_vuptr)(unsigned *)(rowbuf + (size_t)24 * nrow);
    unsigned *const arrive = (unsigned *)(rowbuf + (size_t)24 * nrow);
    if (!ET && wsp64 && k == 0) *progress = 0u;
    double hMine = 1.0;
    long long *est = nullptr;
    bool est_steps = false;
    if constexpr (ET) { est = es->st; est_steps = es->steps; }
    if constexpr (ET) {
        static_assert(NR == 64 && (MODE & 1), "early durations: the wave-specialised <= 64-piece path of a caller that stages");
        const int wave = __builtin_amdgcn_readfirstlane(k >> 6), kk = k & 63;
        const int nT = dp.soft ? cN : cN - 1;
        const int nx = dp.xoff[b + 1] - x0;
        const int v0 = dp.cvoff[b], nvd = 3 * (dp.cvoff[b + 1] - v0);
        const double *vsrc = dp.vrec + 3 * (size_t)v0;
        constexpr int UX = 4, UV = 16, NA = 192;
        double tau = 0.0, sx[UX], sv[UV];
        if (wave == 0) {
            if (kk < nT) tau = x[x0 + kk];
        } else {
#pragma unroll
            for (int u = 0; u < UX; u++) { const int i = nT + t2 + u * NA; sx[u] = nx > 0 ? x[x0 + (i < nx ? i : nx - 1)] : 0.0; }
#pragma unroll
            for (int u = 0; u < UV; u++) { const int i = t2 + u * NA; sv[u] = nvd > 0 ? vsrc[i < nvd ? i : nvd - 1] : 0.0; }
        }
        if (es->sync()) return;
        if (wave == 0) {
            if (kk < nT) xs[kk] = tau;
            if (dp.soft) {
                if (kk < cN) Tc[kk] = tau_to_T(tau, dp.c2 != 0);
            } else if (kk == 0) {
                const int Ms1 = cN - 1;
                double sum = 0.0;
                for (int i = 0; i < Ms1; i++) Tc[i] = tau_to_T(xs[i], dp.c2 != 0);
                Tc[Ms1] = 0.0;
                for (int i = 0; i <= Ms1; i++) sum += Tc[i];
                const double den = 1.0 + sum;
                for (int i = 0; i <= Ms1; i++) Tc[i] /= den;
                sum = 0.0;
                for (int i = 0; i <= Ms1; i++) sum += Tc[i];
                Tc[Ms1] = 1.0 - sum;
                for (int i = 0; i <= Ms1; i++) Tc[i] *= dp.sumT;
            }
            if (kk < N) {
                hMine = Tc[r_pc - c0] / r_piv;
                Tf[kk] = hMine;
                ct_lds[kk * 19 + 18] = hMine;
            }
            asm volatile("s_waitcnt lgkmcnt(0)" ::: "memory");
            if (kk == 0) { progress[4] = 1u; if (est) est[0] = (long long)wall_clock64(); }
        } else {
#pragma unroll
            for (int u = 0; u < UX; u++) { const int i = nT + t2 + u * NA; if (i < nx) xs[i] = sx[u]; }
#pragma unroll
            for (int u = 0; u < UV; u++) { const int i = t2 + u * NA; if (i < nvd) vs[i] = sv[u]; }
            stage_to_lds<4>(xs, x + x0, nx, nT + t2 + UX * NA, NA);
            stage_to_lds<8>(vs, vsrc, nvd, t2 + UV * NA, NA);
            asm volatile("s_waitcnt lgkmcnt(0)" ::: "memory");
            if (kk == 0) __hip_atomic_fetch_add(arrive + 2, 1u, __ATOMIC_RELAXED, __HIP_MEMORY_SCOPE_WORKGROUP);
            lds_wait_ge(progress + 2, 3u);
            if (est && k == 64) est[1] = (long long)wall_clock64();
        }
    } else {
    {
        if (!ro || (MODE & 1)) {
            const int nx = dp.xoff[b + 1] - x0;
            const int v0 = dp.cvoff[b], nvd = 3 * (dp.cvoff[b + 1] - v0);
            const double *vsrc = dp.vrec + 3 * (size_t)v0;
            stage_to_lds<4>(xs, x + x0, nx, k, nthr);
            stage_to_lds<8>(vs, vsrc, nvd, k, nthr);
        }
    }
    __syncthreads();
    FWD_STAMP(1);
    }
    if constexpr (!ET) {
    if (dp.soft) {
        for (int i = k; i < cN; i += nthr) Tc[i] = tau_to_T(xs[i], dp.c2 != 0);
    } else if (k == 0) {
        const int Ms1 = cN - 1;
        double sum = 0.0;
        for (int i = 0; i < Ms1; i++) Tc[i] = tau_to_T(xs[i], dp.c2 != 0);
        Tc[Ms1] = 0.0;
        for (int i = 0; i <= Ms1; i++) sum += Tc[i];
        const double den = 1.0 + sum;
        for (int i = 0; i <= Ms1; i++) Tc[i] /= den;
        sum = 0.0;
        for (int i = 0; i <= Ms1; i++) sum += Tc[i];
        Tc[Ms1] = 1.0 - sum;
        for (int i = 0; i <= Ms1; i++) Tc[i] *= dp.sumT;
    }
    __syncthreads();
    if (k < N) {
        hMine = Tc[r_pc - c0] / r_piv;
        Tf[k] = hMine;
        if ((MODE & 2) && SH && go && go->ll) rk_ll_put(go->ll + 2 * ((size_t)(p0 + k) * 19 + 18), hMine, go->tag, go->mxw ? true : wt);
        else if (!(MODE & 4)) stg<SH>(Tout + p0 + k, hMine, wt);
        if (ct_lds) ct_lds[k * 19 + 18] = hMine;
    }
    }
    FWD_STAMP(2);
    if (wsp64) {
        const int wave = __builtin_amdgcn_readfirstlane(k >> 6), kk = k & 63;
        const int pws = nsteps * 8 + 5;
        double *cstage = ct_lds ? ct_lds : rowbuf;
        if (wave == 0) {
            const double hLs = lane_up1(hMine);
            const bool act0 = kk >= 1 && kk <= N - 1;
            pcr_matrix_wave64<ET>(rowbuf, kk, N, act0 ? hLs : 1.0, act0 ? hMine : 1.0, pwf, pws, ro ? nullptr : pcrw, (size_t)(nsteps * 8 + 4), (size_t)p0, nsteps, progress,
                                  (est && est_steps) ? est + 3 : nullptr);
            if (est && !est_steps && kk == 0) est[3] = (long long)wall_clock64();
            FWD_STAMP(5);
        } else {
            const int ax = wave - 1;
            for (int w0 = 0; w0 < N - 1; w0 += 96) {
                const int w = w0 + (t2 >> 1), sub = t2 & 1;
                double nrm = 0.0, q0 = 0.0, q1 = 0.0, q2 = 0.0;
                const bool wact = w < N - 1;
                const double *V = vs, *xi = xs;
                if (wact) {
                    int wnv = r_wnv, wvb = r_wvb, wxb = r_wxb;
                    if (w0 > 0) { const int gw = p0 - b + w; wnv = dp.wp_nv[gw]; wvb = dp.wp_vbeg[gw]; wxb = dp.wp_xbeg[gw]; }
                    const int nv1 = wnv - 1;
                    V = vs + 3 * (wvb - cv0) + (ro ? ro->vskew * w : 0);
                    xi = xs + (wxb - x0);
                    for (int a0 = sub; a0 < nv1; a0 += 8) {
                        double xv[4], v0[4], v1[4], v2[4];
#pragma unroll
                        for (int j = 0; j < 4; j++) { const int a = min(a0 + 2 * j, nv1 - 1); xv[j] = xi[a]; v0[j] = V[3 * (a + 1)]; v1[j] = V[3 * (a + 1) + 1]; v2[j] = V[3 * (a + 1) + 2]; }
#pragma unroll
                        for (int j = 0; j < 4; j++)
                            if (a0 + 2 * j < nv1) { const double x2 = xv[j] * xv[j]; nrm += x2; q0 += v0[j] * x2; q1 += v1[j] * x2; q2 += v2[j] * x2; }
                    }
                }
                nrm += dpp_mov<0xB1>(nrm); q0 += dpp_mov<0xB1>(q0); q1 += dpp_mov<0xB1>(q1); q2 += dpp_mov<0xB1>(q2);
                if (wact && sub == 0) {
                    if (ro && ro->wq) { double *wq = ro->wq + 4 * w; wq[0] = nrm; wq[1] = q0; wq[2] = q1; wq[3] = q2; }
                    else if (dp.wq_glob) { double2 *wq = (double2 *)(dp.wq_glob + 4 * (size_t)(p0 - b + w)); wq[0] = make_double2(nrm, q0); wq[1] = make_double2(q1, q2); }
                    const double sc = 2.0 / (1.0 + nrm), sc2 = sc * sc;
                    KN(KP, 0, w + 1) = sc2 * q0 + V[0]; KN(KP, 1, w + 1) = sc2 * q1 + V[1]; KN(KP, 2, w + 1) = sc2 * q2 + V[2];
                }
            }
            if (t2 < 3) {
                KN(KP, t2, 0) = r_bs[0]; KN(KV, t2, 0) = r_bs[1]; KN(KA, t2, 0) = r_bs[2];
                KN(KP, t2, N) = r_bs[3]; KN(KV, t2, N) = r_bs[4]; KN(KA, t2, N) = r_bs[5];
            }
            FWD_STAMP_AX(8);
            if constexpr (ET) {
                asm volatile("s_waitcnt lgkmcnt(0)" ::: "memory");
                if (kk == 0) __hip_atomic_fetch_add(arrive + 3, 1u, __ATOMIC_RELAXED, __HIP_MEMORY_SCOPE_WORKGROUP);
                lds_wait_ge(progress + 3, 3u);
                lds_wait_ge(progress + 4, 1u);
                if (est && k == 64) est[2] = (long long)wall_clock64();
            } else
            asm volatile("s_waitcnt lgkmcnt(0)\n\ts_barrier" ::: "memory");
            FWD_STAMP_AX(9);
            const bool act = kk >= 1 && kk <= N - 1;
            const int kc = act ? kk : 1;
            double r0 = 0.0, r1 = 0.0;
            if (act) {
                const double hL = Tf[kk - 1], hR = Tf[kk];
                knot_row_rhs(hL, hR, KN(KP, ax, kk) - KN(KP, ax, kk - 1), KN(KP, ax, kk + 1) - KN(KP, ax, kk), r0, r1);
                if (kk == 1 || kk == N - 1) {
                    KnotRow m0;
                    knot_row_matrix(hL, hR, m0);
                    if (kk == 1) {
                        r0 -= m0.L[0] * KN(KV, ax, 0) + m0.L[1] * KN(KA, ax, 0);
                        r1 -= m0.L[2] * KN(KV, ax, 0) + m0.L[3] * KN(KA, ax, 0);
                    }
                    if (kk == N - 1) {
                        r0 -= m0.U[0] * KN(KV, ax, N) + m0.U[1] * KN(KA, ax, N);
                        r1 -= m0.U[2] * KN(KV, ax, N) + m0.U[3] * KN(KA, ax, N);
                    }
                }
            }
            FWD_STAMP_AX(10);
            if ((MODE & 2) && SH && go && go->ll && go->mxw && wave == 3) {
                unsigned vq = go->gate_val;
                if (kk < go->nmx) vq = __hip_atomic_load(go->mxw + kk, __ATOMIC_RELAXED, __HIP_MEMORY_SCOPE_AGENT);
                const bool all_here = __builtin_amdgcn_ballot_w64(vq != go->gate_val) == 0ull;
                if (kk == 0) progress[1] = all_here ? 1u : 0u;
            }
            int nst = 0;
            for (int s = 1; s < N - 1; s <<= 1) nst++;
            for (int st = 0; st < nst; st++) {
                lds_wait_ge(progress, (unsigned)(st + 1));
                const int s = 1 << st;
// ... 1271 lines not shown
```

### fast-racing_amd/csrc/frx_launch_forms.hpp

```cpp
#pragma once
#include <cstddef>
#include <map>
#include <utility>

namespace frx {

constexpr int pen_wave_doubles(int ppw, int Kmax) { return ppw * 19 + ppw * (Kmax + 1) * 4 + 64 * 21; }
constexpr size_t pen_wg_bytes(int ppg, int Kmax, int waves, int doubles_per_lane) {
    return sizeof(double) * ((size_t)ppg * 19 + (size_t)ppg * (Kmax + 1) * 4 + (size_t)64 * waves * doubles_per_lane);
}

class LdsLimits {
    std::map<std::pair<int, const void *>, size_t> held_;
public:
    template <class Set> int raise(int dev, const void *fn, size_t bytes, Set &&set) {
        if (!bytes) return 0;
        size_t &held = held_[{dev, fn}];
        if (bytes <= held) return 0;
        const int e = set(fn, bytes);
        if (!e) held = bytes;
        return e;
    }
};

struct EvalClusterForm { bool argp, et, tail, ho, ch, geo; };
inline bool operator==(const EvalClusterForm &a, const EvalClusterForm &b) {
    return a.argp == b.argp && a.et == b.et && a.tail == b.tail && a.ho == b.ho && a.ch == b.ch && a.geo == b.geo;
}
struct EvalSwitches {
    bool argptr, early_t, tail, handoff, chain, geom;
    constexpr bool handoff_on() const { return handoff && argptr && tail; }
    constexpr bool chain_on() const { return chain && handoff_on(); }
    constexpr bool geom_on() const { return geom && handoff_on() && early_t; }
};
inline bool eval_cluster_form(const EvalSwitches &s, bool geom_class, bool stamped, bool have_dev_args, EvalClusterForm &f) {
    const bool chained = s.chain_on() && !stamped;
    if (s.geom_on() && geom_class) f = {true, true, true, true, chained, true};
    else if (s.handoff_on()) f = {true, s.early_t, true, true, chained, false};
    else if (s.argptr) f = {true, s.early_t, !(s.early_t && !s.tail), false, false, false};
    else f = {false, s.early_t, true, false, false, false};
    return !f.argp || have_dev_args;
}
inline int eval_cluster_raised_forms(const EvalSwitches &s, EvalClusterForm out[4]) {
    int n = 0;
    for (int geom_class = 0; geom_class <= (s.geom_on() ? 1 : 0); geom_class++)
        for (int stamped = 0; stamped <= (s.chain_on() ? 1 : 0); stamped++) (void)eval_cluster_form(s, geom_class, stamped, true, out[n++]);
    return n;
}

enum PenaltyForm { PEN_THR, PEN_LAT, PEN_LAT2_17, PEN_LAT2_49, PEN_LAT2_0, PEN_LAT2_R5 };
constexpr PenaltyForm penalty_lat2_form(int lpp) { return lpp == 17 ? PEN_LAT2_17 : lpp == 49 ? PEN_LAT2_49 : PEN_LAT2_0; }
constexpr PenaltyForm penalty_form(bool lds_pen2, int lpp, int forced, char twophase_char) {
    return forced == 2 ? PEN_THR : !lds_pen2 || twophase_char == '0' ? PEN_LAT : twophase_char == '5' ? PEN_LAT2_R5 : penalty_lat2_form(lpp);
}
constexpr int penalty_form_code(PenaltyForm f) { return f == PEN_THR ? 0 : f == PEN_LAT ? 1 : 2; }

enum EvalRoute { EVAL_CLUSTER, EVAL_SOLO, EVAL_STAGES };
constexpr EvalRoute eval_route(bool backward, bool tap, bool cand_active, bool stamps, bool eval_fused, bool eval_fused_stamps, int eval_solo, int B, int solo_min_B,
                               int solo_max_B, bool lds_solo, bool knot_solver) {
    const bool solo_ok = backward && lds_solo && knot_solver && (!stamps || eval_solo == 2);
    return solo_ok && eval_solo == 2 ? EVAL_SOLO
         : backward && eval_fused && knot_solver && !tap && !cand_active && (!stamps || eval_fused_stamps) ? EVAL_CLUSTER
         : solo_ok && eval_solo == 1 && B >= solo_min_B && B <= solo_max_B ? EVAL_SOLO : EVAL_STAGES;
}

}
```

### include/frx_debug.h

```cpp
#ifndef FRX_DEBUG_H
#define FRX_DEBUG_H

#include "frx.h"

#ifdef __cplusplus
extern "C" {
#endif

int frx_debug_trace(const frx_problem *p, double *out, int cap_rows);
int frx_resident_profile(const frx_problem *p, unsigned long long *out, int cap_words);

int frx_debug_direction_log(frx_problem *p, int cap_steps, int n_cands);
int frx_debug_direction_log_read(const frx_problem *p, int cand, double *out, int cap_rows, int *rows, int *row_doubles);
int frx_debug_set_resident_retry(frx_problem *p, int enable);
int frx_debug_resident_counts(const frx_problem *p, int *failed, int *retried);
int frx_debug_resident_clusters(const frx_problem *p, int *clusters);
int frx_debug_resident_predictions(const frx_problem *p, unsigned long long *out3);

int frx_eval_stage_times(frx_problem *p, const double *x, int reps, double *out3_us);
int frx_debug_set_eval_fused(frx_problem *p, int enable);
int frx_debug_eval_fused(const frx_problem *p);
int frx_debug_eval_geometry(const frx_problem *p);
int frx_debug_set_eval_solo(frx_problem *p, int mode);
int frx_debug_penalty_kernel(const frx_problem *p);
int frx_debug_eval_solo(const frx_problem *p);
int frx_eval_launch_time(frx_problem *p, const double *x, int reps, double *out_us);
int frx_debug_profile_eval_cluster(frx_problem *p, const double *x, long long *out64);
int frx_debug_profile_eval_tail(frx_problem *p, const double *x, long long *out80);

int frx_profile_phases(frx_problem *p, const double *x, long long *out32);

int frx_dv_selftest(int device, int n, int B, int m, int iters, const int *geom4, unsigned seed, double *max_rel_err,
                    double *avg_us);

int frx_debug_dv_layout(int n_max, const int *geom4, int tight, int *out5);
int frx_debug_dv_round(int device, int B, int m, const int *geom4, int hs, const long long *lens7, const int *xoff, double *x, double *g, double *xp, double *gp,
                       double *d, double *S, double *Y, double *ys, double *gt, const void *cmd, void *res, const int *poff, int *dflags, int *pflags,
                       const double *f);

int frx_jps_tables(int *ns3, int *f13, int *f23, int *ns2, int *f12, int *f22);

int frx_debug_host_cpu_share(int clusters, int extra_plans, double *budget, int *share, int *mailbox_threads);

int frx_debug_taken_over(const frx_problem *p, int *candidates);
int frx_debug_set_takeover_at(frx_problem *p, long rounds);
int frx_debug_compact_from_history(int m, int n, int hs, int bound, int newest, const double *S, const double *Y, double *rinv129, double *yy, double *vd);

int frx_debug_set_clear_chunk(frx_problem *p, int points);

int frx_debug_fold_rows(int kind, int B, const int *piece_off, const double *T, const double *rows, const double *limits, double *cand_out, unsigned *flags);

int frx_debug_map_blocked_device(int device, const frx_voxel_map *map, int n_pairs, const double *a, const double *b, int *out);

int frx_debug_shader_clock(int device, double ms, double *mhz_min, double *mhz_mean, double *mhz_max);
int frx_debug_mailbox_numa(const frx_problem *p, int *out4);

#ifdef __cplusplus
}
#endif
#endif
```

Baseline: 2.699 billion samples/s.

## Precompute per-candidate front records and pack leading kernel args into cache lines

Adds a 64-byte per-candidate EvalFront record (piece/knot/variable offsets, counts, task count) that is built on the host and uploaded once. The fused evaluation kernel loads this record plus a packed 192-byte argument lead, instead of chasing several offset arrays and a large DevProblem struct at kernel start. The kernel also prefetches the duration variables and piece metadata into registers before the early sync. The goal is to shorten the dependent global-load chain at the front of each evaluation launch. In exchange it adds more template instantiations and more argument-struct complexity, and the old path stays available through FRX_EVAL_FRONT.

```diff
diff --git a/fast-racing_amd/__init__.py b/fast-racing_amd/__init__.py
--- a/fast-racing_amd/__init__.py
+++ b/fast-racing_amd/__init__.py
@@ -66,7 +66,7 @@
 DEBUG_SYMBOLS = [
     "frx_debug_trace", "frx_resident_profile", "frx_debug_direction_log", "frx_debug_direction_log_read", "frx_debug_set_resident_retry",
     "frx_debug_resident_counts", "frx_debug_resident_clusters", "frx_debug_resident_predictions", "frx_eval_stage_times", "frx_profile_phases", "frx_dv_selftest", "frx_jps_tables", "frx_debug_host_cpu_share", "frx_debug_taken_over", "frx_debug_compact_from_history",
-    "frx_debug_set_eval_fused", "frx_debug_eval_fused", "frx_debug_eval_geometry", "frx_debug_set_eval_solo", "frx_debug_eval_solo", "frx_debug_penalty_kernel", "frx_debug_mailbox_numa", "frx_eval_launch_time", "frx_debug_profile_eval_cluster", "frx_debug_profile_eval_tail", "frx_debug_set_takeover_at", "frx_debug_shader_clock",
+    "frx_debug_set_eval_fused", "frx_debug_eval_fused", "frx_debug_eval_geometry", "frx_debug_eval_front", "frx_debug_set_eval_solo", "frx_debug_eval_solo", "frx_debug_penalty_kernel", "frx_debug_mailbox_numa", "frx_eval_launch_time", "frx_debug_profile_eval_cluster", "frx_debug_profile_eval_tail", "frx_debug_set_takeover_at", "frx_debug_shader_clock",
     "frx_debug_set_clear_chunk", "frx_debug_map_blocked_device", "frx_debug_dv_layout", "frx_debug_dv_round", "frx_debug_fold_rows",
 ]
 
@@ -129,6 +129,7 @@
         L.frx_debug_set_eval_fused.argtypes = [C.c_void_p, C.c_int]
         L.frx_debug_eval_fused.argtypes = [C.c_void_p]
         L.frx_debug_eval_geometry.argtypes = [C.c_void_p]
+        L.frx_debug_eval_front.argtypes = [C.c_void_p]
         L.frx_debug_set_eval_solo.argtypes = [C.c_void_p, C.c_int]
         L.frx_debug_eval_solo.argtypes = [C.c_void_p]
         L.frx_debug_penalty_kernel.argtypes = [C.c_void_p]
@@ -820,6 +821,9 @@
     def eval_geometry(self) -> int:
         return int(lib().frx_debug_eval_geometry(self.h))
 
+    def eval_front(self) -> int:
+        return int(lib().frx_debug_eval_front(self.h))
+
     def set_eval_solo(self, mode: int):
         _check(lib().frx_debug_set_eval_solo(self.h, int(mode)))
 
diff --git a/fast-racing_amd/csrc/frx_api.cpp b/fast-racing_amd/csrc/frx_api.cpp
--- a/fast-racing_amd/csrc/frx_api.cpp
+++ b/fast-racing_amd/csrc/frx_api.cpp
@@ -27,6 +27,7 @@
 #include "../../include/frx_debug.h"
 #include "frx_device.hpp"
 #include "frx_launch_forms.hpp"
+#include "frx_eval_front.hpp"
 #include "frx_internal.hpp"
 #include "frx_lbfgs.hpp"
 #include "frx_host_pool.hpp"
@@ -246,6 +247,7 @@
     int eval_fused = 0, eval_fused_G = 0, eval_fused_stamps = 0;
     unsigned long long eval_fused_ticks = 25000000ull;
     std::vector<unsigned char> ev_args, ev_args_st;
+    DevBuf<frx::EvalFront> d_ev_front;
     DevBuf<unsigned char> d_ev_args, d_ev_args_st;
     PinBuf<unsigned> h_ev_status;
     unsigned eval_fused_code = 0;
@@ -506,6 +508,9 @@
         p->d_ev_words = (unsigned *)(p->d_ev_ll.p + n_ll);
         { NumaScope numa_alloc(device); CR(p->h_ev_status.alloc(16)); }
         p->ev_args.assign(frx::eval_cluster_args_bytes(), 0); CR(p->d_ev_args.alloc(p->ev_args.size()));
+        std::vector<frx::EvalFront> front((size_t)B);
+        frx::eval_front_fill(B, p->poff.data(), p->coff.data(), p->xoff.data(), cvoff.data(), p->softT, p->geo.ppw, front.data());
+        CR(p->d_ev_front.upload(front));
     }
     {
         NumaScope numa_alloc(device);
@@ -533,7 +538,7 @@
     d.wp_vbeg = p->d_wp_vbeg.p; d.wp_nv = p->d_wp_nv.p; d.wp_xbeg = p->d_wp_xbeg.p;
     d.hblk = p->d_hblk.p; d.vrec = p->d_vrec.p; d.wq_glob = p->d_wq.p; d.stamps = nullptr; d.cand_active = nullptr; d.piece_active = nullptr;
     if (p->eval_fused_G) {
-        frx::eval_cluster_args(p->dp, p->geo, p->d_T.p, p->d_C.p, p->d_ev_ll.p, p->d_ev_words, p->ev_args.data());
+        frx::eval_cluster_args(p->dp, p->geo, p->d_T.p, p->d_C.p, p->d_ev_ll.p, p->d_ev_words, p->d_ev_front.p, p->ev_args.data());
         const hipError_t e_ = hipMemcpy(p->d_ev_args.p, p->ev_args.data(), p->ev_args.size(), hipMemcpyHostToDevice);
         if (e_ != hipSuccess) { const std::string m_ = std::string("upload of the evaluation arguments: ") + hipGetErrorString(e_); (void)hipStreamDestroy(p->stream); delete p; return fail(FRX_ERR_HIP, m_); }
     }
@@ -626,7 +631,7 @@
     p->dp.stamps = p->d_stamps.p; p->eval_fused_stamps = 1;
     {
         p->ev_args_st.assign(frx::eval_cluster_args_bytes(), 0);
-        frx::eval_cluster_args(p->dp, p->geo, p->d_T.p, p->d_C.p, p->d_ev_ll.p, p->d_ev_words, p->ev_args_st.data());
+        frx::eval_cluster_args(p->dp, p->geo, p->d_T.p, p->d_C.p, p->d_ev_ll.p, p->d_ev_words, p->d_ev_front.p, p->ev_args_st.data());
         hipError_t e_ = p->d_ev_args_st.p ? hipSuccess : p->d_ev_args_st.alloc(p->ev_args_st.size());
         if (e_ == hipSuccess) e_ = hipMemcpy(p->d_ev_args_st.p, p->ev_args_st.data(), p->ev_args_st.size(), hipMemcpyHostToDevice);
         if (e_ != hipSuccess) { p->dp.stamps = nullptr; p->eval_fused_stamps = 0; return fail(FRX_ERR_HIP, hipGetErrorString(e_)); }
@@ -838,6 +843,7 @@
 }
 int frx_debug_eval_fused(const frx_problem *p) { return (p && p->eval_fused) ? p->eval_fused_G : 0; }
 int frx_debug_eval_geometry(const frx_problem *p) { return (p && p->eval_fused) ? frx::eval_cluster_class(p->geo) : 0; }
+int frx_debug_eval_front(const frx_problem *p) { return (p && p->eval_fused) ? frx::eval_cluster_front(p->geo) : 0; }
 int frx_debug_set_eval_solo(frx_problem *p, int mode) {
     if (!p || mode < 0 || mode > 2) return fail(FRX_ERR_INVALID_ARG, "null argument or unknown mode");
     if (mode == 2 && !p->geo.lds_solo) return fail(FRX_ERR_INVALID_ARG, "the solo form does not apply to this handle (more than 64 pieces or samples per piece, or the banded solver)");
diff --git a/fast-racing_amd/csrc/frx_device.hpp b/fast-racing_amd/csrc/frx_device.hpp
--- a/fast-racing_amd/csrc/frx_device.hpp
+++ b/fast-racing_amd/csrc/frx_device.hpp
@@ -64,7 +64,8 @@
 int eval_cluster_class(const LaunchGeom &g);
 int eval_cluster_geometry(LaunchGeom &g);
 size_t eval_cluster_args_bytes();
-void eval_cluster_args(const DevProblem &dp, const LaunchGeom &g, double *T, double *C, unsigned long long *ll, unsigned *words, void *out);
+void eval_cluster_args(const DevProblem &dp, const LaunchGeom &g, double *T, double *C, unsigned long long *ll, unsigned *words, const void *front_dev, void *out);
+int eval_cluster_front(const LaunchGeom &g);
 int launch_eval_cluster(const LaunchGeom &g, int B, const void *args_host, const void *args_dev, const double *x, double *f, double *grad,
                         unsigned long long timeout_ticks, void *stream, unsigned *status_host = nullptr);
 int eval_cluster_blocks_per_cu(size_t lds_bytes);
diff --git a/fast-racing_amd/csrc/frx_device_eval.hip b/fast-racing_amd/csrc/frx_device_eval.hip
--- a/fast-racing_amd/csrc/frx_device_eval.hip
+++ b/fast-racing_amd/csrc/frx_device_eval.hip
@@ -14,16 +14,22 @@
 namespace frx {
 
 static const EvalSwitches &eval_switches() {
-    static const EvalSwitches s{!env_off("FRX_EVAL_ARGPTR"), !env_off("FRX_EVAL_EARLY_T"), !env_off("FRX_EVAL_TAIL"), !env_off("FRX_EVAL_HANDOFF"), !env_off("FRX_EVAL_CHAIN"), !env_off("FRX_EVAL_GEOM")};
+    static const EvalSwitches s{!env_off("FRX_EVAL_ARGPTR"), !env_off("FRX_EVAL_EARLY_T"), !env_off("FRX_EVAL_TAIL"), !env_off("FRX_EVAL_HANDOFF"), !env_off("FRX_EVAL_CHAIN"), !env_off("FRX_EVAL_GEOM"),
+                                env_off("FRX_EVAL_FRONT")};
     return s;
 }
 typedef eval_geom<EvalGeomK16> GeomK16;
 static_assert(GeomK16::pen_lds == pen_wave_doubles(GeomK16::ppw, GeomK16::kmax), "the class's per-wave LDS is pen_wave_doubles of its integers");
 static bool eval_geom_class(const LaunchGeom &g) { return g.ev_G && g.lpp == GeomK16::lpp && g.ppw == GeomK16::ppw && g.Kmax == GeomK16::kmax && g.pcr_steps == GeomK16::nsteps; }
 int eval_cluster_class(const LaunchGeom &g) { return (eval_switches().geom_on() && eval_geom_class(g)) ? 1 : 0; }
+int eval_cluster_front(const LaunchGeom &g) {
+    EvalClusterForm m;
+    if (!g.ev_G || !eval_cluster_form(eval_switches(), eval_geom_class(g), false, true, m)) return 0;
+    return (m.argp && m.et && !m.old_front) ? 1 : 0;
+}
 
-template <bool ARGP, bool ET, bool TAIL = true, bool HO = false, bool CH = false, class GEO = void> struct eval_inst {
-    static constexpr EvalClusterForm form() { return {ARGP, ET, TAIL, HO, CH, !std::is_void<GEO>::value}; }
+template <bool ARGP, bool ET, bool TAIL = true, bool HO = false, bool CH = false, class GEO = void, bool FR = false> struct eval_inst {
+    static constexpr EvalClusterForm form() { return {ARGP, ET, TAIL, HO, CH, !std::is_void<GEO>::value, ARGP && ET && !FR}; }
 };
 template <class F> static int with_eval_kernel(const EvalClusterForm &m, F &&f) {
 #define FRX_EVAL_FORM(...) if (m == eval_inst<__VA_ARGS__>::form()) return f(k_eval_cluster<__VA_ARGS__>);
@@ -38,6 +44,12 @@
     FRX_EVAL_FORM(false, false)
     FRX_EVAL_FORM(true, true, true, true, true, EvalGeomK16)
     FRX_EVAL_FORM(true, true, true, true, false, EvalGeomK16)
+    FRX_EVAL_FORM(true, true, true, true, true, EvalGeomK16, true)
+    FRX_EVAL_FORM(true, true, true, true, false, EvalGeomK16, true)
+    FRX_EVAL_FORM(true, true, true, true, true, void, true)
+    FRX_EVAL_FORM(true, true, true, true, false, void, true)
+    FRX_EVAL_FORM(true, true, false, false, false, void, true)
+    FRX_EVAL_FORM(true, true, true, false, false, void, true)
 #undef FRX_EVAL_FORM
     return (int)hipErrorInvalidValue;
 }
@@ -70,12 +82,19 @@
     return n;
 }
 size_t eval_cluster_args_bytes() { return sizeof(EvalClusterArgs); }
-void eval_cluster_args(const DevProblem &dp, const LaunchGeom &g, double *T, double *C, unsigned long long *ll, unsigned *words, void *out) {
+void eval_cluster_args(const DevProblem &dp, const LaunchGeom &g, double *T, double *C, unsigned long long *ll, unsigned *words, const void *front_dev, void *out) {
     EvalClusterArgs a;
     std::memset(&a, 0, sizeof(a));
     assert(!eval_switches().handoff_on() || (reinterpret_cast<uintptr_t>(ll) & 15u) == 0);
     a.dp = dp; a.T = T; a.C = C; a.out20ll = ll; a.words = words; a.status = words + (size_t)64 * dp.B;
     a.G = g.ev_G; a.maxCN = g.maxCN; a.maxXb = g.maxXb; a.maxVb = g.maxVb; a.nsteps = g.pcr_steps; a.lpp = g.lpp; a.ppw = g.ppw; a.Kmax = g.Kmax; a.pen_lds = pen_wave_doubles(g.ppw, g.Kmax); a.maxN19 = g.maxN * 19;
+    a.front = (const EvalFront *)front_dev;
+    EvalArgsLead &l = a.lead;
+    l.piece_coarse = dp.piece_coarse; l.piece_iv = dp.piece_iv; l.wp_nv = dp.wp_nv; l.wp_vbeg = dp.wp_vbeg; l.wp_xbeg = dp.wp_xbeg;
+    l.vrec = dp.vrec; l.hblk = dp.hblk; l.headPVA = dp.headPVA; l.tailPVA = dp.tailPVA; l.status = a.status; l.words = a.words;
+    l.maxN19 = a.maxN19; l.maxXb = a.maxXb; l.maxVb = a.maxVb; l.maxCN = a.maxCN; l.nsteps = a.nsteps; l.pen_lds = a.pen_lds; l.ppw = a.ppw; l.Kmax = a.Kmax; l.soft = dp.soft; l.c2 = dp.c2;
+    for (int q = 0; q < 4; q++) l.chi[q] = dp.pc.chi[q];
+    l.inv_kappa = dp.inv_kappa; l.out20ll = a.out20ll; l.kappa = dp.kappa;
     std::memcpy(out, &a, sizeof(a));
 }
 int launch_eval_cluster(const LaunchGeom &g, int B, const void *args_host, const void *args_dev, const double *x, double *f, double *grad,
@@ -84,6 +103,7 @@
     EvalCallArgs c;
     c.x = x; c.f = f; c.g = grad; c.status_host = status_host; c.timeout_ticks = timeout_ticks;
     c.force_wt = env_is("FRX_EVAL_FUSED_WT", '1') ? 1 : 0;
+    c.G = (unsigned short)g.ev_G; c.B = (unsigned short)B;
     c.test_drop_members = timeout_ticks == 1ull ? 1 : 0;
     if (c.test_drop_members) c.timeout_ticks = 5000ull;
     const dim3 grid(8 * g.ev_G * ((B + 7) / 8));
@@ -91,9 +111,12 @@
     EvalClusterForm m;
     if (!eval_cluster_form(eval_switches(), eval_geom_class(g), host->dp.stamps != nullptr, args_dev != nullptr, m)) return (int)hipErrorInvalidValue;
     assert(!m.geo || (host->pen_lds == GeomK16::pen_lds && host->nsteps == GeomK16::nsteps));
+    if (m.argp && m.et && !m.old_front) {
+        if (!host->front || g.ev_G > 0xFFFF || B > 0xFFFF) return (int)hipErrorInvalidValue;
+    }
     return with_eval_kernel(m, [&](auto kernel) {
-        if constexpr (std::is_same<decltype(kernel), void (*)(EvalClusterArgs, EvalCallArgs)>::value) hipLaunchKernelGGL(kernel, grid, dim3(256), g.lds_ev, (hipStream_t)stream, *host, c);
-        else hipLaunchKernelGGL(kernel, grid, dim3(256), g.lds_ev, (hipStream_t)stream, (const EvalClusterArgs *)args_dev, c);
+        if constexpr (std::is_same<decltype(kernel), void (*)(EvalClusterArgs, EvalCallArgs, const EvalFront *)>::value) hipLaunchKernelGGL(kernel, grid, dim3(256), g.lds_ev, (hipStream_t)stream, *host, c, host->front);
+        else hipLaunchKernelGGL(kernel, grid, dim3(256), g.lds_ev, (hipStream_t)stream, (const EvalClusterArgs *)args_dev, c, host->front);
         return (int)hipGetLastError();
     });
 }
diff --git a/fast-racing_amd/csrc/frx_eval_front.hpp b/fast-racing_amd/csrc/frx_eval_front.hpp
--- /dev/null
+++ b/fast-racing_amd/csrc/frx_eval_front.hpp
@@ -0,0 +1,32 @@
+#pragma once
+#include <cstddef>
+
+namespace frx {
+
+struct alignas(64) EvalFront {
+    int p0, N;
+    int c0, cN;
+    int x0, nx;
+    int nT;
+    int cv0, nvd;
+    int wbase;
+    int ntasks;
+    int pad[5];
+};
+static_assert(sizeof(EvalFront) == 64 && alignof(EvalFront) == 64, "one record, one line");
+
+inline void eval_front_fill(int B, const int *poff, const int *coff, const int *xoff, const int *cvoff, bool soft, int ppw, EvalFront *out) {
+    for (int b = 0; b < B; b++) {
+        EvalFront r = {};
+        r.p0 = poff[b]; r.N = poff[b + 1] - poff[b];
+        r.c0 = coff[b]; r.cN = coff[b + 1] - coff[b];
+        r.x0 = xoff[b]; r.nx = xoff[b + 1] - xoff[b];
+        r.nT = soft ? r.cN : r.cN - 1;
+        r.cv0 = cvoff[b]; r.nvd = 3 * (cvoff[b + 1] - cvoff[b]);
+        r.wbase = r.p0 - b;
+        r.ntasks = (r.N + ppw - 1) / ppw;
+        out[b] = r;
+    }
+}
+
+}
diff --git a/fast-racing_amd/csrc/frx_eval_kernel.hpp b/fast-racing_amd/csrc/frx_eval_kernel.hpp
--- a/fast-racing_amd/csrc/frx_eval_kernel.hpp
+++ b/fast-racing_amd/csrc/frx_eval_kernel.hpp
@@ -1,18 +1,31 @@
 #pragma once
 #include <type_traits>
 
+#include "frx_eval_front.hpp"
 #include "frx_round_kernel.hpp"
 
 namespace frx {
 
+struct EvalArgsLead {
+    const int *piece_coarse, *piece_iv, *wp_nv, *wp_vbeg, *wp_xbeg;
+    const double *vrec, *hblk, *headPVA, *tailPVA;
+    unsigned *status, *words;
+    int maxN19, maxXb, maxVb, maxCN, nsteps, pen_lds, ppw, Kmax, soft, c2;
+    double chi[4], inv_kappa; ll_u64 *out20ll; int kappa, pad[3];
+};
+static_assert(sizeof(EvalArgsLead) == 192 && offsetof(EvalArgsLead, chi) == 128, "three 64-byte lines");
+
 struct EvalClusterArgs {
+    EvalArgsLead lead;
     DevProblem dp;
     double *T, *C;
     ll_u64 *out20ll;
     unsigned *words;
     unsigned *status;
     int G, maxCN, maxXb, maxVb, nsteps, lpp, ppw, Kmax, pen_lds, maxN19;
-};
+    const EvalFront *front;
+};
+static_assert(offsetof(EvalClusterArgs, lead) == 0, "the leading lines lead");
 
 struct EvalClusterLds { int ctl, xs, vs, pw, wq, ev, mem, total; };
 __host__ __device__ inline EvalClusterLds eval_cluster_lds(int maxN19, int maxXb, int maxVb, int maxCN, int nsteps, int pen_lds) {
@@ -35,12 +48,17 @@
     const double *x; double *f, *g;
     unsigned *status_host;
     rk_u64 timeout_ticks;
-    int test_drop_members;
-    int force_wt;
-};
-template <class F, bool NS = false> struct EvalEarlySync {
+    unsigned short G, B;
+    unsigned char test_drop_members;
+    unsigned char force_wt;
+};
+static_assert(sizeof(EvalCallArgs) + 2 * sizeof(void *) <= 64, "argument pointer, call arguments and the records' pointer: one 64-byte line of the kernarg segment");
+template <class F, bool NS = false, bool FRN = false> struct EvalEarlySync {
     static constexpr bool nostamps = NS;
+    static constexpr bool front_held = FRN;
     const F &f; long long *st; bool steps;
+    long long *front;
+    int nT, nx, nvd, soft, c2; gptr<const double> vsrc; double tau;
     __device__ __forceinline__ bool sync() const { return f(); }
 };
 struct EvalGeomK16 { static constexpr int LPP = 17, PPW = 3, KMAX = 8, NSTEPS = 6; };
@@ -51,29 +69,59 @@
     static_assert(ppw * lpp <= 64 && ppw * hstride <= 2 * 64, "a wave-task: one lane per sample, one double2 of its corridor blocks per lane");
 };
 template <> struct eval_geom<void> { static constexpr bool fixed = false; static constexpr int lpp = 0, ppw = 0, kmax = 0, nsteps = 0, hstride = 0, pen_lds = 0; };
-template <bool ARGP, bool ET, bool TAIL = true, bool HO = false, bool CH = false, class GEO = void>
-__global__ __launch_bounds__(256, 1) void k_eval_cluster(typename std::conditional<ARGP, const EvalClusterArgs *__restrict__, EvalClusterArgs>::type arg, EvalCallArgs call) {
+template <bool ARGP, bool ET, bool TAIL = true, bool HO = false, bool CH = false, class GEO = void, bool FR = false>
+__global__ __launch_bounds__(256, 1) void k_eval_cluster(typename std::conditional<ARGP, const EvalClusterArgs *__restrict__, EvalClusterArgs>::type arg, EvalCallArgs call,
+                                                         const EvalFront *__restrict__ front) {
     static_assert(!CH || (ARGP && TAIL && HO), "the production form: argument pointer, inline tail, value-major hand-off");
     typedef eval_geom<GEO> GC;
     constexpr bool GF = GC::fixed;
     static_assert(!GF || (ARGP && ET && TAIL && HO), "the geometry class: the default form of every other switch");
+    static_assert(!FR || (ARGP && ET), "the two-trip front: the argument pointer and early durations");
     const EvalClusterArgs &a = [&]() -> const EvalClusterArgs & { if constexpr (ARGP) return *arg; else return arg; }();
     const auto stp = [&]() -> long long * { if constexpr (CH) return nullptr; else return a.dp.stamps; };
     extern __shared__ __attribute__((aligned(16))) double sm[];
+    long long fr_entry = 0, fr_entry_cyc = 0;
+    if constexpr (FR && !CH) { fr_entry = (long long)wall_clock64(); fr_entry_cyc = (long long)__builtin_readcyclecounter(); }
     const int lane8 = blockIdx.x & 7, rest = blockIdx.x >> 3;
-    const int wg = rest % a.G, k = lane8 + 8 * (rest / a.G);
-    if (k >= a.dp.B) return;
+    const int nG = [&]() -> int { if constexpr (FR) return call.G; else return a.G; }();
+    const int wg = rest % nG, k = lane8 + 8 * (rest / nG);
+    if (k >= [&]() -> int { if constexpr (FR) return call.B; else return a.dp.B; }()) return;
     const int t = threadIdx.x, lane = t & 63, wave = __builtin_amdgcn_readfirstlane(t >> 6);
     const int c = k;
+    EvalFront fr = {};
+    EvalArgsLead ld = {};
+    gptr<const int> l_pc = nullptr, l_piv = nullptr, l_wnv = nullptr, l_wvb = nullptr, l_wxb = nullptr;
+    gptr<const double> l_vrec = nullptr, l_hblk = nullptr, l_head = nullptr, l_tail = nullptr;
+    gptr<unsigned> l_status = nullptr, l_words = nullptr;
+    if constexpr (FR) {
+        fr = front[k]; ld = a.lead;
+        l_pc = (gptr<const int>)ld.piece_coarse; l_piv = (gptr<const int>)ld.piece_iv; l_wnv = (gptr<const int>)ld.wp_nv; l_wvb = (gptr<const int>)ld.wp_vbeg; l_wxb = (gptr<const int>)ld.wp_xbeg;
+        l_vrec = (gptr<const double>)ld.vrec; l_hblk = (gptr<const double>)ld.hblk; l_head = (gptr<const double>)ld.headPVA; l_tail = (gptr<const double>)ld.tailPVA;
+        l_status = (gptr<unsigned>)ld.status; l_words = (gptr<unsigned>)ld.words;
+#define FRX_FRONT_PINS "+s"(fr.p0), "+s"(fr.N), "+s"(fr.c0), "+s"(fr.cN), "+s"(fr.x0), "+s"(fr.nx), "+s"(fr.nT), "+s"(fr.cv0), "+s"(fr.nvd), "+s"(fr.wbase), "+s"(fr.ntasks), \
+                        "+s"(l_pc), "+s"(l_piv), "+s"(l_wnv), "+s"(l_wvb), "+s"(l_wxb), "+s"(l_vrec), "+s"(l_hblk), "+s"(l_head), "+s"(l_tail), "+s"(l_status), "+s"(l_words), \
+                        "+s"(ld.maxN19), "+s"(ld.maxXb), "+s"(ld.maxVb), "+s"(ld.maxCN), "+s"(ld.soft), "+s"(ld.c2)
+        if constexpr (GF) asm volatile("" : FRX_FRONT_PINS, "+s"(ld.chi[0]), "+s"(ld.chi[1]), "+s"(ld.chi[2]), "+s"(ld.chi[3]), "+s"(ld.inv_kappa), "+s"(ld.kappa));
+        else asm volatile("" : FRX_FRONT_PINS, "+s"(ld.nsteps), "+s"(ld.pen_lds), "+s"(ld.ppw), "+s"(ld.Kmax));
+#undef FRX_FRONT_PINS
+    }
+    if constexpr (FR) { if (stp() && k == 0 && wg == 0 && t == 0) { stp()[40] = fr_entry; stp()[49] = fr_entry_cyc; } }
+    else
     if (stp() && k == 0 && wg == 0 && t == 0) { stp()[40] = (long long)wall_clock64(); stp()[49] = (long long)__builtin_readcyclecounter(); }
-    unsigned *flag = a.words + (size_t)k * 64, *done = flag + 32;
-    const int p0 = a.dp.poff[c], N = a.dp.poff[c + 1] - p0;
+    unsigned *flag = FR ? (unsigned *)l_words + (size_t)k * 64 : a.words + (size_t)k * 64, *done = flag + 32;
+    const int p0 = [&]() -> int { if constexpr (FR) return fr.p0; else return a.dp.poff[c]; }();
+    const int N = [&]() -> int { if constexpr (FR) return fr.N; else return a.dp.poff[c + 1] - p0; }();
     const auto g_ppw = [&]() -> int { if constexpr (GF) return GC::ppw; else return a.ppw; };
     const auto g_pen_lds = [&]() -> int { if constexpr (GF) return GC::pen_lds; else return a.pen_lds; };
     const auto g_kmax = [&]() -> int { if constexpr (GF) return GC::kmax; else return a.Kmax; };
-    const int ntasks = (N + g_ppw() - 1) / g_ppw();
+    const auto f_ppw = [&]() -> int { if constexpr (GF) return GC::ppw; else if constexpr (FR) return ld.ppw; else return a.ppw; };
+    const auto f_pen_lds = [&]() -> int { if constexpr (GF) return GC::pen_lds; else if constexpr (FR) return ld.pen_lds; else return a.pen_lds; };
+    const auto f_kmax = [&]() -> int { if constexpr (GF) return GC::kmax; else if constexpr (FR) return ld.Kmax; else return a.Kmax; };
+    const int ntasks = [&]() -> int { if constexpr (FR) return fr.ntasks; else return (N + g_ppw() - 1) / g_ppw(); }();
     if (wg != 0 && ((wg - 1) * 4 >= ntasks || call.test_drop_members)) return;
     unsigned st0 = 0u;
+    if constexpr (FR) { if (t == 0) st0 = __hip_atomic_load(l_status, FRX_RLX_AGENT); }
+    else
     if constexpr (ET) { if (t == 0) st0 = __hip_atomic_load(a.status, FRX_RLX_AGENT); }
     else {
     if (__builtin_expect(__hip_atomic_load(a.status, FRX_RLX_AGENT) != 0u, 0)) {
@@ -81,15 +129,19 @@
         return;
     }
     }
-    unsigned tag = __hip_atomic_load(done, FRX_RLX_AGENT) + 1u;
+    unsigned tag = 0u, tag_v = 0u;
+    if constexpr (FR) { int tag_at = 0; asm volatile("" : "+v"(tag_at)); tag_v = __hip_atomic_load(done + tag_at, FRX_RLX_AGENT); }
+    else {
+    tag = __hip_atomic_load(done, FRX_RLX_AGENT) + 1u;
     if (tag >= (1u << 28)) tag = 1u;
+    }
     unsigned my_xcc = 0;
     asm volatile("s_getreg_b32 %0, hwreg(HW_REG_XCC_ID)" : "=s"(my_xcc));
     my_xcc = call.force_wt ? 0u : (my_xcc & 7u) + 1u;
     int nsteps = GC::nsteps;
-    if constexpr (!GF) nsteps = a.nsteps;
+    if constexpr (!GF) { if constexpr (FR) nsteps = ld.nsteps; else nsteps = a.nsteps; }
     if constexpr (CH || GF) asm volatile("" : "+s"(nsteps));
-    const EvalClusterLds L = eval_cluster_lds(a.maxN19, a.maxXb, a.maxVb, a.maxCN, nsteps, g_pen_lds());
+    const EvalClusterLds L = FR ? eval_cluster_lds(ld.maxN19, ld.maxXb, ld.maxVb, ld.maxCN, nsteps, f_pen_lds()) : eval_cluster_lds(a.maxN19, a.maxXb, a.maxVb, a.maxCN, nsteps, g_pen_lds());
     double *ctl = sm + L.ctl, *ev = sm + L.ev;
     const lds_vuptr verdict = (lds_vuptr)(unsigned *)sm;
     ResidentOps ro;
@@ -97,20 +149,20 @@
     ro.quiet = wg != 0;
     const int task = (wg - 1) * 4 + wave;
     const bool has_task = wg != 0 && task < ntasks;
-    const int gp0 = p0 + task * g_ppw(), npieces = has_task ? min(g_ppw(), N - task * g_ppw()) : 0;
-    const int hstride = (g_kmax() + 1) * 4;
-    double *wsm = sm + L.mem + (size_t)wave * g_pen_lds(), *hS = wsm, *red = wsm + (size_t)g_ppw() * hstride;
+    const int gp0 = p0 + task * f_ppw(), npieces = has_task ? min(f_ppw(), N - task * f_ppw()) : 0;
+    const int hstride = (f_kmax() + 1) * 4;
+    double *wsm = sm + L.mem + (size_t)wave * f_pen_lds(), *hS = wsm, *red = wsm + (size_t)f_ppw() * hstride;
     double2 hv[4];
-    const double2 *h2 = (const double2 *)(a.dp.hblk + (size_t)gp0 * hstride);
+    const double2 *h2 = (const double2 *)((FR ? (const double *)l_hblk : a.dp.hblk) + (size_t)gp0 * hstride);
     const int nh2 = (npieces * hstride) >> 1;
     bool bad = false;
     double m_chi[4] = {0.0, 0.0, 0.0, 0.0}, m_invk = 0.0; int m_kappa = 0;
     gptr<ll_u64> m_llv = nullptr;
     if constexpr (GF) {
 #pragma unroll
-        for (int i = 0; i < 4; i++) m_chi[i] = a.dp.pc.chi[i];
-        m_invk = a.dp.inv_kappa; m_kappa = a.dp.kappa;
-        m_llv = (gptr<ll_u64>)(a.out20ll + (size_t)p0 * 40);
+        for (int i = 0; i < 4; i++) m_chi[i] = FR ? ld.chi[i] : a.dp.pc.chi[i];
+        m_invk = FR ? ld.inv_kappa : a.dp.inv_kappa; m_kappa = FR ? ld.kappa : a.dp.kappa;
+        m_llv = (gptr<ll_u64>)((FR ? ld.out20ll : a.out20ll) + (size_t)p0 * 40);
         asm volatile("" : "+v"(m_chi[0]), "+v"(m_chi[1]), "+v"(m_chi[2]), "+v"(m_chi[3]), "+v"(m_invk), "+v"(m_kappa), "+v"(m_llv));
     }
     if constexpr (ET) {
@@ -126,15 +178,52 @@
             unsigned *w = (unsigned *)(ev + 24 * 64);
             if (t == 0) { w[0] = 0u; w[2] = 0u; w[3] = 0u; w[4] = 0u; w[5] = st0; *verdict = 0u; }
             asm volatile("s_waitcnt lgkmcnt(0)\n\ts_barrier" ::: "memory");
-            bad = *(volatile unsigned *)(w + 5) != 0u;
+            if constexpr (FR) {
+                bad = ((lds_vuptr)w)[5] != 0u;
+                if (!bad && wg == 0 && t == 0) {
+                    unsigned tv = tag_v;
+                    asm volatile("" : "+v"(tv));
+                    tag = tv + 1u;
+                    if (tag >= (1u << 28)) tag = 1u;
+                }
+            }
+            else bad = *(volatile unsigned *)(w + 5) != 0u;
             if (!bad && wg == 0 && t == 0) __hip_atomic_store(flag, (tag << 4) | (my_xcc ? my_xcc : 15u), FRX_RLX_AGENT);
             return bad;
         };
-        const int wg_last = min(a.G - 1, (ntasks - 1) / 4 + 1);
+        const int wg_last = min(nG - 1, (ntasks - 1) / 4 + 1);
         long long *est = nullptr;
         if (stp() && k == 0 && (wg == 0 || wg == wg_last)) est = stp() + (wg == 0 ? 50 : 60);
-        const EvalEarlySync<decltype(early), CH> es{early, est, wg == 0};
+        long long *const fst = (stp() && k == 0 && wg == 0) ? stp() + 32 : nullptr;
+        if constexpr (FR) {
+            const int t2 = t - 64;
+            double tau = 0.0, r_bs[6] = {0.0, 0.0, 0.0, 0.0, 0.0, 0.0};
+            asm volatile("" : "+v"(tau));
+            int r_pc = 0, r_piv = 1, r_wnv = 1, r_wvb = 0, r_wxb = 0;
+            long long f_iss = 0;
+            if (wave == 0) {
+                if (fst) { asm volatile("" :: "v"(call.x + fr.x0 + lane), "v"(fr.nT)); f_iss = (long long)wall_clock64(); }
+                if (lane < fr.nT) tau = call.x[fr.x0 + lane];
+            }
+            if (t < fr.N) { r_pc = l_pc[fr.p0 + t]; r_piv = l_piv[fr.p0 + t]; }
+            const int wq = t2 >= 0 ? (t2 >> 1) : fr.N;
+            if (wq < fr.N - 1) { const int gw = fr.wbase + wq; r_wnv = l_wnv[gw]; r_wvb = l_wvb[gw]; r_wxb = l_wxb[gw]; }
+            if (t2 >= 0 && t2 < 3) {
+                const gptr<const double> hd = l_head + c * 9, tl = l_tail + c * 9;
+#pragma unroll
+                for (int q = 0; q < 3; q++) { r_bs[q] = hd[3 * q + t2]; r_bs[3 + q] = tl[3 * q + t2]; }
+            }
+            if (wave == 0 && fst) { asm volatile("" :: "v"(tau)); const long long f_in = (long long)wall_clock64(); if (lane == 0) { fst[0] = f_iss; fst[1] = f_in; } }
+            const KnotPre kpre{fr.p0, fr.N, fr.c0, fr.cN, fr.x0, fr.cv0, r_pc, r_piv, r_wnv, r_wvb, r_wxb, {r_bs[0], r_bs[1], r_bs[2], r_bs[3], r_bs[4], r_bs[5]}};
+            const EvalEarlySync<decltype(early), CH, true> es{early, est, wg == 0, nullptr, fr.nT, fr.nx, fr.nvd, ld.soft, ld.c2, l_vrec + 3 * (size_t)fr.cv0, tau};
+            forward_knot_body<false, 64, 5, 0, true>(a.dp, call.x, a.T, a.C, ld.maxCN, ld.maxXb, ld.maxVb, 64, nullptr, nsteps, c, ev, ctl, true, &ro, &kpre, nullptr, &es);
+            asm volatile("" : "+v"(tag_v));
+            tag = tag_v + 1u;
+            if (tag >= (1u << 28)) tag = 1u;
+        } else {
+        const EvalEarlySync<decltype(early), CH> es{early, est, wg == 0, fst, 0, 0, 0, 0, 0, nullptr, 0.0};
         forward_knot_body<false, 64, 5, 0, true>(a.dp, call.x, a.T, a.C, a.maxCN, a.maxXb, a.maxVb, 64, nullptr, nsteps, c, ev, ctl, true, &ro, nullptr, nullptr, &es);
+        }
         if (bad) {
             if (wg == 0 && t == 0) call.f[k] = __builtin_nan("");
             return;
diff --git a/fast-racing_amd/csrc/frx_kernels.hpp b/fast-racing_amd/csrc/frx_kernels.hpp
--- a/fast-racing_amd/csrc/frx_kernels.hpp
+++ b/fast-racing_amd/csrc/frx_kernels.hpp
@@ -51,6 +51,8 @@
 template <> struct ho_chain<void> { static constexpr bool value = false; };
 template <class ES> struct es_nostamps { static constexpr bool value = ES::nostamps; };
 template <> struct es_nostamps<void> { static constexpr bool value = false; };
+template <class ES> struct es_front { static constexpr bool value = ES::front_held; };
+template <> struct es_front<void> { static constexpr bool value = false; };
 template <class T> using gptr = __attribute__((address_space(1))) T *;
 template <class V> __device__ __forceinline__ V as_uniform(V v) {
     static_assert(sizeof(V) == 4 || sizeof(V) == 8, "a 4- or 8-byte value");
@@ -1130,14 +1132,21 @@
     if constexpr (ET) {
         static_assert(NR == 64 && (MODE & 1), "early durations: the wave-specialised <= 64-piece path of a caller that stages");
         const int wave = __builtin_amdgcn_readfirstlane(k >> 6), kk = k & 63;
-        const int nT = dp.soft ? cN : cN - 1;
-        const int nx = dp.xoff[b + 1] - x0;
-        const int v0 = dp.cvoff[b], nvd = 3 * (dp.cvoff[b + 1] - v0);
-        const double *vsrc = dp.vrec + 3 * (size_t)v0;
+        constexpr bool FH = es_front<ES>::value;
+        const int nT = [&]() -> int { if constexpr (FH) return es->nT; else return dp.soft ? cN : cN - 1; }();
+        const int nx = [&]() -> int { if constexpr (FH) return es->nx; else return dp.xoff[b + 1] - x0; }();
+        const int nvd = [&]() -> int { if constexpr (FH) return es->nvd; else return 3 * (dp.cvoff[b + 1] - dp.cvoff[b]); }();
+        const double *vsrc = [&]() -> const double * { if constexpr (FH) return (const double *)es->vsrc; else return dp.vrec + 3 * (size_t)dp.cvoff[b]; }();
+        const auto t_soft = [&]() -> int { if constexpr (FH) return es->soft; else return dp.soft; };
+        const auto t_c2 = [&]() -> int { if constexpr (FH) return es->c2; else return dp.c2; };
         constexpr int UX = 4, UV = 16, NA = 192;
         double tau = 0.0, sx[UX], sv[UV];
         if (wave == 0) {
-            if (kk < nT) tau = x[x0 + kk];
+            long long *fst = nullptr, f_iss = 0;
+            if constexpr (!es_nostamps<ES>::value && !FH) fst = es->front;
+            if (fst) { asm volatile("" :: "v"(x + x0 + kk), "v"(nT)); f_iss = (long long)wall_clock64(); }
+            if constexpr (!FH) { if (kk < nT) tau = x[x0 + kk]; }
+            if (fst) { asm volatile("" :: "v"(tau)); const long long f_in = (long long)wall_clock64(); if (kk == 0) { fst[0] = f_iss; fst[1] = f_in; } }
         } else {
 #pragma unroll
             for (int u = 0; u < UX; u++) { const int i = nT + t2 + u * NA; sx[u] = nx > 0 ? x[x0 + (i < nx ? i : nx - 1)] : 0.0; }
@@ -1146,13 +1155,14 @@
         }
         if (es->sync()) return;
         if (wave == 0) {
+            if constexpr (FH) tau = es->tau;
             if (kk < nT) xs[kk] = tau;
-            if (dp.soft) {
-                if (kk < cN) Tc[kk] = tau_to_T(tau, dp.c2 != 0);
+            if (t_soft()) {
+                if (kk < cN) Tc[kk] = tau_to_T(tau, t_c2() != 0);
             } else if (kk == 0) {
                 const int Ms1 = cN - 1;
                 double sum = 0.0;
-                for (int i = 0; i < Ms1; i++) Tc[i] = tau_to_T(xs[i], dp.c2 != 0);
+                for (int i = 0; i < Ms1; i++) Tc[i] = tau_to_T(xs[i], t_c2() != 0);
                 Tc[Ms1] = 0.0;
                 for (int i = 0; i <= Ms1; i++) sum += Tc[i];
                 const double den = 1.0 + sum;
diff --git a/fast-racing_amd/csrc/frx_launch_forms.hpp b/fast-racing_amd/csrc/frx_launch_forms.hpp
--- a/fast-racing_amd/csrc/frx_launch_forms.hpp
+++ b/fast-racing_amd/csrc/frx_launch_forms.hpp
@@ -23,12 +23,12 @@
     }
 };
 
-struct EvalClusterForm { bool argp, et, tail, ho, ch, geo; };
+struct EvalClusterForm { bool argp, et, tail, ho, ch, geo; bool old_front = false; };
 inline bool operator==(const EvalClusterForm &a, const EvalClusterForm &b) {
-    return a.argp == b.argp && a.et == b.et && a.tail == b.tail && a.ho == b.ho && a.ch == b.ch && a.geo == b.geo;
+    return a.argp == b.argp && a.et == b.et && a.tail == b.tail && a.ho == b.ho && a.ch == b.ch && a.geo == b.geo && a.old_front == b.old_front;
 }
 struct EvalSwitches {
-    bool argptr, early_t, tail, handoff, chain, geom;
+    bool argptr, early_t, tail, handoff, chain, geom; bool old_front = false;
     constexpr bool handoff_on() const { return handoff && argptr && tail; }
     constexpr bool chain_on() const { return chain && handoff_on(); }
     constexpr bool geom_on() const { return geom && handoff_on() && early_t; }
@@ -39,6 +39,7 @@
     else if (s.handoff_on()) f = {true, s.early_t, true, true, chained, false};
     else if (s.argptr) f = {true, s.early_t, !(s.early_t && !s.tail), false, false, false};
     else f = {false, s.early_t, true, false, false, false};
+    f.old_front = s.old_front && f.argp && f.et;
     return !f.argp || have_dev_args;
 }
 inline int eval_cluster_raised_forms(const EvalSwitches &s, EvalClusterForm out[4]) {
diff --git a/include/frx_debug.h b/include/frx_debug.h
--- a/include/frx_debug.h
+++ b/include/frx_debug.h
@@ -21,6 +21,7 @@
 int frx_debug_set_eval_fused(frx_problem *p, int enable);
 int frx_debug_eval_fused(const frx_problem *p);
 int frx_debug_eval_geometry(const frx_problem *p);
+int frx_debug_eval_front(const frx_problem *p);
 int frx_debug_set_eval_solo(frx_problem *p, int mode);
 int frx_debug_penalty_kernel(const frx_problem *p);
 int frx_debug_eval_solo(const frx_problem *p);
```

Result: faster. 2.834 billion samples/s, median of 6 (+5.0%).
